# NingZhang1/pyscf_isdf

Measured on AMD Instinct MI355X. Metric: isdf_build_plus_get_jk_wall_time, lower is better.
Workload: dtype f64

## Files before the change

include/mi355_isdf.h:

```cpp
#ifndef MI355_ISDF_H
#define MI355_ISDF_H

#include <stdint.h>

#ifdef __cplusplus
extern "C" {
#endif

typedef struct isdf_ctx* isdf_handle;

#define ISDF_OK 0
#define ISDF_ERR_ARG 1
#define ISDF_ERR_HIP 2
#define ISDF_ERR_LIB 3
#define ISDF_ERR_NUM 4

int isdf_abi_version(void);

int isdf_create(int device_id, isdf_handle* out);
int isdf_destroy(isdf_handle h);
int isdf_set_stream(isdf_handle h, void* hip_stream);
const char* isdf_last_error(isdf_handle h);
int64_t isdf_workspace_bytes(isdf_handle h);
int isdf_release_workspace(isdf_handle h);
// ... 22 lines not shown
int isdf_eval_ao_deriv2(isdf_handle h, const int32_t* atm, int natm, const int32_t* bas, int nbas, const double* env,
                        int nenv, const double* Ls, int nimgs, const double* rcut, const double* d_coords,
                        int64_t ngrids, double* d_ao, int64_t ld, int64_t plane_stride);
int isdf_eval_ao_k_deriv1(isdf_handle h, const int32_t* atm, int natm, const int32_t* bas, int nbas, const double* env,
                          int nenv, const double* Ls, int nimgs, const double* rcut, const double kpt[3], int periodic_part,
                          const double* d_coords, int64_t ngrids, double* d_re, double* d_im, int64_t ld,
                          int64_t plane_stride);

int isdf_eval_ao_k(isdf_handle h,
                   const int32_t* atm, int natm, const int32_t* bas, int nbas,
                   const double* env, int nenv,
                   const double* Ls, int nimgs, const double* rcut,
                   const double kpt[3], int periodic_part,
                   const double* d_coords, int64_t ngrids,
                   double* d_re, double* d_im, int64_t ld);

int isdf_block_row_absmax(isdf_handle h, const double* d_src, int nrow, int64_t ld, int nblk, const int64_t* d_blk_off,
                          double* d_out);
int isdf_gather_cols(isdf_handle h, const double* d_src, int nrow, int64_t ld_src,
                     const int64_t* d_idx, int64_t n, double* d_dst, int64_t ld_dst);

int isdf_partition_by_atom(isdf_handle h, const double* d_coords, int64_t ngrids, const double* atom_coords, int natm,
                           const double a[9], double tie_atol, int32_t* d_owner);

int isdf_select_ip(isdf_handle h, const double* d_ao, int nao, int64_t ld,
                   int nblk, const int64_t* blk_off, const int32_t* nip,
                   double tol, double tie_rtol,
                   double* d_L, int64_t ldL, int64_t* d_piv, int32_t* rank);

int isdf_select_ip_ws(isdf_handle h, const double* d_ao, int nao, int64_t ld,
                      int nblk, const int64_t* blk_off, const int32_t* nip,
                      double tol, double tie_rtol,
                      double* d_L, int64_t ldL, int64_t* d_piv, int32_t* rank,
                      void* d_work, int64_t work_bytes);
int64_t isdf_select_ip_work_bytes(int nao, int64_t m);

int isdf_select_ip_gram(isdf_handle h, double* d_A, int m, int64_t ldA, int nip, double tol, double tie_rtol,
                        int panel, int64_t* d_piv, int32_t* rank);

int isdf_select_ip_cplx(isdf_handle h, const double* d_ao, int nao, int nh, int64_t ld,
                        int nblk, const int64_t* blk_off, const int32_t* nip,
                        double tol, double tie_rtol,
                        double* d_L, int64_t ldL, int64_t* d_piv, int32_t* rank);

int isdf_fit_from_chol(isdf_handle h, double* d_L, int k, int64_t m, int64_t ldL,
                       const int64_t* d_piv);

int isdf_fit_prepare(isdf_handle h, const double* d_ao, int nao, int64_t ld,
                     const int64_t* d_ip, int P, double reg_rel, double* d_aoP, double* d_chol,
                     double* reg_used);
int isdf_fit_apply(isdf_handle h, const double* d_chol, const double* d_aoP, int P, int nao,
                   const double* d_ao, int64_t ng, int64_t ld, int forward_only,
                   double* d_theta, int64_t ldt);
int isdf_fit_prepare_cplx(isdf_handle h, const double* d_ao, int nao, int nh, int64_t ld,
                          const int64_t* d_ip, int P, double reg_rel, double* d_aoP, double* d_chol,
                          double* reg_used);
int isdf_fit_apply_cplx(isdf_handle h, const double* d_chol, const double* d_aoP, int P, int nao, int nh,
                        const double* d_ao, int64_t ng, int64_t ld, int forward_only,
                        double* d_theta, int64_t ldt);
int isdf_fit_global(isdf_handle h, const double* d_ao, int nao, int64_t ngrids, int64_t ld,
                    const int64_t* d_ip, int P, double reg_rel, double* d_theta, int64_t ldt,
                    double* d_aoP, double* reg_used);

int isdf_gather_aoP(isdf_handle h, const double* d_ao, int nao, int64_t ld, const int64_t* d_ip, int P,
                    double* d_aoP);
int isdf_gram_sq(isdf_handle h, const double* d_aoP, int P, int nao, int nh, double* d_A);
int isdf_pair_gram_rows(isdf_handle h, const double* d_aoP, int P, int nao, int nh, const double* d_ao,
                        int64_t ng, int64_t ld, double* d_B, int64_t ldb);
int isdf_block_chol(isdf_handle h, const double* d_A, int P, int nblk, const int32_t* blk_off,
                    double shift_rel, double* d_D, double* shift_used);
int isdf_block_solve(isdf_handle h, const double* d_D, int P, int nblk, const int32_t* blk_off, int side,
                     int trans, double* d_X, int64_t n, int64_t ldx);
int isdf_block_invert(isdf_handle h, const double* d_D, int P, int nblk, const int32_t* blk_off, double* d_Dinv);
int isdf_block_apply(isdf_handle h, const double* d_Dinv, int64_t ldd, int nblk, const int32_t* blk_off,
                     double* d_X, int64_t n, int64_t ldx);
int isdf_pair_rows_block_apply(isdf_handle h, const double* d_aoP, int P, int nao, const double* d_ao, int64_t ng,
                               int64_t ld, const double* d_Dinv, int64_t ldd, int nblk, const int32_t* blk_off,
                               double* d_B, int64_t ldb);
int isdf_pair_rows_squared(isdf_handle h, const double* d_aoP, int rows, int nao, const double* d_ao, int64_t ng,
                           int64_t ld, int* squared);
int isdf_pair_rows_frontier(isdf_handle h, const double* d_aoP, int nnew, int nao, const double* d_ao, int64_t ng,
                            int64_t ld, int squared, const double* d_Dinv, int64_t ldd, int nblk, const int32_t* blk_off,
                            double* d_B, int64_t ldb, int have);

int isdf_gram_prod(isdf_handle h, const double* d_aoP, int P, int nao, const double* d_psiP, int nocc, double* d_A);
int isdf_pair_prod_rows(isdf_handle h, const double* d_aoP, int P, int nao, const double* d_psiP, int nocc,
                        const double* d_ao, int64_t ld, const double* d_psi, int64_t ldpsi, int64_t ng,
                        double* d_B, int64_t ldb);
int isdf_factor_solve_half(isdf_handle h, const double* d_fac, int P, int backward, double* d_X, int64_t n, int64_t ldx);
int isdf_gram_prod_cplx(isdf_handle h, const double* d_aoP, int P, int nao, int nh, const double* d_psiP, int npsi, int npsi_h,
                        double* d_A);
int isdf_pair_prod_rows_cplx(isdf_handle h, const double* d_aoP, int P, int nao, int nh, const double* d_psiP, int npsi,
                             int npsi_h, const double* d_ao, int64_t ld, const double* d_psi, int64_t ldpsi, int64_t ng,
                             double* d_B, int64_t ldb);

int isdf_shift_diag(isdf_handle h, double* d_A, int P, double shift_rel);
int isdf_chol_inplace(isdf_handle h, double* d_A, int P, double shift_rel, double* d_scratch, double* reg_used);

int isdf_factor_solve(isdf_handle h, const double* d_fac, int P, double* d_X, int64_t n, int64_t ldx);

int isdf_bj_probe_vectors(isdf_handle h, double* d_T, int n, const double* d_fac, const double* d_D, int P,
                          int nblk, const int32_t* blk_off);
int isdf_rows_combine(isdf_handle h, const double* d_E, int n, int64_t ldE, int rows, const double* d_Y,
                      int64_t ng, int64_t ldy, double* d_F, int64_t ldf, int accumulate);

int isdf_bj_probe_rows(isdf_handle h, double* d_T, int n, const double* d_fac, const double* d_D, int P, int nblk,
                       const int32_t* blk_off, const double* d_Yp, int64_t ng, int64_t ldy, double* d_F, int64_t ldf);

int isdf_gather_T(isdf_handle h, const double* d_L, int k, int64_t ldL, const int64_t* d_piv,
                  double* d_T);
int isdf_W_from_factor(isdf_handle h, const double* d_F, int P, int kind, double* d_M, int64_t ldm);

int isdf_coulomb_W(isdf_handle h, const double* d_theta, int P, int64_t ldt,
                   const int32_t mesh[3], const double a[9],
                   int row0, int nrows, int batch, int upper_only, double* d_W, int64_t ldw);
int isdf_coulG_half(isdf_handle h, const int32_t mesh[3], const double a[9], double* d_out);
int isdf_spectral_supported(isdf_handle h, const int32_t mesh[3], int batch, int* ok);
int isdf_spectral_rows(isdf_handle h, const double* d_in, int nrows, int64_t ld, const int32_t mesh[3], const int32_t* d_idx,
                       const double* d_scale, int npts, int batch, double* d_out, int64_t ldx);
int isdf_coulomb_rows(isdf_handle h, const double* d_in, int nrows, int64_t ld,
                      const int32_t mesh[3], const double a[9], int batch, double* d_out, int64_t ldo);
int isdf_symmetrize_upper(isdf_handle h, double* d_W, int P, int64_t ldw);
int isdf_symmetrize_mean(isdf_handle h, double* d_W, int P, int64_t ldw, int antisymmetric);

int isdf_get_j(isdf_handle h, const double* d_ao, int nao, int64_t ngrids, int64_t ld,
               const int32_t mesh[3], const double a[9],
               const double* d_dm, int nset, double* d_vj);
int isdf_rho(isdf_handle h, const double* d_ao, int nao, int64_t ng, int64_t ld,
             const double* d_dm, int nset, double* d_rho, int64_t ldrho);
int isdf_coulomb_potential(isdf_handle h, double* d_rho_inout, int nset, int64_t ldrho,
                           const int32_t mesh[3], const double a[9]);
int isdf_vj_from_vR(isdf_handle h, const double* d_ao, int nao, int64_t ng, int64_t ld,
                    const double* d_vR, int nset, int64_t ldv, double* d_vj);

int isdf_get_k_exact(isdf_handle h, const double* d_ao, int nao, int64_t ngrids, int64_t ld,
                     const double* d_C, int nocc, const int32_t mesh[3], const double a[9],
                     int i0, int ni, int max_rows, double* d_vk);

int isdf_get_k(isdf_handle h, const double* d_aoP, int P, int nao,
               const double* d_W, int64_t ldw, int row0, int nrows,
               const double* d_dm, int nset, double* d_vk);

int isdf_coulG_q(isdf_handle h, const int32_t mesh[3], const double a[9], const double q[3], int wrap_around,
                 double omega, double* d_out);

int isdf_coulomb_Wq(isdf_handle h, const double* d_theta, int P, int64_t ldt, const int32_t mesh[3],
                    const double* d_coulG, double weight, int row0, int nrows, int batch,
                    int upper_only, double* d_Wre, double* d_Wim, int64_t ldw);
int isdf_symmetrize_hermitian(isdf_handle h, double* d_Wre, double* d_Wim, int P, int64_t ldw);
int isdf_finish_Wq(isdf_handle h, const double* d_Wre, const double* d_Wim, int P, int64_t ldw,
                   const double* d_phase, double* d_Wc);
int isdf_get_k_pair(isdf_handle h, const double* d_A1, const double* d_A2, const double* d_D2,
                    const double* d_Wq, int P, int nao, double scale, double* d_vk);

int isdf_get_k_exact_kpt(isdf_handle h, const double* d_u1r, const double* d_u1i, int nao, int64_t ld1,
                         const double* d_m2r, const double* d_m2i, int nocc, int64_t ld2, const int32_t mesh[3],
                         const double* d_coulG, double weight, int i0, int ni, int max_rows, double* d_vk_re,
                         double* d_vk_im);

int isdf_coulomb_rows_q(isdf_handle h, const double* d_rows, int nrows, int64_t ld, const int32_t mesh[3],
                        const double* d_coulG, double* d_re, double* d_im);
int isdf_nyquist_spectra(isdf_handle h, const double* d_rows, int nrows, int64_t ld, const int32_t mesh[3], int axis,
                         double* d_re, double* d_im);
int isdf_zhadamard_planes(isdf_handle h, double* d_Ar, double* d_Ai, int64_t lda, const double* d_Br, const double* d_Bi,
                          int64_t ldb, int rows, int64_t cols);
int isdf_rho_k(isdf_handle h, const double* d_ur, const double* d_ui, int nao, int64_t ng, int64_t ld,
               const double* d_DTr, const double* d_DTi, double scale, double* d_rho);
int isdf_vj_k(isdf_handle h, const double* d_ur, const double* d_ui, int nao, int64_t ng, int64_t ld,
              const double* d_vR, double* d_vj_re, double* d_vj_im);

int isdf_pp_local_potential(isdf_handle h, int natm, const double* coords, const double* pp_par,
                            const int32_t mesh[3], const double a[9], double* d_vlocR);
int isdf_pp_projector_overlaps(isdf_handle h, const int32_t* atm, int natm, const int32_t* bas, int nbas,
                               const double* env, int nenv, const double* coords, const double kpt[3],
                               const int32_t* proj_tab, const double* proj_rl, int nproj,
                               const int32_t mesh[3], const double a[9], double* d_out);

int isdf_pp_local_force(isdf_handle h, const double* d_rho, int nset, int64_t ldrho, int natm, const double* coords,
                        const double* pp_par, const int32_t mesh[3], const double a[9], double* d_out);
int isdf_pp_projector_overlaps_ip(isdf_handle h, const int32_t* atm, int natm, const int32_t* bas, int nbas,
                                  const double* env, int nenv, const double* coords, const double kpt[3],
                                  const int32_t* proj_tab, const double* proj_rl, int nproj,
                                  const int32_t mesh[3], const double a[9], double* d_out);
int isdf_rowdot3(isdf_handle h, int M, int64_t K, double alpha, const double* d_A, int64_t lda, int64_t astride, const double* d_s,
                 const double* d_B, int64_t ldb, int accumulate, double* d_out, int64_t ldo);
int isdf_gga_aow(isdf_handle h, int M, int64_t K, const double* d_ao, int64_t ld, int64_t plane, const double* d_w, int64_t ldw,
                 double* d_Z, int64_t ldz, double* d_G, int64_t ldg, int64_t gstride);

int isdf_gemm_nn(isdf_handle h, int M, int64_t N, int K, double alpha, const double* d_A, int64_t lda, const double* d_B,
                 int64_t ldb, double beta, double* d_C, int64_t ldc);
int isdf_hadamard_rows(isdf_handle h, double* d_X, int64_t ldx, const double* d_Y, int64_t ldy, int rows, int64_t cols);

int isdf_uniform_grid(isdf_handle h, const int32_t mesh[3], const double a[9], double* d_coords_soa);
int isdf_rho_pair(isdf_handle h, const double* d_aoA, int nA, const double* d_aoB, int nB, int64_t ng, int64_t ld,
                  const double* d_dm, int nset, double* d_rho, int64_t ldrho);
int isdf_mg_embed_density(isdf_handle h, const double* d_field, int nset, const int32_t mesh_sub[3], double scale,
                          double* d_spec, const int32_t mesh[3], int accumulate);
int isdf_mg_restrict_potential(isdf_handle h, const double* d_spec, int nset, const int32_t mesh[3],
                               const int32_t mesh_sub[3], double scale, double* d_field);
int isdf_mg_coulomb_kernel(isdf_handle h, double* d_spec, int nset, const int32_t mesh[3], const double a[9]);
int isdf_lda_exchange(isdf_handle h, const double* d_rho, int64_t n, double* d_exc, double* d_vxc);
int isdf_lda_vwn_add(isdf_handle h, const double* d_rho, int64_t n, double* d_exc, double* d_vxc);
// ... 33 lines not shown
```

pyscf_isdf_amd/backend.py:

```python
import ctypes
import os
import numpy as np
import torch
from . import lib as _lib

_vp = ctypes.c_void_p


def _np_ptr(a):
    return a.ctypes.data_as(_vp)


class HipBackend:
    name = 'hip-gfx950'

    def __init__(self, device=0):
        if not torch.cuda.is_available():
            raise _lib.IsdfError('no GPU visible to torch; the ISDF path has no CPU fallback')
        self.device = torch.device('cuda', device)
        torch.cuda.set_device(self.device)
        self.handle = _lib.Handle(device)
        if os.environ.get('ISDF_TRSM') == 'subst':
            self.set_option('trsm_substitution', 1)
        if os.environ.get('ISDF_OWN_FFT') in ('0', '1', '2'):
# ... 217 lines not shown

    def gram_sq(self, aoP, A, nh=0):
        self._stream()
        self.handle.call('isdf_gram_sq', self._p(aoP), aoP.shape[0], aoP.shape[1], int(nh), self._p(A))

    def pair_gram_rows(self, aoP, ao, ng, B, nh=0):
        self._stream()
        self.handle.call('isdf_pair_gram_rows', self._p(aoP), aoP.shape[0], aoP.shape[1], int(nh), self._p(ao), int(ng),
                         ao.stride(0), self._p(B), B.stride(0))

    def gram_prod(self, aoP, psiP, A):
        self._stream()
        assert aoP.is_contiguous() and psiP.is_contiguous() and A.is_contiguous() and aoP.shape[0] == psiP.shape[0]
        self.handle.call('isdf_gram_prod', self._p(aoP), aoP.shape[0], aoP.shape[1], self._p(psiP), psiP.shape[1], self._p(A))

    def pair_prod_rows(self, aoP, psiP, ao, psi, ng, B):
        self._stream()
        assert aoP.is_contiguous() and psiP.is_contiguous() and aoP.shape[0] == psiP.shape[0]
        assert ao.stride(1) == 1 and psi.stride(1) == 1 and B.stride(1) == 1
        self.handle.call('isdf_pair_prod_rows', self._p(aoP), aoP.shape[0], aoP.shape[1], self._p(psiP), psiP.shape[1],
                         self._p(ao), ao.stride(0), self._p(psi), psi.stride(0), int(ng), self._p(B), B.stride(0))

    def gram_prod_cplx(self, aoP, nh, psiP, npsi_h, A):
        self._stream()
        assert aoP.is_contiguous() and psiP.is_contiguous() and A.is_contiguous() and aoP.shape[0] == psiP.shape[0]
        self.handle.call('isdf_gram_prod_cplx', self._p(aoP), aoP.shape[0], aoP.shape[1], int(nh), self._p(psiP), psiP.shape[1],
                         int(npsi_h), self._p(A))

    def pair_prod_rows_cplx(self, aoP, nh, psiP, npsi_h, ao, psi, ng, B):
        self._stream()
        assert aoP.is_contiguous() and psiP.is_contiguous() and aoP.shape[0] == psiP.shape[0]
        assert ao.stride(1) == 1 and psi.stride(1) == 1 and B.stride(1) == 1
        self.handle.call('isdf_pair_prod_rows_cplx', self._p(aoP), aoP.shape[0], aoP.shape[1], int(nh), self._p(psiP),
                         psiP.shape[1], int(npsi_h), self._p(ao), ao.stride(0), self._p(psi), psi.stride(0), int(ng), self._p(B),
                         B.stride(0))

    def factor_solve_half(self, fac, backward, X):
        self._stream()
        self.handle.call('isdf_factor_solve_half', self._p(fac), fac.shape[0], int(bool(backward)), self._p(X), X.shape[1],
                         X.stride(0))

    def block_chol(self, A, blk_off, shift_rel, D):
        self._stream()
        blk_off = np.ascontiguousarray(blk_off, dtype=np.int32)
        used = ctypes.c_double(0.0)
        self.handle.call('isdf_block_chol', self._p(A), A.shape[0], len(blk_off) - 1, _np_ptr(blk_off), float(shift_rel),
                         self._p(D), ctypes.byref(used))
        return used.value

    def block_solve(self, D, blk_off, side, trans, X):
        self._stream()
        blk_off = np.ascontiguousarray(blk_off, dtype=np.int32)
        n = X.shape[1] if side == 0 else X.shape[0]
        self.handle.call('isdf_block_solve', self._p(D), D.stride(0), len(blk_off) - 1, _np_ptr(blk_off), int(side), int(trans),
                         self._p(X), int(n), X.stride(0))

    def block_invert(self, D, blk_off, Dinv):
        self._stream()
        blk_off = np.ascontiguousarray(blk_off, dtype=np.int32)
        assert D.is_contiguous() and Dinv.is_contiguous() and Dinv.shape == D.shape
        self.handle.call('isdf_block_invert', self._p(D), D.shape[0], len(blk_off) - 1, _np_ptr(blk_off), self._p(Dinv))

    def block_apply(self, Dinv, blk_off, X):
        self._stream()
        blk_off = np.ascontiguousarray(blk_off, dtype=np.int32)
        self.handle.call('isdf_block_apply', self._p(Dinv), Dinv.stride(0), len(blk_off) - 1, _np_ptr(blk_off), self._p(X),
                         X.shape[1], X.stride(0))

    def pair_rows_block_apply(self, aoP, ao, ng, Dinv, blk_off, B):
        self._stream()
        blk_off = np.ascontiguousarray(blk_off, dtype=np.int32)
        assert aoP.stride(1) == 1 and aoP.stride(0) == aoP.shape[1]
        self.handle.call('isdf_pair_rows_block_apply', self._p(aoP), aoP.shape[0], aoP.shape[1], self._p(ao), int(ng), ao.stride(0),
                         self._p(Dinv), Dinv.stride(0), len(blk_off) - 1, _np_ptr(blk_off), self._p(B), B.stride(0))

    def pair_rows_squared(self, aoP, rows, ao, ng):
        self._stream()
        sq = ctypes.c_int(0)
        self.handle.call('isdf_pair_rows_squared', self._p(aoP), int(rows), aoP.shape[1], self._p(ao), int(ng), ao.stride(0),
                         ctypes.byref(sq))
        return bool(sq.value)

    def pair_rows_frontier(self, aoP_new, ao, ng, squared, Dinv, blk_off, B, have):
        self._stream()
        blk_off = np.ascontiguousarray(blk_off, dtype=np.int32)
        nnew = aoP_new.shape[0]
        assert aoP_new.stride(1) == 1 and aoP_new.stride(0) == aoP_new.shape[1] and B.stride(1) == 1
        assert have + nnew <= B.shape[0] and blk_off[0] == 0 and blk_off[-1] <= have + nnew and B.shape[1] >= ng
        assert len(blk_off) == 1 or (Dinv.shape[0] >= blk_off[-1] and Dinv.shape[1] >= blk_off[-1])
        self.handle.call('isdf_pair_rows_frontier', self._p(aoP_new) if nnew else None, nnew, aoP_new.shape[1], self._p(ao), int(ng),
                         ao.stride(0), int(bool(squared)), self._p(Dinv) if len(blk_off) > 1 else None, Dinv.stride(0) if len(blk_off) > 1 else 0,
                         len(blk_off) - 1, _np_ptr(blk_off), self._p(B), B.stride(0), int(have))

    def shift_diag(self, A, shift_rel):
        self._stream()
        self.handle.call('isdf_shift_diag', self._p(A), A.shape[0], float(shift_rel))

    def chol_inplace(self, A, shift_rel, scratch=None):
        self._stream()
        reg = ctypes.c_double(0.0)
        assert scratch is None or scratch.numel() >= A.numel()
        self.handle.call('isdf_chol_inplace', self._p(A), A.shape[0], float(shift_rel),
                         self._p(scratch) if scratch is not None else None, ctypes.byref(reg))
        return reg.value

    def factor_solve(self, fac, X):
        self._stream()
        self.handle.call('isdf_factor_solve', self._p(fac), fac.shape[0], self._p(X), X.shape[1], X.stride(0))

    def bj_probe_rows(self, T, fac, D, blk_off, Yp, ng, F):
        self._stream()
        blk_off = np.ascontiguousarray(blk_off, dtype=np.int32)
        self.handle.call('isdf_bj_probe_rows', self._p(T), T.shape[0], self._p(fac), self._p(D), D.shape[0],
                         len(blk_off) - 1, _np_ptr(blk_off), self._p(Yp), int(ng), Yp.stride(0), self._p(F), F.stride(0))

    def bj_probe_vectors(self, T, fac, D, blk_off):
        self._stream()
        blk_off = np.ascontiguousarray(blk_off, dtype=np.int32)
        assert T.is_contiguous()
        self.handle.call('isdf_bj_probe_vectors', self._p(T), T.shape[0], self._p(fac), self._p(D), D.shape[0],
                         len(blk_off) - 1, _np_ptr(blk_off))

    def rows_combine(self, E, Y, F, accumulate=False):
        self._stream()
        assert E.stride(1) == 1 and Y.stride(1) == 1 and F.stride(1) == 1 and E.shape[1] == Y.shape[0]
        self.handle.call('isdf_rows_combine', self._p(E), E.shape[0], E.stride(0), E.shape[1], self._p(Y), Y.shape[1],
                         Y.stride(0), self._p(F), F.stride(0), int(bool(accumulate)))

    def gather_T(self, L, k, piv, T):
        self._stream()
        assert T.is_contiguous() and T.shape == (k, k)
        self.handle.call('isdf_gather_T', self._p(L), int(k), L.stride(0), self._p(piv), self._p(T))

    def W_from_factor(self, F, kind, M):
        self._stream()
        assert F.is_contiguous()
        self.handle.call('isdf_W_from_factor', self._p(F), M.shape[0], int(kind), self._p(M), M.stride(0))

    def fit_global(self, ao, ngrids, ip, reg_rel, theta, aoP):
        self._stream()
        assert ip.dtype == torch.int64 and aoP.is_contiguous()
        reg = ctypes.c_double(0.0)
        self.handle.call('isdf_fit_global', self._p(ao), ao.shape[0], int(ngrids), ao.stride(0), self._p(ip),
                         ip.numel(), float(reg_rel), self._p(theta), theta.stride(0), self._p(aoP), ctypes.byref(reg))
        return reg.value

    def coulomb_W(self, theta, mesh, a, row0, nrows, batch, W, upper_only=False):
        self._stream()
        mesh = np.ascontiguousarray(mesh, dtype=np.int32)
        a = np.ascontiguousarray(a, dtype=np.float64)
        self.handle.call('isdf_coulomb_W', self._p(theta), theta.shape[0], theta.stride(0), _np_ptr(mesh), _np_ptr(a),
                         int(row0), int(nrows), int(batch), int(bool(upper_only)), self._p(W), W.stride(0))

    def coulomb_rows(self, rows, mesh, a, batch, out=None):
        self._stream()
        out = rows if out is None else out
        mesh = np.ascontiguousarray(mesh, dtype=np.int32)
        a = np.ascontiguousarray(a, dtype=np.float64)
        self.handle.call('isdf_coulomb_rows', self._p(rows), rows.shape[0], rows.stride(0), _np_ptr(mesh), _np_ptr(a),
                         int(batch), self._p(out), out.stride(0))

    def spectral_supported(self, mesh, batch=512):
        ok = ctypes.c_int(0)
        mesh = np.ascontiguousarray(mesh, dtype=np.int32)
        self.handle.call('isdf_spectral_supported', _np_ptr(mesh), int(batch), ctypes.byref(ok))
        return bool(ok.value)

    def coulG_half(self, mesh, a):
        self._stream()
        mesh = np.ascontiguousarray(mesh, dtype=np.int32)
        a = np.ascontiguousarray(a, dtype=np.float64)
        out = self.empty((int(mesh[0]) * int(mesh[1]) * (int(mesh[2]) // 2 + 1),))
        self.handle.call('isdf_coulG_half', _np_ptr(mesh), _np_ptr(a), self._p(out))
        return self.to_host(out).reshape(int(mesh[0]), int(mesh[1]), int(mesh[2]) // 2 + 1)

    def spectral_rows(self, rows, mesh, idx, scale, out, batch=512):
        self._stream()
        mesh = np.ascontiguousarray(mesh, dtype=np.int32)
        assert rows.is_contiguous() and out.stride(1) == 1 and idx.dtype == torch.int32 and out.stride(0) % 2 == 0
        self.handle.call('isdf_spectral_rows', self._p(rows), rows.shape[0], rows.stride(0), _np_ptr(mesh), self._p(idx),
                         self._p(scale), int(idx.numel()), int(batch), self._p(out), out.stride(0))

    def symmetrize_upper(self, W):
        self._stream()
        self.handle.call('isdf_symmetrize_upper', self._p(W), W.shape[0], W.stride(0))

    def symmetrize_mean(self, W, antisymmetric=False):
        self._stream()
        self.handle.call('isdf_symmetrize_mean', self._p(W), W.shape[0], W.stride(0), int(bool(antisymmetric)))

    def get_j(self, ao, ngrids, mesh, a, dm, vj):
        self._stream()
        mesh = np.ascontiguousarray(mesh, dtype=np.int32)
        a = np.ascontiguousarray(a, dtype=np.float64)
        assert dm.is_contiguous() and vj.is_contiguous()
        self.handle.call('isdf_get_j', self._p(ao), ao.shape[0], int(ngrids), ao.stride(0), _np_ptr(mesh), _np_ptr(a),
                         self._p(dm), dm.shape[0], self._p(vj))

    def rho(self, ao, ng, dm, rho):
        self._stream()
        self.handle.call('isdf_rho', self._p(ao), ao.shape[0], int(ng), ao.stride(0), self._p(dm), dm.shape[0],
                         self._p(rho), rho.stride(0))

    def coulomb_potential(self, rho, mesh, a):
        self._stream()
        mesh = np.ascontiguousarray(mesh, dtype=np.int32)
        a = np.ascontiguousarray(a, dtype=np.float64)
        self.handle.call('isdf_coulomb_potential', self._p(rho), rho.shape[0], rho.stride(0), _np_ptr(mesh), _np_ptr(a))

    def vj_from_vR(self, ao, ng, vR, vj):
        self._stream()
        self.handle.call('isdf_vj_from_vR', self._p(ao), ao.shape[0], int(ng), ao.stride(0), self._p(vR), vR.shape[0],
                         vR.stride(0), self._p(vj))

    def get_k(self, aoP, W, row0, nrows, dm, vk):
        self._stream()
        assert aoP.is_contiguous() and dm.is_contiguous() and vk.is_contiguous()
        self.handle.call('isdf_get_k', self._p(aoP), aoP.shape[0], aoP.shape[1], self._p(W), W.stride(0), int(row0),
                         int(nrows), self._p(dm), dm.shape[0], self._p(vk))

    def get_k_exact(self, ao, ngrids, C, mesh, a, i0, ni, max_rows, vk):
        self._stream()
        mesh = np.ascontiguousarray(mesh, dtype=np.int32)
        a = np.ascontiguousarray(a, dtype=np.float64)
        assert C.is_contiguous() and vk.is_contiguous()
        self.handle.call('isdf_get_k_exact', self._p(ao), ao.shape[0], int(ngrids), ao.stride(0), self._p(C), C.shape[1],
                         _np_ptr(mesh), _np_ptr(a), int(i0), int(ni), int(max_rows), self._p(vk))

    def gemm_nn(self, A, B, C, alpha=1.0, beta=0.0):
        self._stream()
        self.handle.call('isdf_gemm_nn', A.shape[0], B.shape[1], A.shape[1], float(alpha), self._p(A), A.stride(0), self._p(B),
                         B.stride(0), float(beta), self._p(C), C.stride(0))

    def hadamard_rows(self, X, Y):
        self._stream()
        self.handle.call('isdf_hadamard_rows', self._p(X), X.stride(0), self._p(Y), Y.stride(0), X.shape[0], X.shape[1])

    def gemm_nt(self, A, B, C, alpha=1.0, beta=0.0, kscale=None):
        self._stream()
        M, K = A.shape
        N = B.shape[0]
        assert B.shape[1] == K and tuple(C.shape) == (M, N) and A.stride(1) == 1 and B.stride(1) == 1 and C.stride(1) == 1
        ks = self._p(kscale) if kscale is not None else _vp(0)
        self.handle.call('isdf_gemm_nt', M, N, K, float(alpha), self._p(A), A.stride(0), self._p(B), B.stride(0), ks,
                         float(beta), self._p(C), C.stride(0))

    def gemm_nt_had3(self, A, H, B3, C3, alpha=1.0, beta=0.0):
        self._stream()
        M, K = A.shape
        N = B3.shape[1]
        assert tuple(B3.shape) == (3, N, K) and tuple(C3.shape) == (3, M, N) and A.stride(1) == 1 and B3.stride(2) == 1 and C3.stride(2) == 1
        assert H is None or (tuple(H.shape) == (M, K) and H.stride(1) == 1)
        self.handle.call('isdf_gemm_nt_had3', M, N, K, float(alpha), self._p(A), A.stride(0), self._p(H) if H is not None else _vp(0),
                         H.stride(0) if H is not None else 0, self._p(B3), B3.stride(1), B3.stride(0), float(beta), self._p(C3),
                         C3.stride(1), C3.stride(0))

    def pack_table_pm(self, table, mesh, idx, scale, s, a):
        self._stream()
        mesh = np.ascontiguousarray(mesh, dtype=np.int32)
        assert idx.dtype == torch.int32 and table.is_contiguous() and table.numel() == int(np.prod(mesh))
        assert s.is_contiguous() and a.is_contiguous() and s.numel() == a.numel()
        self.handle.call('isdf_pack_table_pm', self._p(table), _np_ptr(mesh), self._p(idx), int(idx.numel()), float(scale),
                         self._p(s), self._p(a), int(s.numel()))

# ... 274 lines not shown
```

pyscf_isdf_amd/csrc/common.h:

```cpp
#pragma once
#include <hip/hip_runtime.h>
#include <rocblas/rocblas.h>
#include <rocsolver/rocsolver.h>
#include <hipfft/hipfft.h>
#include <cstdint>
#include <cstdio>
#include <cstring>
#include <string>
#include <vector>
#include <map>
#include "../../include/mi355_isdf.h"

struct FftPlan {
  hipfftHandle fwd = 0, bwd = 0;
  size_t work_bytes = 0;
};

struct ProfRec {
  hipEvent_t e0 = nullptr, e1 = nullptr;
};
struct ProfEntry {
  std::vector<ProfRec> recs;
  double work = 0.0;
  double ms = 0.0;
  int64_t launches = 0;
};

struct WsKernel {
  double alpha = 0.0;
  double ak[9] = {0};
  int mesh[3] = {0, 0, 0};
  double maxq[3] = {0, 0, 0};
  const double* vq = nullptr;
};

struct isdf_ctx {
  int profiling = 0;
  std::map<std::string, ProfEntry> prof;
  int device = 0;
  hipStream_t stream = nullptr;
  rocblas_handle blas = nullptr;
  std::string err;
  std::map<std::vector<int>, FftPlan> plans;
  std::map<std::string, std::pair<void*, size_t>> ws;
  int num_cu = 256;
  int trsm_substitution = 0;
  int own_fft = 2;
  int gemm_nn_own = 0;
  int attr_gemm_b = 0, attr_gemm_nn = 0, attr_gram_tri = 0, attr_herm = 0;
  int cand_gram = 1;
  int conv_pipe = 1;
  int conv_sub_rows = 0;
  int gram_pivot_tpb = 256;
  int gram_compact = 1;
  int gram_compact_permille = 875;
  int block_apply_waves = 16;
  int block_apply_reg = 1;
  double coul_omega = 0.0;
  double coul_rc = 0.0;
  int coul_sphere = 0;
  WsKernel wsk;
};

int isdf_fail(isdf_handle h, int code, const char* fmt, ...);
void* isdf_ws(isdf_handle h, const char* name, size_t bytes);
int isdf_get_plan(isdf_handle h, const int32_t mesh[3], int batch, FftPlan** out);
int get_coulG_half(isdf_handle h, const int32_t mesh[3], const double a[9], double extra_scale, double** out);
bool conv_rows_own_supported(const int32_t mesh[3], int nb);
bool conv_rows_q_own_supported(isdf_handle h, const int32_t mesh[3], int nb);
bool spectral_rows_own_supported(isdf_handle h, const int32_t mesh[3], int nb);
int spectral_rows_own(isdf_handle h, const double* d_in, int nb, const int32_t mesh[3], const int32_t* d_idx, const double* d_scale,
                      int npts, double* d_out, int64_t ldx, HIP_vector_type<double, 2u>* zbuf);
int conv_rows_q_own(isdf_handle h, const double* d_in, double* d_re, double* d_im, int nb, const int32_t mesh[3], const double* tab,
                    double2* zhalf, double2* zfull);
int conv_rows_own(isdf_handle h, const double* d_in, double* d_out, int nb, const int32_t mesh[3], const double* cg,
                  double2* zbuf);

#define HIP_TRY(h, expr)                                                                    \
  do {                                                                                      \
    hipError_t e_ = (expr);                                                                 \
    if (e_ != hipSuccess)                                                                   \
      return isdf_fail(h, ISDF_ERR_HIP, "%s:%d %s -> %s", __FILE__, __LINE__, #expr,        \
                       hipGetErrorString(e_));                                              \
  } while (0)
#define BLAS_TRY(h, expr)                                                                   \
  do {                                                                                      \
    rocblas_status s_ = (expr);                                                             \
    if (s_ != rocblas_status_success)                                                       \
      return isdf_fail(h, ISDF_ERR_LIB, "%s:%d %s -> rocblas status %d", __FILE__, __LINE__, \
                       #expr, (int)s_);                                                     \
  } while (0)
#define FFT_TRY(h, expr)                                                                    \
  do {                                                                                      \
    hipfftResult r_ = (expr);                                                               \
    if (r_ != HIPFFT_SUCCESS)                                                               \
      return isdf_fail(h, ISDF_ERR_LIB, "%s:%d %s -> hipfft result %d", __FILE__, __LINE__,  \
                       #expr, (int)r_);                                                     \
  } while (0)
#define KERNEL_CHECK(h) HIP_TRY(h, hipGetLastError())
#define ARG_CHECK(h, cond)                                                                  \
  do {                                                                                      \
    if (!(cond)) return isdf_fail(h, ISDF_ERR_ARG, "%s:%d argument check failed: %s",       \
                                  __FILE__, __LINE__, #cond);                               \
  } while (0)

static inline int64_t cdiv(int64_t a, int64_t b) { return (a + b - 1) / b; }

struct ProfScope {
  isdf_handle h;
  ProfRec rec;
  ProfEntry* ent = nullptr;
  ProfScope(isdf_handle h_, const char* name, double work, int64_t launches = 1) : h(h_) {
    if (!h || !h->profiling) return;
    ent = &h->prof[name];
    ent->work += work;
    ent->launches += launches;
    if (hipEventCreate(&rec.e0) != hipSuccess || hipEventCreate(&rec.e1) != hipSuccess) { ent = nullptr; return; }
    (void)hipEventRecord(rec.e0, h->stream);
  }
  ~ProfScope() {
    if (!ent) return;
    (void)hipEventRecord(rec.e1, h->stream);
    ent->recs.push_back(rec);
  }
};

int gemm_nt_f64(isdf_handle h, int M, int N, int64_t K, double alpha, const double* A, int64_t lda,
                const double* B, int64_t ldb, double beta, double* C, int64_t ldc);
int gemm_nt_f64_scaled(isdf_handle h, int M, int N, int64_t K, double alpha, const double* A, int64_t lda,
                       const double* B, int64_t ldb, const double* kscale, double beta, double* C,
                       int64_t ldc);
int trsm_lower_left(isdf_handle h, bool trans, int m, int64_t n, const double* L, int64_t ldl, double* X, int64_t ldx);
int trsm_lower_right(isdf_handle h, bool trans, int m, int64_t n, const double* L, int64_t ldl, double* X, int64_t ldx);
int block_forward_solve(isdf_handle h, const double* D, int64_t ldd, int nblk, const int32_t* blk_off_host, double* X,
                        int64_t ldx, int64_t n);
int block_apply_inverse(isdf_handle h, const double* Dinv, int64_t ldd, int nblk, const int32_t* blk_off_host, double* X,
                        int64_t ldx, int64_t n, bool square_input = false);
int transpose_rm(isdf_handle h, const double* src, int64_t lds, int64_t rows, int64_t cols, double* dst, int64_t ldd);
int tri_left(isdf_handle h, bool trans, int m, int64_t n, const double* L, int64_t ldl, double* X, int64_t ldx);
int tri_right(isdf_handle h, bool trans, int m, int64_t n, const double* L, int64_t ldl, double* X, int64_t ldx);
bool gemm_nn_f64_supported(isdf_handle h, int64_t M, int64_t N, int64_t K, const double* A, int64_t lda, const double* B,
                           int64_t ldb);
int gemm_nn_f64(isdf_handle h, int64_t M, int64_t N, int64_t K, const double* A, int64_t lda, const double* B, int64_t ldb,
                double* C, int64_t ldc, bool square);
int gemm_rm(isdf_handle h, char opA, char opB, int64_t M, int64_t N, int64_t K, double alpha,
            const double* A, int64_t lda, const double* B, int64_t ldb, double beta, double* C,
            int64_t ldc);

__host__ __device__ inline int64_t gram_tri_row(int64_t r) {
  const int64_t tm = r >> 8;
  return 32768 * tm * (tm + 1) + (r & 255) * ((tm + 1) << 8);
}
static inline int64_t gram_tri_size(int64_t m) { return m > 0 ? gram_tri_row(m - 1) + (((m - 1) >> 8) + 1) * 256 : 0; }
struct GramTriUnit { int blk, tm, tn, pad; };
int gram_tri_blocks(isdf_handle h, const double* X, int64_t ldx, int K, const GramTriUnit* d_units, int64_t nunits,
                    const int64_t* d_blk_off, int64_t row0, const int64_t* d_tri_off, double* S, double flop);
```

pyscf_isdf_amd/csrc/coulomb.hip:

```cpp
#include "common.h"

namespace {

struct Recip { double b[9]; };
__device__ inline double g2_of(int ix, int iy, int iz, int n0, int n1, int n2, const Recip& r) {
  const double fx = (ix < (n0 + 1) / 2) ? ix : ix - n0;
  const double fy = (iy < (n1 + 1) / 2) ? iy : iy - n1;
  const double fz = (iz < (n2 + 1) / 2) ? iz : iz - n2;
  const double gx = fx * r.b[0] + fy * r.b[3] + fz * r.b[6];
  const double gy = fx * r.b[1] + fy * r.b[4] + fz * r.b[7];
  const double gz = fx * r.b[2] + fy * r.b[5] + fz * r.b[8];
  return gx * gx + gy * gy + gz * gz;
}

__device__ inline double range_factor(double g2, double omega) {
  if (omega == 0.0) return 1.0;
  const double e = exp(-0.25 * g2 / (omega * omega));
  return omega > 0.0 ? e : 1.0 - e;
}
__device__ inline double kernel_value(double g2, double omega, double rc) {
  const double fourpi = 4.0 * 3.14159265358979323846;
  if (rc > 0.0) return g2 == 0.0 ? 0.5 * fourpi * rc * rc : fourpi / g2 * (1.0 - cos(sqrt(g2) * rc));
  return g2 == 0.0 ? 0.0 : fourpi / g2 * range_factor(g2, omega);
}
// ... 250 lines not shown
  const int64_t gc = (int64_t)mesh[0] * mesh[1] * (mesh[2] / 2 + 1);
  ARG_CHECK(h, ldt == G);
  if (nrows == 0) return ISDF_OK;
  if (batch > nrows) batch = nrows;
  double* cg = nullptr;
  int rc = get_coulG_half(h, mesh, a, 1.0, &cg);
  if (rc) return rc;
  double* V = (double*)isdf_ws(h, "coul_V", sizeof(double) * (size_t)batch * G);
  double2* Z = (double2*)isdf_ws(h, "coul_Z", sizeof(double2) * (size_t)batch * gc);
  if (!V || !Z) return ISDF_ERR_HIP;
  const double det = a[0] * (a[4] * a[8] - a[5] * a[7]) - a[1] * (a[3] * a[8] - a[5] * a[6]) +
                     a[2] * (a[3] * a[7] - a[4] * a[6]);
  const double w = fabs(det) / (double)G;
  for (int r = row0; r < row0 + nrows; r += batch) {
    const int nb = std::min(batch, row0 + nrows - r);
    rc = convolve_rows(h, d_theta + (int64_t)r * ldt, V, nb, mesh, cg, Z);
    if (rc) return rc;
    const int c0 = upper_only ? r : 0;
    rc = gemm_nt_f64(h, nb, P - c0, G, w, V, G, d_theta + (int64_t)c0 * ldt, ldt, 0.0,
                     d_W + (int64_t)r * ldw + c0, ldw);
    if (rc) return rc;
  }
  return ISDF_OK;
}

extern "C" int isdf_coulomb_potential(isdf_handle h, double* d_rho, int nset, int64_t ldrho,
                                      const int32_t mesh[3], const double a[9]) {
  if (!h) return ISDF_ERR_ARG;
  ARG_CHECK(h, d_rho && mesh && a && nset > 0);
  const int64_t G = (int64_t)mesh[0] * mesh[1] * mesh[2];
  const int64_t gc = (int64_t)mesh[0] * mesh[1] * (mesh[2] / 2 + 1);
  ARG_CHECK(h, ldrho == G);
  const double det = a[0] * (a[4] * a[8] - a[5] * a[7]) - a[1] * (a[3] * a[8] - a[5] * a[6]) +
                     a[2] * (a[3] * a[7] - a[4] * a[6]);
  double* cg = nullptr;
  int rc = get_coulG_half(h, mesh, a, fabs(det) / (double)G, &cg);
  if (rc) return rc;
  double2* Z = (double2*)isdf_ws(h, "coul_Z", sizeof(double2) * (size_t)nset * gc);
  if (!Z) return ISDF_ERR_HIP;
  return convolve_rows(h, d_rho, d_rho, nset, mesh, cg, Z);
}

extern "C" int isdf_coulomb_rows(isdf_handle h, const double* d_in, int nrows, int64_t ld,
                                 const int32_t mesh[3], const double a[9], int batch, double* d_out,
                                 int64_t ldo) {
  if (!h) return ISDF_ERR_ARG;
  ARG_CHECK(h, d_in && d_out && mesh && a && nrows >= 0 && batch > 0);
  const int64_t G = (int64_t)mesh[0] * mesh[1] * mesh[2];
  const int64_t gc = (int64_t)mesh[0] * mesh[1] * (mesh[2] / 2 + 1);
  ARG_CHECK(h, ld == G && ldo == G);
  if (nrows == 0) return ISDF_OK;
  if (batch > nrows) batch = nrows;
  double* cg = nullptr;
  int rc = get_coulG_half(h, mesh, a, 1.0, &cg);
  if (rc) return rc;
  double2* Z = (double2*)isdf_ws(h, "coul_Z", sizeof(double2) * (size_t)batch * gc);
  if (!Z) return ISDF_ERR_HIP;
  for (int r = 0; r < nrows; r += batch) {
    const int nb = std::min(batch, nrows - r);
    rc = convolve_rows(h, d_in + (int64_t)r * ld, d_out + (int64_t)r * ldo, nb, mesh, cg, Z);
    if (rc) return rc;
  }
  return ISDF_OK;
}

extern "C" int isdf_coulG_half(isdf_handle h, const int32_t mesh[3], const double a[9], double* d_out) {
  if (!h) return ISDF_ERR_ARG;
  ARG_CHECK(h, mesh && a && d_out);
  double* cg = nullptr;
  int rc = get_coulG_half(h, mesh, a, 1.0, &cg);
  if (rc) return rc;
  const int64_t gc = (int64_t)mesh[0] * mesh[1] * (mesh[2] / 2 + 1);
  HIP_TRY(h, hipMemcpyAsync(d_out, cg, sizeof(double) * gc, hipMemcpyDeviceToDevice, h->stream));
  return ISDF_OK;
}

extern "C" int isdf_spectral_supported(isdf_handle h, const int32_t mesh[3], int batch, int* ok) {
  if (!h) return ISDF_ERR_ARG;
  ARG_CHECK(h, mesh && ok && batch > 0);
  *ok = spectral_rows_own_supported(h, mesh, batch) ? 1 : 0;
  return ISDF_OK;
}

extern "C" int isdf_spectral_rows(isdf_handle h, const double* d_in, int nrows, int64_t ld, const int32_t mesh[3],
                                  const int32_t* d_idx, const double* d_scale, int npts, int batch, double* d_out, int64_t ldx) {
  if (!h) return ISDF_ERR_ARG;
  ARG_CHECK(h, d_in && d_out && mesh && d_idx && d_scale && nrows >= 0 && batch > 0 && npts > 0);
  const int64_t G = (int64_t)mesh[0] * mesh[1] * mesh[2];
  const int64_t gc = (int64_t)mesh[0] * mesh[1] * (mesh[2] / 2 + 1);
  ARG_CHECK(h, ld == G && npts <= gc);
  if (nrows == 0) return ISDF_OK;
  if (batch > nrows) batch = nrows;
  if (!spectral_rows_own_supported(h, mesh, batch))
    return isdf_fail(h, ISDF_ERR_ARG, "isdf_spectral_rows: mesh %d x %d x %d is not covered by the plane FFT", mesh[0], mesh[1], mesh[2]);
  double2* Z = (double2*)isdf_ws(h, "coul_Z", sizeof(double2) * (size_t)batch * gc);
  if (!Z) return ISDF_ERR_HIP;
  for (int r = 0; r < nrows; r += batch) {
    const int nb = std::min(batch, nrows - r);
    int rc = spectral_rows_own(h, d_in + (int64_t)r * ld, nb, mesh, d_idx, d_scale, npts, d_out + (int64_t)r * ldx, ldx, Z);
    if (rc) return rc;
  }
  return ISDF_OK;
}
```

pyscf_isdf_amd/csrc/fft_conv.hip:

```cpp
#include "common.h"
#include <type_traits>

namespace {

constexpr int TPB = 256;
constexpr int MAXSTAGE = 12;

struct Axis {
  int n;
  int nstage;
  int radix[MAXSTAGE];
  const double2* tw;
};

__device__ inline double2 cadd(double2 a, double2 b) { return make_double2(a.x + b.x, a.y + b.y); }
__device__ inline double2 csub(double2 a, double2 b) { return make_double2(a.x - b.x, a.y - b.y); }
__device__ inline double2 cmul(double2 a, double2 b) { return make_double2(a.x * b.x - a.y * b.y, a.x * b.y + a.y * b.x); }
template <int SIGN>
__device__ inline double2 mul_si(double2 a) { return SIGN > 0 ? make_double2(-a.y, a.x) : make_double2(a.y, -a.x); }
template <int SIGN>
__device__ inline double2 twid(const double2* __restrict__ tw, int idx) {
  double2 w = tw[idx];
  if (SIGN > 0) w.y = -w.y;
  return w;
// ... 388 lines not shown
      }
      __syncthreads();
      z = stockham_all<1>(z, (z == x) ? y : x, ax, ZC, M);
    }
  }
  for (int c = threadIdx.x; c < n * ZC; c += TPB) {
    const int e = c / ZC, m = c - e * ZC;
    if (m < M) base[(int64_t)e * es + m] = z[c];
  }
}

template <int SIGN, int ZCT>
__device__ inline void fft_fast(double2* buf, const Axis& ax, int Ls, const double2* tw) {
  fft<SIGN, TPB, 2048 / TPB, true, FixedLines<ZCT>>(buf, ax, Ls, ZCT, tw);
}

template <int ZCT>
__global__ __launch_bounds__(TPB) void z_r2c_fast_kernel(const double* __restrict__ in, double2* __restrict__ out,
                                                         int64_t nlines, Axis ax) {
  extern __shared__ double2 lds[];
  const int n = ax.n, nh = n / 2 + 1;
  constexpr int Ls = ZCT + 1;
  double2* x = lds;
  double2* tw = lds + n * Ls;
  for (int k = threadIdx.x; k < n; k += TPB) tw[k] = ax.tw[k];
  const int64_t line0 = (int64_t)blockIdx.x * 2 * ZCT;
  const int nl = (int)min((int64_t)2 * ZCT, nlines - line0);
  const double* src = in + line0 * n;
  const float inv_n = 1.0f / (float)n;
  for (int c = threadIdx.x; c < 2 * ZCT * n; c += TPB) {
    const int l = (int)(((float)c + 0.5f) * inv_n), e = c - l * n;
    const double v = (l < nl) ? src[c] : 0.0;
    ((double*)(x + e * Ls + (l >> 1)))[l & 1] = v;
  }
  __syncthreads();
  fft_fast<-1, ZCT>(x, ax, Ls, tw);
  double2* dstc = out + line0 * nh;
  const float inv_nh = 1.0f / (float)nh;
  for (int c = threadIdx.x; c < nl * nh; c += TPB) {
    const int l = (int)(((float)c + 0.5f) * inv_nh), k = c - l * nh;
    const int m = l >> 1;
    const double2 zk = x[k * Ls + m];
    const double2 zn = x[(k == 0 ? 0 : n - k) * Ls + m];
    double2 r;
    if ((l & 1) == 0) r = make_double2(0.5 * (zk.x + zn.x), 0.5 * (zk.y - zn.y));
    else r = make_double2(0.5 * (zk.y + zn.y), -0.5 * (zk.x - zn.x));
    dstc[c] = r;
  }
}

template <int ZCT>
__global__ __launch_bounds__(TPB) void z_c2r_fast_kernel(const double2* __restrict__ in, double* __restrict__ out,
                                                         int64_t nlines, Axis ax) {
  extern __shared__ double2 lds[];
  const int n = ax.n, nh = n / 2 + 1;
  constexpr int Ls = ZCT + 1;
  double2* x = lds;
  double2* tw = lds + n * Ls;
  for (int k = threadIdx.x; k < n; k += TPB) tw[k] = ax.tw[k];
  const int64_t line0 = (int64_t)blockIdx.x * 2 * ZCT;
  const int nl = (int)min((int64_t)2 * ZCT, nlines - line0);
  const int M = (nl + 1) / 2;
  const double2* src = in + line0 * nh;
  const float inv_nh = 1.0f / (float)nh;
  for (int c = threadIdx.x; c < M * nh; c += TPB) {
    const int m = (int)(((float)c + 0.5f) * inv_nh), k = c - m * nh;
    double2 a = src[(int64_t)(2 * m) * nh + k];
    double2 b = (2 * m + 1 < nl) ? src[(int64_t)(2 * m + 1) * nh + k] : make_double2(0.0, 0.0);
    const bool selfconj = (k == 0) || (2 * k == n);
    if (selfconj) { a.y = 0.0; b.y = 0.0; }
    x[k * Ls + m] = make_double2(a.x - b.y, a.y + b.x);
    if (!selfconj) x[(n - k) * Ls + m] = make_double2(a.x + b.y, -a.y + b.x);
  }
  __syncthreads();
  fft_fast<1, ZCT>(x, ax, Ls, tw);
  double* dst = out + line0 * n;
  const float inv_n = 1.0f / (float)n;
  for (int c = threadIdx.x; c < nl * n; c += TPB) {
    const int l = (int)(((float)c + 0.5f) * inv_n), e = c - l * n;
    dst[c] = ((const double*)(x + e * Ls + (l >> 1)))[l & 1];
  }
}

template <int MODE, int ZCT>
__global__ __launch_bounds__(TPB) void strided_fft_fast_kernel(double2* __restrict__ data, int64_t os, int64_t es, int Mtot,
                                                               Axis ax, int ntile, const double* __restrict__ table) {
  extern __shared__ double2 lds[];
  const int n = ax.n;
  double2* x = lds;
  double2* tw = lds + n * ZCT;
  for (int k = threadIdx.x; k < n; k += TPB) tw[k] = ax.tw[k];
  const int nouter = gridDim.x / ntile;
  const int64_t outer = (MODE == 2) ? blockIdx.x % nouter : blockIdx.x / ntile;
  const int m0 = (int)((MODE == 2) ? blockIdx.x / nouter : blockIdx.x % ntile) * ZCT;
  const int M = min(ZCT, Mtot - m0);
  double2* base = data + outer * os + m0;
  for (int c = threadIdx.x; c < n * ZCT; c += TPB) {
    const int e = c / ZCT, m = c & (ZCT - 1);
    if (m < M) x[c] = base[(int64_t)e * es + m];
  }
  __syncthreads();
  if (MODE == 1) {
    fft_fast<1, ZCT>(x, ax, ZCT, tw);
  } else {
    fft_fast<-1, ZCT>(x, ax, ZCT, tw);
    if (MODE == 2) {
      const double* tb = table + m0;
      for (int c = threadIdx.x; c < n * ZCT; c += TPB) {
        const int e = c / ZCT, m = c & (ZCT - 1);
        if (m < M) {
          const double g = tb[(int64_t)e * es + m];
          double2 v = x[c];
          v.x *= g;
          v.y *= g;
          x[c] = v;
        }
      }
      __syncthreads();
      fft_fast<1, ZCT>(x, ax, ZCT, tw);
    }
  }
  for (int c = threadIdx.x; c < n * ZCT; c += TPB) {
    const int e = c / ZCT, m = c & (ZCT - 1);
    if (m < M) base[(int64_t)e * es + m] = x[c];
  }
}

constexpr int TPBP = 1024;
constexpr int PLANE_ENTRIES = 10240;
constexpr int PIPE_NT = 768;

template <int SIGN, int NT, int N, int RA, int RB, int MMAX>
__device__ __forceinline__ void fft_plane_fixed(double2* buf, int Ls, int M, const double2* tw) {
  static_assert(RA * RB == N, "two stages");
  stage<SIGN, RA, NT, ((N / RA) * MMAX + NT - 1) / NT, true, AnyLines>(buf, N, N, 1, Ls, M, tw, opaque_tid());
  stage<SIGN, RB, NT, ((N / RB) * MMAX + NT - 1) / NT, true, AnyLines>(buf, N, N / RA, RA, Ls, M, tw, opaque_tid());
}

struct PlaneAny {
  static constexpr int NT = TPBP, PER = PLANE_ENTRIES / TPBP;
  static constexpr int KS_HALF = PER, KS_PAIR = PER / 2 + 1, KS_FULL = PER;
  int n1, n2, n2h, npair;
  __device__ PlaneAny(const Axis& az, const Axis& ay) : n1(ay.n), n2(az.n), n2h(az.n / 2 + 1), npair((ay.n + 1) / 2) {}
  __device__ static int tid() { return threadIdx.x; }
  template <int SIGN, bool FULL>
  __device__ __forceinline__ static void transform(double2* buf, const Axis& ax, int Ls, int M, const double2* tw) {
    fft<SIGN, NT, PER, false, AnyLines>(buf, ax, Ls, M, tw);
  }
};
template <int N, int RA, int RB>
struct PlaneSquare {
  static constexpr int NT = PIPE_NT, n1 = N, n2 = N, n2h = N / 2 + 1, npair = (N + 1) / 2;
  static constexpr int KS_HALF = (n1 * n2h + NT - 1) / NT, KS_PAIR = (npair * n2h + NT - 1) / NT, KS_FULL = (N * N + NT - 1) / NT;
  constexpr PlaneSquare() = default;
  __device__ static int tid() { return opaque_tid(); }
  template <int SIGN, bool FULL>
  __device__ __forceinline__ static void transform(double2* buf, const Axis&, int Ls, int M, const double2* tw) {
    fft_plane_fixed<SIGN, NT, N, RA, RB, FULL ? N : N / 2 + 1>(buf, Ls, M, tw);
  }
};

__device__ inline double zero_of(const double*) { return 0.0; }
__device__ inline double2 zero_of(const double2*) { return make_double2(0.0, 0.0); }
template <int NT, int NPRE, class T>
__device__ __forceinline__ void prefetch(T (&pre)[NPRE], const T* __restrict__ src, int count, int tid) {
#pragma unroll
  for (int u = 0; u < NPRE; ++u) {
    const int c = tid + u * NT;
    pre[u] = c < count ? src[c] : zero_of(src);
  }
}

template <class D>
__device__ __forceinline__ void plane_fwd_body(const D d, double2* lds, int Lz, int bufsz, const Axis& az, const Axis& ay,
                                               double2* __restrict__ dst, double2 (&r)[D::KS_HALF]) {
  double2* x = lds;
  const double2* twz = lds + bufsz;
  const double2* twy = twz + d.n2;
  d.template transform<-1, false>(x, az, Lz, d.npair, twz);
  int tid = D::tid();
  const float inv_nh = 1.0f / (float)d.n2h;
#pragma unroll
  for (int u = 0; u < D::KS_HALF; ++u) {
    const int c = tid + u * D::NT;
    if (c < d.n1 * d.n2h) {
      const int l = fdiv(c, inv_nh), k = c - l * d.n2h;
      const int m = l >> 1;
      r[u] = separate_pair(x[k * Lz + m], x[(k == 0 ? 0 : d.n2 - k) * Lz + m], l & 1);
    }
  }
  __syncthreads();
#pragma unroll
  for (int u = 0; u < D::KS_HALF; ++u) {
    const int c = tid + u * D::NT;
    if (c < d.n1 * d.n2h) x[c] = r[u];
  }
  __syncthreads();
  d.template transform<-1, false>(x, ay, d.n2h, d.n2h, twy);
  tid = D::tid();
  for (int c = tid; c < d.n1 * d.n2h; c += D::NT) dst[c] = x[c];
}

template <class D>
__device__ __forceinline__ void plane_inv_body(const D d, double2* lds, int Lz, int bufsz, const Axis& az, const Axis& ay,
                                               double* __restrict__ dst, double2 (&za)[D::KS_PAIR], double2 (&zb)[D::KS_PAIR]) {
  double2* x = lds;
  const double2* twz = lds + bufsz;
  const double2* twy = twz + d.n2;
// ... 281 lines not shown
    static const int big[] = {16, 15, 12, 10, 9, 8, 6, 5, 4, 3, 2};
    int best[MAXSTAGE], nbest = MAXSTAGE + 1, bestmax = 1 << 30;
    int cur[MAXSTAGE];
    struct Rec {
      static void go(int rest, int maxr, int depth, int* cur, int* best, int& nbest, int& bestmax) {
        if (rest == 1) {
          const int mx = depth ? cur[0] : 1;
          if (depth < nbest || (depth == nbest && mx < bestmax)) {
            nbest = depth; bestmax = mx;
            for (int i = 0; i < depth; ++i) best[i] = cur[i];
          }
          return;
        }
        if (depth + 1 > nbest || depth >= MAXSTAGE) return;
        for (int r : big)
          if (r <= maxr && rest % r == 0) { cur[depth] = r; go(rest / r, r, depth + 1, cur, best, nbest, bestmax); }
      }
    };
    Rec::go(n, 16, 0, cur, best, nbest, bestmax);
    if (nbest <= MAXSTAGE) {
      ax->nstage = nbest;
      for (int i = 0; i < nbest; ++i) ax->radix[i] = best[i];
      return true;
    }
  }
  const int order[4] = {4, 2, 3, 5};
  for (int r : order)
    while (n % r == 0 && n > 1) {
      if (ax->nstage >= MAXSTAGE) return false;
      ax->radix[ax->nstage++] = r;
      n /= r;
    }
  for (int p = 7; n > 1 && p <= 13; p += 2)
    while (n % p == 0) {
      if (ax->nstage >= MAXSTAGE) return false;
      ax->radix[ax->nstage++] = p;
      n /= p;
    }
  return n == 1;
}

int make_axes(isdf_handle h, const int32_t mesh[3], Axis ax[3], const char* who) {
  for (int d = 0; d < 3; ++d) {
    if (!factorise(mesh[d], &ax[d])) return isdf_fail(h, ISDF_ERR_ARG, "%s: unsupported mesh dimension %d", who, mesh[d]);
    char name[32];
    snprintf(name, sizeof(name), "fft_tw_%d", mesh[d]);
    const bool fresh = h->ws.find(name) == h->ws.end();
    double2* tw = (double2*)isdf_ws(h, name, sizeof(double2) * (size_t)mesh[d]);
    if (!tw) return ISDF_ERR_HIP;
    if (fresh) {
      std::vector<double2> host(mesh[d]);
      for (int k = 0; k < mesh[d]; ++k) {
        const double t = -2.0 * 3.14159265358979323846 * (double)k / (double)mesh[d];
        host[k] = make_double2(cos(t), sin(t));
      }
      HIP_TRY(h, hipMemcpyAsync(tw, host.data(), sizeof(double2) * (size_t)mesh[d], hipMemcpyHostToDevice, h->stream));
      HIP_TRY(h, hipStreamSynchronize(h->stream));
    }
    ax[d].tw = tw;
  }
  return ISDF_OK;
}

template <bool FWD, class IN, class OUT>
void launch_z(isdf_handle h, bool fast, int L, const IN* in, OUT* out, int64_t nlines, const Axis& ax) {
  const dim3 grid((unsigned)cdiv(nlines, 2 * L));
  const size_t n = ax.n;
  if (fast) {
    const size_t lds = sizeof(double2) * (n * (L + 1) + n);
    with_lines(L, [&](auto z) {
      constexpr int ZCT = decltype(z)::value;
      if constexpr (FWD) z_r2c_fast_kernel<ZCT><<<grid, dim3(TPB), lds, h->stream>>>(in, out, nlines, ax);
      else z_c2r_fast_kernel<ZCT><<<grid, dim3(TPB), lds, h->stream>>>(in, out, nlines, ax);
    });
  } else {
    const size_t lds = sizeof(double2) * 2 * n * (L + 1);
    if constexpr (FWD) z_r2c_kernel<<<grid, dim3(TPB), lds, h->stream>>>(in, out, nlines, ax, L);
    else z_c2r_kernel<<<grid, dim3(TPB), lds, h->stream>>>(in, out, nlines, ax, L);
  }
}

template <int MODE>
void launch_strided(isdf_handle h, bool fast, int L, double2* data, int64_t nouter, int64_t os, int64_t es, int Mtot, const Axis& ax,
                    const double* table) {
  const int nt = (int)cdiv(Mtot, L);
  const dim3 grid((unsigned)(nouter * nt));
  const size_t n = ax.n;
  if (fast)
    with_lines(L, [&](auto z) {
      strided_fft_fast_kernel<MODE, decltype(z)::value><<<grid, dim3(TPB), sizeof(double2) * (n * L + n), h->stream>>>(
          data, os, es, Mtot, ax, nt, table);
    });
  else
    strided_fft_kernel<MODE><<<grid, dim3(TPB), sizeof(double2) * 2 * n * L, h->stream>>>(data, os, es, Mtot, ax, L, nt, table);
}

#define ISDF_PLANE_SIZES(X) X(64, 8, 8) X(72, 9, 8) X(80, 10, 8) X(96, 12, 8) X(100, 10, 10) X(108, 12, 9) X(120, 12, 10)
constexpr int PIPE_ANY = 1024, PIPE_Q_MAX = 96;

template <class F>
bool with_pipe_size(isdf_handle h, const Axis& az, const Axis& ay, int nmax, F f) {
  if (h->conv_pipe == 0 || ay.n != az.n || ay.n > nmax || ay.nstage != 2) return false;
#define ISDF_PLANE_SIZE(NN, RA, RB)                                \
  if (ay.n == NN && ay.radix[0] == RA && ay.radix[1] == RB) {      \
    f(PlaneSquare<NN, RA, RB>{});                                  \
    return true;                                                   \
  }
  ISDF_PLANE_SIZES(ISDF_PLANE_SIZE)
#undef ISDF_PLANE_SIZE
  return false;
}

template <class K>
int raise_lds(isdf_handle h, K kernel) {
  HIP_TRY(h, hipFuncSetAttribute((const void*)kernel, hipFuncAttributeMaxDynamicSharedMemorySize, LDS_MAX));
  return ISDF_OK;
}
dim3 pipe_grid(isdf_handle h, int nplanes) { return dim3((unsigned)std::min<int64_t>(nplanes, h->num_cu)); }

int launch_plane_fwd(isdf_handle h, const double* in, double2* out, const Axis* ax, const PlaneGeo& g, int nplanes, int pipe_max) {
  int rc = ISDF_OK;
  const bool piped = with_pipe_size(h, ax[2], ax[1], pipe_max, [&](auto d) {
    auto kernel = plane_fwd_pipe_kernel<decltype(d)>;
    if ((rc = raise_lds(h, kernel)) == ISDF_OK)
      kernel<<<pipe_grid(h, nplanes), dim3(PIPE_NT), g.bytes, h->stream>>>(in, out, ax[2], ax[1], g.Lz, g.bufsz, nplanes);
  });
  if (!piped && (rc = raise_lds(h, plane_fwd_kernel)) == ISDF_OK)
    plane_fwd_kernel<<<dim3((unsigned)nplanes), dim3(TPBP), g.bytes, h->stream>>>(in, out, ax[2], ax[1], g.Lz, g.bufsz);
  return rc;
}

int launch_plane_inv(isdf_handle h, const double2* in, double* out, const Axis* ax, const PlaneGeo& g, int nplanes, int pipe_max) {
  int rc = ISDF_OK;
  const bool piped = with_pipe_size(h, ax[2], ax[1], pipe_max, [&](auto d) {
    auto kernel = plane_inv_pipe_kernel<decltype(d)>;
    if ((rc = raise_lds(h, kernel)) == ISDF_OK)
      kernel<<<pipe_grid(h, nplanes), dim3(PIPE_NT), g.bytes, h->stream>>>(in, out, ax[2], ax[1], g.Lz, g.bufsz, nplanes);
  });
  if (!piped && (rc = raise_lds(h, plane_inv_kernel)) == ISDF_OK)
    plane_inv_kernel<<<dim3((unsigned)nplanes), dim3(TPBP), g.bytes, h->stream>>>(in, out, ax[2], ax[1], g.Lz, g.bufsz);
  return rc;
}

int launch_plane_c2c_inv(isdf_handle h, const double2* in, double* out_re, double* out_im, const Axis* ax, const PlaneGeo& g,
                         int nplanes) {
  int rc = ISDF_OK;
  const bool piped = with_pipe_size(h, ax[2], ax[1], PIPE_Q_MAX, [&](auto d) {
    if constexpr (decltype(d)::n1 <= PIPE_Q_MAX) {
      auto kernel = plane_c2c_inv_pipe_kernel<decltype(d)>;
      if ((rc = raise_lds(h, kernel)) == ISDF_OK)
        kernel<<<pipe_grid(h, nplanes), dim3(PIPE_NT), g.bytes, h->stream>>>(in, out_re, out_im, ax[2], ax[1], g.Lz, g.bufsz, nplanes);
    } else {
      rc = isdf_fail(h, ISDF_ERR_ARG, "launch_plane_c2c_inv: no pipelined kernel for %d^2", (int)decltype(d)::n1);
    }
  });
  if (!piped && (rc = raise_lds(h, plane_c2c_inv_kernel)) == ISDF_OK)
    plane_c2c_inv_kernel<<<dim3((unsigned)nplanes), dim3(TPBP), g.bytes, h->stream>>>(in, out_re, out_im, ax[2], ax[1], g.Lz, g.bufsz);
  return rc;
}

}

bool conv_rows_own_supported(const int32_t mesh[3], int nb) {
  if (nb < 1 || (int64_t)nb * mesh[0] * mesh[1] * 4 >= 2147483647LL || (int64_t)nb * mesh[1] * (mesh[2] / 2 + 1) >= 2147483647LL)
    return false;
  for (int d = 0; d < 3; ++d) {
    Axis ax;
    if (mesh[d] < 1 || mesh[d] > 1024 || !factorise(mesh[d], &ax)) return false;
    if (lines_per_tile(mesh[d], d == 2 ? 1 : 0) < 1) return false;
  }
  return true;
}

int conv_rows_own(isdf_handle h, const double* d_in, double* d_out, int nb, const int32_t mesh[3], const double* cg,
                  double2* zbuf) {
  const int n0 = mesh[0], n1 = mesh[1], n2 = mesh[2], n2h = n2 / 2 + 1;
  Axis ax[3];
  if (int rc = make_axes(h, mesh, ax, "conv_rows_own")) return rc;
  const int64_t gc = (int64_t)n0 * n1 * n2h;
  const int64_t nlines = (int64_t)nb * n0 * n1;
  ARG_CHECK(h, nlines * 4 < 2147483647LL && (int64_t)nb * cdiv((int64_t)n1 * n2h, 1) < 2147483647LL);
  const int LP = lines_per_tile(n2, 1);
  const int ZY = lines_per_tile(n1, 0), ZX = lines_per_tile(n0, 0);
  if (LP < 1 || ZY < 1 || ZX < 1) return isdf_fail(h, ISDF_ERR_ARG, "conv_rows_own: mesh too large for the LDS tiles");
  const int64_t G = (int64_t)n0 * n1 * n2;
  const int FZ = fast_lines(n2), FY = fast_lines(n1), FX = fast_lines(n0);
  const bool smooth = smooth235(ax[0]) && smooth235(ax[1]) && smooth235(ax[2]);
  const PlaneGeo geo = (h->own_fft == 2 && smooth && FX >= 1) ? plane_geometry(n1, n2, false) : PlaneGeo{0, 0, 0};
  ProfScope ps(h, geo.bytes ? "coulomb_conv_own_3pass[byte]" : "coulomb_conv_own_5pass[byte]", 32.0 * (double)G * nb,
               geo.bytes ? 3 : 5);
  if (geo.bytes) {
    const int sub = h->conv_sub_rows > 0 ? std::min(nb, h->conv_sub_rows) : nb;
    for (int r0 = 0; r0 < nb; r0 += sub) {
      const int nr = std::min(sub, nb - r0);
      double2* zb = zbuf + (int64_t)r0 * gc;
      const int nplanes = (int)((int64_t)nr * n0);
      if (int rc = launch_plane_fwd(h, d_in + (int64_t)r0 * G, zb, ax, geo, nplanes, PIPE_ANY)) return rc;
      launch_strided<2>(h, true, FX, zb, nr, gc, (int64_t)n1 * n2h, n1 * n2h, ax[0], cg);
      if (int rc = launch_plane_inv(h, zb, d_out + (int64_t)r0 * G, ax, geo, nplanes, PIPE_ANY)) return rc;
    }
    KERNEL_CHECK(h);
    return ISDF_OK;
  }
  const bool fast = smooth && FZ >= 1 && FY >= 1 && FX >= 1;
  const int Lz = fast ? FZ : LP, Ly = fast ? FY : ZY, Lx = fast ? FX : ZX;
  launch_z<true>(h, fast, Lz, d_in, zbuf, nlines, ax[2]);
  launch_strided<0>(h, fast, Ly, zbuf, (int64_t)nb * n0, (int64_t)n1 * n2h, (int64_t)n2h, n2h, ax[1], nullptr);
  launch_strided<2>(h, fast, Lx, zbuf, nb, gc, (int64_t)n1 * n2h, n1 * n2h, ax[0], cg);
  launch_strided<1>(h, fast, Ly, zbuf, (int64_t)nb * n0, (int64_t)n1 * n2h, (int64_t)n2h, n2h, ax[1], nullptr);
  launch_z<false>(h, fast, Lz, zbuf, d_out, nlines, ax[2]);
  KERNEL_CHECK(h);
  return ISDF_OK;
}

__global__ void spectral_pack_kernel(const double2* __restrict__ z, int64_t gc, const int32_t* __restrict__ idx,
                                     const double* __restrict__ scale, int npts, double2* __restrict__ out, int64_t ldx2) {
  const int64_t j = (int64_t)blockIdx.x * blockDim.x + threadIdx.x;
  if (j >= ldx2) return;
  const int row = blockIdx.y;
  double2 v = make_double2(0.0, 0.0);
  if (j < npts) {
    const double2 t = z[(int64_t)row * gc + idx[j]];
    const double s = scale[j];
    v = make_double2(t.x * s, t.y * s);
  }
  out[(int64_t)row * ldx2 + j] = v;
}

bool spectral_rows_own_supported(isdf_handle h, const int32_t mesh[3], int nb) {
  if (h->own_fft != 2 || !conv_rows_own_supported(mesh, nb)) return false;
  Axis ax[3];
  for (int d = 0; d < 3; ++d)
    if (!factorise(mesh[d], &ax[d]) || !smooth235(ax[d])) return false;
  return fast_lines(mesh[0]) >= 1 && plane_geometry(mesh[1], mesh[2], false).bytes != 0;
}

int spectral_rows_own(isdf_handle h, const double* d_in, int nb, const int32_t mesh[3], const int32_t* d_idx,
                      const double* d_scale, int npts, double* d_out, int64_t ldx, double2* zbuf) {
  const int n0 = mesh[0], n1 = mesh[1], n2 = mesh[2], n2h = n2 / 2 + 1;
  Axis ax[3];
  if (int rc = make_axes(h, mesh, ax, "spectral_rows_own")) return rc;
  const int64_t gc = (int64_t)n0 * n1 * n2h;
  const PlaneGeo geo = plane_geometry(n1, n2, false);
  const int FX = fast_lines(n0);
  ARG_CHECK(h, geo.bytes && FX >= 1 && (int64_t)nb * n0 < 2147483647LL && nb <= 65535 && (ldx & 1) == 0 && ldx >= 2 * (int64_t)npts);
  ProfScope ps(h, "spectral_rows_own[byte]", (8.0 * (double)n0 * n1 * n2 + 8.0 * (double)ldx) * nb, 3);
  if (int rc = launch_plane_fwd(h, d_in, zbuf, ax, geo, (int)((int64_t)nb * n0), PIPE_ANY)) return rc;
  launch_strided<0>(h, true, FX, zbuf, nb, gc, (int64_t)n1 * n2h, n1 * n2h, ax[0], nullptr);
  const int64_t ldx2 = ldx / 2;
  spectral_pack_kernel<<<dim3((unsigned)cdiv(ldx2, 256), (unsigned)nb), dim3(256), 0, h->stream>>>(zbuf, gc, d_idx, d_scale, npts,
                                                                                                  (double2*)d_out, ldx2);
  KERNEL_CHECK(h);
  return ISDF_OK;
}

bool conv_rows_q_own_supported(isdf_handle h, const int32_t mesh[3], int nb) {
  if (!h->own_fft) return false;
  if (nb < 1 || nb > 65535 || (int64_t)nb * mesh[0] >= 2147483647LL) return false;
  Axis ax[3];
  for (int d = 0; d < 3; ++d)
    if (mesh[d] < 2 || mesh[d] > 1024 || !factorise(mesh[d], &ax[d]) || !smooth235(ax[d])) return false;
  return fast_lines(mesh[0]) >= 1 && plane_geometry(mesh[1], mesh[2], false).bytes && plane_geometry(mesh[1], mesh[2], true).bytes;
}

int conv_rows_q_own(isdf_handle h, const double* d_in, double* d_re, double* d_im, int nb, const int32_t mesh[3],
                    const double* tab, double2* zhalf, double2* zfull) {
  const int n0 = mesh[0], n1 = mesh[1], n2 = mesh[2], n2h = n2 / 2 + 1;
  Axis ax[3];
  if (int rc = make_axes(h, mesh, ax, "conv_rows_q_own")) return rc;
  const int64_t G = (int64_t)n0 * n1 * n2, gc = (int64_t)n0 * n1 * n2h;
  const PlaneGeo geo_r = plane_geometry(n1, n2, false), geo_c = plane_geometry(n1, n2, true);
  const int FX = fast_lines(n0);
  ARG_CHECK(h, geo_r.bytes && geo_c.bytes && FX >= 1 && (int64_t)nb * n0 < 2147483647LL && nb <= 65535);
  ProfScope ps(h, "coulomb_conv_q_own[byte]", 64.0 * (double)G * nb, 5);
  const int nplanes = (int)((int64_t)nb * n0);
  if (int rc = launch_plane_fwd(h, d_in, zhalf, ax, geo_r, nplanes, PIPE_Q_MAX)) return rc;
  launch_strided<0>(h, true, FX, zhalf, nb, gc, (int64_t)n1 * n2h, n1 * n2h, ax[0], nullptr);
  expand_mul_kernel<<<dim3((unsigned)cdiv(G, 256), (unsigned)nb), dim3(256), 0, h->stream>>>(zhalf, zfull, tab, n0, n1, n2,
                                                                                            1.0 / (double)G);
  launch_strided<1>(h, true, FX, zfull, nb, G, (int64_t)n1 * n2, n1 * n2, ax[0], nullptr);
  if (int rc = launch_plane_c2c_inv(h, zfull, d_re, d_im, ax, geo_c, nplanes)) return rc;
  KERNEL_CHECK(h);
  return ISDF_OK;
}
```

pyscf_isdf_amd/csrc/fit.hip:

```cpp
#include "common.h"
#include <cstdlib>

namespace {

__global__ void gather_T_kernel(const double* __restrict__ L, int64_t ldL,
                                const int64_t* __restrict__ piv, int k, double* __restrict__ T) {
  const int s = blockIdx.x * blockDim.x + threadIdx.x;
  const int t = blockIdx.y;
  if (s >= k) return;
  T[(int64_t)t * k + s] = (s >= t) ? L[(int64_t)t * ldL + piv[s]] : 0.0;
}

__global__ void square_kernel(double* __restrict__ x, int64_t rows, int64_t cols, int64_t ld) {
  const int64_t c = (int64_t)blockIdx.x * blockDim.x + threadIdx.x;
  const int64_t r = blockIdx.y;
  if (c >= cols) return;
  const double v = x[r * ld + c];
  x[r * ld + c] = v * v;
}

__global__ void square_add_kernel(double* __restrict__ x, int64_t ld, const double* __restrict__ y, int64_t ldy,
                                  int64_t cols) {
  const int64_t c = (int64_t)blockIdx.x * blockDim.x + threadIdx.x;
  const int64_t r = blockIdx.y;
// ... 284 lines not shown
      for (int pp = 0; pp < np; ++pp) {
        const double v = y[(int64_t)pp * ldy];
#pragma unroll
        for (int j = 0; j < 8; ++j) acc[j] = fma(sE[j][pp], v, acc[j]);
      }
    }
  }
  if (live)
    for (int j = 0; j < n; ++j) F[(int64_t)j * ldf + g] = accumulate ? F[(int64_t)j * ldf + g] + acc[j] : acc[j];
}

__global__ void add_diag_const_kernel(double* __restrict__ A, int n, int64_t ld, double v) {
  const int i = blockIdx.x * blockDim.x + threadIdx.x;
  if (i < n) A[(int64_t)i * ld + i] += v;
}
}

extern "C" int isdf_block_chol(isdf_handle h, const double* d_A, int P, int nblk, const int32_t* blk_off,
                               double shift_rel, double* d_D, double* shift_used) {
  if (!h) return ISDF_ERR_ARG;
  ARG_CHECK(h, d_A && d_D && blk_off && P > 0 && nblk > 0 && blk_off[0] == 0 && blk_off[nblk] == P && shift_rel >= 0);
  int* info = (int*)isdf_ws(h, "fit_info", 256);
  if (!info) return ISDF_ERR_HIP;
  double* maxdiag = (double*)(info + 16);
  HIP_TRY(h, hipMemsetAsync(d_D, 0, sizeof(double) * (size_t)P * P, h->stream));
  hipLaunchKernelGGL(max_diag_kernel, dim3(1), dim3(256), 0, h->stream, d_A, P, maxdiag);
  double md = 0.0;
  HIP_TRY(h, hipMemcpyAsync(&md, maxdiag, sizeof(double), hipMemcpyDeviceToHost, h->stream));
  HIP_TRY(h, hipStreamSynchronize(h->stream));
  double worst = 0.0;
  for (int b = 0; b < nblk; ++b) {
    const int off = blk_off[b], nb = blk_off[b + 1] - off;
    if (nb <= 0) continue;
    ARG_CHECK(h, nb <= 65535);
    double reg = shift_rel;
    int h_info = 1;
    for (int attempt = 0; attempt < 6 && h_info != 0; ++attempt) {
      hipLaunchKernelGGL(copy_block_kernel, dim3((unsigned)cdiv(nb, 128), (unsigned)nb), dim3(128), 0, h->stream, d_A, P,
                         off, nb, d_D);
      if (reg > 0)
        hipLaunchKernelGGL(add_diag_const_kernel, dim3((unsigned)cdiv(nb, 256)), dim3(256), 0, h->stream,
                           d_D + (int64_t)off * P + off, nb, (int64_t)P, reg * md);
      KERNEL_CHECK(h);
      BLAS_TRY(h, rocsolver_dpotrf(h->blas, rocblas_fill_upper, nb, d_D + (int64_t)off * P + off, P, info));
      HIP_TRY(h, hipMemcpyAsync(&h_info, info, sizeof(int), hipMemcpyDeviceToHost, h->stream));
      HIP_TRY(h, hipStreamSynchronize(h->stream));
      if (h_info == 0) { worst = std::max(worst, reg); break; }
      reg = (reg > 0.0) ? reg * 100.0 : 1e-14;
    }
    if (h_info != 0)
      return isdf_fail(h, ISDF_ERR_NUM, "diagonal block %d of A_PP is not positive definite even with shift %g * max diag "
                       "(minor %d of %d)", b, reg / 100.0, h_info, nb);
  }
  if (shift_used) *shift_used = worst;
  return ISDF_OK;
}

extern "C" int isdf_block_solve(isdf_handle h, const double* d_D, int P, int nblk, const int32_t* blk_off, int side,
                                int trans, double* d_X, int64_t n, int64_t ldx) {
  if (!h) return ISDF_ERR_ARG;
  ARG_CHECK(h, d_D && d_X && blk_off && P > 0 && nblk > 0 && n > 0 && (side == 0 || side == 1) && (trans == 0 || trans == 1));
  ARG_CHECK(h, n < 2147483647LL && ldx < 2147483647LL);
  if (side == 0 && trans == 0 && !h->trsm_substitution) {
    ARG_CHECK(h, blk_off[0] == 0 && blk_off[nblk] <= P);
    return block_forward_solve(h, d_D, P, nblk, blk_off, d_X, ldx, n);
  }
  for (int b = 0; b < nblk; ++b) {
    const int off = blk_off[b], nb = blk_off[b + 1] - off;
    if (nb <= 0) continue;
    const double* Db = d_D + (int64_t)off * P + off;
    const int rc = (side == 0) ? tri_left(h, trans != 0, nb, n, Db, P, d_X + (int64_t)off * ldx, ldx)
                               : tri_right(h, trans != 0, nb, n, Db, P, d_X + off, ldx);
    if (rc) return rc;
  }
  return ISDF_OK;
}

namespace {
__global__ void block_identity_kernel(double* __restrict__ E, int P, const int32_t* __restrict__ blk_of_row) {
  const int64_t i = (int64_t)blockIdx.x * blockDim.x + threadIdx.x;
  if (i < (int64_t)P * P) E[i] = (i / P == i % P) ? 1.0 : 0.0;
  (void)blk_of_row;
}
}

extern "C" int isdf_block_invert(isdf_handle h, const double* d_D, int P, int nblk, const int32_t* blk_off, double* d_Dinv) {
  if (!h) return ISDF_ERR_ARG;
  ARG_CHECK(h, d_D && d_Dinv && blk_off && P > 0 && nblk > 0 && blk_off[0] == 0 && blk_off[nblk] <= P);
  hipLaunchKernelGGL(block_identity_kernel, dim3((unsigned)cdiv((int64_t)P * P, 256)), dim3(256), 0, h->stream, d_Dinv, P,
                     (const int32_t*)nullptr);
  KERNEL_CHECK(h);
  return block_forward_solve(h, d_D, P, nblk, blk_off, d_Dinv, P, P);
}

extern "C" int isdf_block_apply(isdf_handle h, const double* d_Dinv, int64_t ldd, int nblk, const int32_t* blk_off,
                                double* d_X, int64_t n, int64_t ldx) {
  if (!h) return ISDF_ERR_ARG;
  ARG_CHECK(h, d_Dinv && d_X && blk_off && nblk > 0 && n > 0 && ldx >= n && blk_off[0] == 0 && blk_off[nblk] <= ldd);
  return block_apply_inverse(h, d_Dinv, ldd, nblk, blk_off, d_X, ldx, n);
}

extern "C" int isdf_pair_rows_block_apply(isdf_handle h, const double* d_aoP, int P, int nao, const double* d_ao, int64_t ng,
                                          int64_t ld, const double* d_Dinv, int64_t ldd, int nblk, const int32_t* blk_off,
                                          double* d_B, int64_t ldb) {
  if (!h) return ISDF_ERR_ARG;
  ARG_CHECK(h, d_aoP && d_ao && d_Dinv && d_B && blk_off && P > 0 && nao > 0 && ng > 0 && ld >= ng && ldb >= ng && nblk > 0);
  ARG_CHECK(h, blk_off[0] == 0 && blk_off[nblk] == P);
  const bool own = gemm_nn_f64_supported(h, P, ng, nao, d_aoP, nao, d_ao, ld);
  int rc = product_rows(h, P, ng, nao, d_aoP, d_ao, ld, d_B, ldb, own);
  if (rc) return rc;
  return block_apply_inverse(h, d_Dinv, ldd, nblk, blk_off, d_B, ldb, ng, !own);
}

extern "C" int isdf_pair_rows_squared(isdf_handle h, const double* d_aoP, int rows, int nao, const double* d_ao, int64_t ng,
                                      int64_t ld, int* squared) {
  if (!h) return ISDF_ERR_ARG;
  ARG_CHECK(h, d_aoP && d_ao && squared && rows > 0 && nao > 0 && ng > 0 && ld >= ng);
  *squared = gemm_nn_f64_supported(h, rows, ng, nao, d_aoP, nao, d_ao, ld) ? 1 : 0;
  return ISDF_OK;
}

extern "C" int isdf_pair_rows_frontier(isdf_handle h, const double* d_aoP, int nnew, int nao, const double* d_ao, int64_t ng,
                                       int64_t ld, int squared, const double* d_Dinv, int64_t ldd, int nblk,
                                       const int32_t* blk_off, double* d_B, int64_t ldb, int have) {
  if (!h) return ISDF_ERR_ARG;
  ARG_CHECK(h, d_ao && d_B && nnew >= 0 && nnew <= 65535 && have >= 0 && nblk >= 0 && nao > 0 && ng > 0 && ld >= ng && ldb >= ng);
  ARG_CHECK(h, (nnew == 0 || d_aoP) && (nblk == 0 || (d_Dinv && blk_off && blk_off[0] == 0 && blk_off[nblk] <= have + nnew)));
  if (nnew > 0) {
    double* rows = d_B + (int64_t)have * ldb;
    int rc = squared ? product_rows(h, nnew, ng, nao, d_aoP, d_ao, ld, rows, ldb, true)
                     : gemm_rm(h, 'N', 'N', nnew, ng, nao, 1.0, d_aoP, nao, d_ao, ld, 0.0, rows, ldb);
    if (rc) return rc;
  }
  if (nblk == 0) return ISDF_OK;
  return block_apply_inverse(h, d_Dinv, ldd, nblk, blk_off, d_B, ldb, ng, !squared);
}

extern "C" int isdf_shift_diag(isdf_handle h, double* d_A, int P, double shift_rel) {
  if (!h) return ISDF_ERR_ARG;
  ARG_CHECK(h, d_A && P > 0 && shift_rel >= 0);
  if (shift_rel == 0.0) return ISDF_OK;
  int* info = (int*)isdf_ws(h, "fit_info", 256);
  if (!info) return ISDF_ERR_HIP;
  double* maxdiag = (double*)(info + 16);
  hipLaunchKernelGGL(max_diag_kernel, dim3(1), dim3(256), 0, h->stream, d_A, P, maxdiag);
  hipLaunchKernelGGL(add_diag_kernel, dim3((unsigned)cdiv(P, 256)), dim3(256), 0, h->stream, d_A, P, maxdiag, shift_rel);
  KERNEL_CHECK(h);
  return ISDF_OK;
}

extern "C" int isdf_chol_inplace(isdf_handle h, double* d_A, int P, double shift_rel, double* d_scratch,
                                 double* reg_used) {
  if (!h) return ISDF_ERR_ARG;
  ARG_CHECK(h, d_A && P > 0 && shift_rel >= 0);
  int* info = (int*)isdf_ws(h, "fit_info", 256);
  double* keep = d_scratch ? d_scratch : (double*)isdf_ws(h, "chol_keep", sizeof(double) * (size_t)P * P);
  if (!info || !keep) return ISDF_ERR_HIP;
  double* maxdiag = (double*)(info + 16);
  HIP_TRY(h, hipMemcpyAsync(keep, d_A, sizeof(double) * (size_t)P * P, hipMemcpyDeviceToDevice, h->stream));
  double reg = shift_rel;
  for (int attempt = 0; attempt < 5; ++attempt) {
    if (attempt > 0)
      HIP_TRY(h, hipMemcpyAsync(d_A, keep, sizeof(double) * (size_t)P * P, hipMemcpyDeviceToDevice, h->stream));
    if (reg > 0) {
      hipLaunchKernelGGL(max_diag_kernel, dim3(1), dim3(256), 0, h->stream, d_A, P, maxdiag);
      hipLaunchKernelGGL(add_diag_kernel, dim3((unsigned)cdiv(P, 256)), dim3(256), 0, h->stream, d_A, P, maxdiag, reg);
      KERNEL_CHECK(h);
    }
    { ProfScope ps(h, "rocsolver_dpotrf[flop]", (double)P * P * P / 3.0);
      BLAS_TRY(h, rocsolver_dpotrf(h->blas, rocblas_fill_upper, P, d_A, P, info)); }
    int h_info = 0;
    HIP_TRY(h, hipMemcpyAsync(&h_info, info, sizeof(int), hipMemcpyDeviceToHost, h->stream));
    HIP_TRY(h, hipStreamSynchronize(h->stream));
    if (h_info == 0) {
      if (reg_used) *reg_used = reg;
      return ISDF_OK;
    }
    reg = (reg > 0.0) ? reg * 100.0 : 1e-14;
  }
  return isdf_fail(h, ISDF_ERR_NUM, "matrix is not numerically positive definite even with diagonal shift %g * max diag",
                   reg / 100.0);
}

extern "C" int isdf_factor_solve(isdf_handle h, const double* d_fac, int P, double* d_X, int64_t n, int64_t ldx) {
  if (!h) return ISDF_ERR_ARG;
  ARG_CHECK(h, d_fac && d_X && P > 0 && n > 0 && ldx >= n && n < 2147483647LL && ldx < 2147483647LL);
  int rc = tri_left(h, false, P, n, d_fac, P, d_X, ldx);
  if (rc) return rc;
  return tri_left(h, true, P, n, d_fac, P, d_X, ldx);
}

extern "C" int isdf_bj_probe_vectors(isdf_handle h, double* d_T, int n, const double* d_fac, const double* d_D, int P,
                                     int nblk, const int32_t* blk_off) {
  if (!h) return ISDF_ERR_ARG;
  ARG_CHECK(h, d_T && d_fac && d_D && n > 0 && P > 0);
  int rc = isdf_block_solve(h, d_D, P, nblk, blk_off, 1, 1, d_T, n, P);
  if (rc) return rc;
  rc = tri_right(h, true, P, n, d_fac, P, d_T, P);
  if (rc) return rc;
  return tri_right(h, false, P, n, d_fac, P, d_T, P);
}

extern "C" int isdf_rows_combine(isdf_handle h, const double* d_E, int n, int64_t ldE, int rows, const double* d_Y,
                                 int64_t ng, int64_t ldy, double* d_F, int64_t ldf, int accumulate) {
  if (!h) return ISDF_ERR_ARG;
  ARG_CHECK(h, d_E && d_Y && d_F && n > 0 && rows > 0 && ng > 0 && ldE >= rows && ldy >= ng && ldf >= ng);
  if (n > 8) return gemm_rm(h, 'N', 'N', n, ng, rows, 1.0, d_E, ldE, d_Y, ldy, accumulate ? 1.0 : 0.0, d_F, ldf);
  ProfScope ps(h, "skinny_rows_kernel[byte]", 8.0 * (double)rows * (double)ng);
  hipLaunchKernelGGL(skinny_rows_kernel, dim3((unsigned)cdiv(ng, 256)), dim3(256), 0, h->stream, d_E, n, rows, ldE, d_Y, ldy,
                     ng, d_F, ldf, accumulate ? 1 : 0);
  KERNEL_CHECK(h);
  return ISDF_OK;
}

extern "C" int isdf_bj_probe_rows(isdf_handle h, double* d_T, int n, const double* d_fac, const double* d_D, int P,
                                  int nblk, const int32_t* blk_off, const double* d_Yp, int64_t ng, int64_t ldy,
                                  double* d_F, int64_t ldf) {
  if (!h) return ISDF_ERR_ARG;
// ... 183 lines not shown
```

pyscf_isdf_amd/csrc/handle.hip:

```cpp
#include "common.h"
#include <cstdarg>

int isdf_fail(isdf_handle h, int code, const char* fmt, ...) {
  char buf[1024];
  va_list ap;
  va_start(ap, fmt);
  vsnprintf(buf, sizeof(buf), fmt, ap);
  va_end(ap);
  if (h) h->err = buf;
  else fprintf(stderr, "mi355_isdf: %s\n", buf);
  return code;
}

void* isdf_ws(isdf_handle h, const char* name, size_t bytes) {
  auto& slot = h->ws[name];
  if (slot.second >= bytes && slot.first) return slot.first;
  if (slot.first) {
    (void)hipStreamSynchronize(h->stream);
    (void)hipFree(slot.first);
    slot.first = nullptr;
    slot.second = 0;
  }
  void* p = nullptr;
  hipError_t e = hipMalloc(&p, bytes ? bytes : 8);
// ... 6 lines not shown
  slot.second = bytes;
  return p;
}

int isdf_get_plan(isdf_handle h, const int32_t mesh[3], int batch, FftPlan** out) {
  std::vector<int> key = {mesh[0], mesh[1], mesh[2], batch};
  auto it = h->plans.find(key);
  if (it != h->plans.end()) {
    *out = &it->second;
    return ISDF_OK;
  }
  FftPlan p;
  int dims[3] = {mesh[0], mesh[1], mesh[2]};
  int64_t G = (int64_t)mesh[0] * mesh[1] * mesh[2];
  int64_t Gc = (int64_t)mesh[0] * mesh[1] * (mesh[2] / 2 + 1);
  ARG_CHECK(h, G < (int64_t)2147483647);
  FFT_TRY(h, hipfftPlanMany(&p.fwd, 3, dims, nullptr, 1, (int)G, nullptr, 1, (int)Gc, HIPFFT_D2Z, batch));
  hipfftResult r2 = hipfftPlanMany(&p.bwd, 3, dims, nullptr, 1, (int)Gc, nullptr, 1, (int)G, HIPFFT_Z2D, batch);
  if (r2 == HIPFFT_SUCCESS) r2 = hipfftSetStream(p.fwd, h->stream);
  if (r2 == HIPFFT_SUCCESS) r2 = hipfftSetStream(p.bwd, h->stream);
  if (r2 != HIPFFT_SUCCESS) {
    (void)hipfftDestroy(p.fwd);
    if (p.bwd) (void)hipfftDestroy(p.bwd);
    return isdf_fail(h, ISDF_ERR_LIB, "hipFFT plan (%d x %d x %d, batch %d) failed: result %d", mesh[0], mesh[1], mesh[2], batch,
                     (int)r2);
  }
  auto res = h->plans.emplace(key, p);
  *out = &res.first->second;
  return ISDF_OK;
}

extern "C" {

int isdf_abi_version(void) { return 21; }

int isdf_set_coulomb_omega(isdf_handle h, double omega) {
  if (!h) return ISDF_ERR_ARG;
  h->coul_omega = omega;
  return ISDF_OK;
}

int isdf_set_coulomb_cutoff(isdf_handle h, double rc) {
  if (!h) return ISDF_ERR_ARG;
  ARG_CHECK(h, rc >= 0.0);
  h->coul_rc = rc;
  return ISDF_OK;
}

int isdf_set_coulomb_ws(isdf_handle h, double alpha, const double ak[9], const int32_t mesh[3], const double maxq[3],
                        const double* d_vq) {
  if (!h) return ISDF_ERR_ARG;
  if (alpha <= 0.0) { h->wsk = WsKernel(); return ISDF_OK; }
  ARG_CHECK(h, ak && mesh && maxq && d_vq && mesh[0] > 0 && mesh[1] > 0 && mesh[2] > 0);
  h->wsk.alpha = alpha;
  for (int i = 0; i < 9; ++i) h->wsk.ak[i] = ak[i];
  for (int i = 0; i < 3; ++i) { h->wsk.mesh[i] = mesh[i]; h->wsk.maxq[i] = maxq[i]; }
  h->wsk.vq = d_vq;
  return ISDF_OK;
}

int isdf_set_option(isdf_handle h, const char* key, int value) {
  if (!h) return ISDF_ERR_ARG;
  ARG_CHECK(h, key != nullptr);
  if (std::string(key) == "trsm_substitution") { h->trsm_substitution = value ? 1 : 0; return ISDF_OK; }
  if (std::string(key) == "own_fft") { h->own_fft = value < 0 ? 0 : (value > 2 ? 2 : value); return ISDF_OK; }
  if (std::string(key) == "gemm_nn_own") { h->gemm_nn_own = value ? 1 : 0; return ISDF_OK; }
  if (std::string(key) == "coul_sphere") { h->coul_sphere = value < 0 ? 0 : value; return ISDF_OK; }
  if (std::string(key) == "conv_pipe") { h->conv_pipe = value != 0; return ISDF_OK; }
  if (std::string(key) == "conv_sub_rows") { h->conv_sub_rows = value < 0 ? 0 : value; return ISDF_OK; }
  if (std::string(key) == "gram_pivot_tpb") {
    if (value != 64 && value != 128 && value != 256) return ISDF_ERR_ARG;
    h->gram_pivot_tpb = value;
    return ISDF_OK;
  }
  if (std::string(key) == "cand_gram") { h->cand_gram = value ? 1 : 0; return ISDF_OK; }
  if (std::string(key) == "gram_compact") { h->gram_compact = value ? 1 : 0; return ISDF_OK; }
  if (std::string(key) == "gram_compact_permille") {
    if (value < 1 || value > 1000) return isdf_fail(h, ISDF_ERR_ARG, "isdf_set_option: gram_compact_permille %d not in [1, 1000]", value);
    h->gram_compact_permille = value;
    return ISDF_OK;
  }
  if (std::string(key) == "block_apply_waves") { h->block_apply_waves = value < 1 ? 1 : value; return ISDF_OK; }
  if (std::string(key) == "block_apply_reg") { h->block_apply_reg = value ? 1 : 0; return ISDF_OK; }
  return isdf_fail(h, ISDF_ERR_ARG, "isdf_set_option: unknown key '%s'", key);
}

int isdf_create(int device_id, isdf_handle* out) {
  if (!out) return ISDF_ERR_ARG;
  *out = nullptr;
  int ndev = 0;
  hipError_t e = hipGetDeviceCount(&ndev);
  if (e != hipSuccess || ndev == 0)
    return isdf_fail(nullptr, ISDF_ERR_HIP, "no HIP device visible (%s)", hipGetErrorString(e));
  if (device_id < 0 || device_id >= ndev)
    return isdf_fail(nullptr, ISDF_ERR_ARG, "device %d out of range (%d devices)", device_id, ndev);
  isdf_ctx* h = new isdf_ctx();
  h->device = device_id;
  if (hipSetDevice(device_id) != hipSuccess) { delete h; return ISDF_ERR_HIP; }
  hipDeviceProp_t prop;
  if (hipGetDeviceProperties(&prop, device_id) == hipSuccess) h->num_cu = prop.multiProcessorCount;
  if (rocblas_create_handle(&h->blas) != rocblas_status_success) {
    delete h;
    return isdf_fail(nullptr, ISDF_ERR_LIB, "rocblas_create_handle failed");
  }
  rocblas_set_pointer_mode(h->blas, rocblas_pointer_mode_host);
  *out = h;
  return ISDF_OK;
}

int isdf_release_workspace(isdf_handle h) {
  if (!h) return ISDF_ERR_ARG;
  (void)hipStreamSynchronize(h->stream);
  for (auto& kv : h->ws)
    if (kv.second.first) (void)hipFree(kv.second.first);
  h->ws.clear();
  for (auto& kv : h->plans) {
    if (kv.second.fwd) hipfftDestroy(kv.second.fwd);
    if (kv.second.bwd) hipfftDestroy(kv.second.bwd);
  }
  h->plans.clear();
  return ISDF_OK;
}

int isdf_destroy(isdf_handle h) {
  if (!h) return ISDF_OK;
  isdf_prof_reset(h);
  isdf_release_workspace(h);
  if (h->blas) rocblas_destroy_handle(h->blas);
  delete h;
  return ISDF_OK;
}

int isdf_set_stream(isdf_handle h, void* hip_stream) {
  if (!h) return ISDF_ERR_ARG;
  h->stream = (hipStream_t)hip_stream;
  BLAS_TRY(h, rocblas_set_stream(h->blas, h->stream));
  for (auto& kv : h->plans) {
    if (kv.second.fwd) FFT_TRY(h, hipfftSetStream(kv.second.fwd, h->stream));
    if (kv.second.bwd) FFT_TRY(h, hipfftSetStream(kv.second.bwd, h->stream));
  }
  return ISDF_OK;
}

const char* isdf_last_error(isdf_handle h) { return h ? h->err.c_str() : "null handle"; }

int isdf_prof_enable(isdf_handle h, int on) {
  if (!h) return ISDF_ERR_ARG;
  h->profiling = on ? 1 : 0;
  return ISDF_OK;
}

int isdf_prof_reset(isdf_handle h) {
  if (!h) return ISDF_ERR_ARG;
  (void)hipStreamSynchronize(h->stream);
  for (auto& kv : h->prof)
    for (auto& r : kv.second.recs) { (void)hipEventDestroy(r.e0); (void)hipEventDestroy(r.e1); }
  h->prof.clear();
  return ISDF_OK;
}

int isdf_prof_count(isdf_handle h) { return h ? (int)h->prof.size() : 0; }

int isdf_prof_get(isdf_handle h, int index, char* name, int name_cap, int64_t* launches, double* total_ms,
                  double* total_work) {
  if (!h || index < 0 || index >= (int)h->prof.size()) return ISDF_ERR_ARG;
  auto it = h->prof.begin();
// ... 23 lines not shown
```

pyscf_isdf_amd/csrc/trsm.hip:

```cpp
#include "common.h"
#include <cstdlib>

namespace {

constexpr int SB = 64;

template <bool TRANS>
__global__ __launch_bounds__(256) void subst_kernel(const double* __restrict__ L, int64_t ldl, int nb,
                                                    double* __restrict__ X, int64_t ldx, int64_t n) {
  const int64_t c = (int64_t)blockIdx.x * 256 + threadIdx.x;
  if (c >= n) return;
  double x[SB];
#pragma unroll
  for (int i = 0; i < SB; ++i) x[i] = (i < nb) ? X[(int64_t)i * ldx + c] : 0.0;
  if (!TRANS) {
#pragma unroll
    for (int i = 0; i < SB; ++i) {
      if (i < nb) {
        double s = x[i];
#pragma unroll
        for (int k = 0; k < i; ++k) s = fma(-L[(int64_t)i * ldl + k], x[k], s);
        x[i] = s / L[(int64_t)i * ldl + i];
      }
    }
  } else {
#pragma unroll
    for (int i = SB - 1; i >= 0; --i) {
      if (i < nb) {
        double s = x[i];
#pragma unroll
        for (int k = i + 1; k < SB; ++k)
          if (k < nb) s = fma(-L[(int64_t)k * ldl + i], x[k], s);
        x[i] = s / L[(int64_t)i * ldl + i];
      }
    }
  }
#pragma unroll
  for (int i = 0; i < SB; ++i)
    if (i < nb) X[(int64_t)i * ldx + c] = x[i];
}

__global__ void transpose_kernel(const double* __restrict__ src, int64_t lds, int64_t rows, int64_t cols,
                                 double* __restrict__ dst, int64_t ldd) {
  __shared__ double tile[32][33];
  const int64_t r0 = (int64_t)blockIdx.y * 32, c0 = (int64_t)blockIdx.x * 32;
  const int tx = threadIdx.x, ty = threadIdx.y;
  for (int i = ty; i < 32; i += 8) {
    const int64_t r = r0 + i, c = c0 + tx;
    tile[i][tx] = (r < rows && c < cols) ? src[r * lds + c] : 0.0;
  }
  __syncthreads();
  for (int i = ty; i < 32; i += 8) {
    const int64_t r = c0 + i, c = r0 + tx;
    if (r < cols && c < rows) dst[r * ldd + c] = tile[tx][i];
  }
}

__global__ __launch_bounds__(256) void block_forward_kernel(const double* __restrict__ D, int64_t ldd,
                                                            const int32_t* __restrict__ blk_off,
                                                            double* __restrict__ X, int64_t ldx, int64_t n) {
  const int b = blockIdx.y;
  const int off = blk_off[b], m = blk_off[b + 1] - off;
  if (m <= 0) return;
  const int64_t c = (int64_t)blockIdx.x * 256 + threadIdx.x;
  if (c >= n) return;
  const double* Db = D + (int64_t)off * ldd + off;
  double* Xb = X + (int64_t)off * ldx + c;
  const int nsub = (m + 63) >> 6;
  double x[SB];
  for (int j = 0; j < nsub; ++j) {
    const int nbj = min(SB, m - j * SB);
    const double* Lj = Db + (int64_t)(j * SB) * ldd;
#pragma unroll
    for (int q = 0; q < SB; ++q) x[q] = (q < nbj) ? Xb[(int64_t)(j * SB + q) * ldx] : 0.0;
    for (int r0 = 0; r0 < j * SB; r0 += 8) {
      double v[8];
#pragma unroll
      for (int t = 0; t < 8; ++t) v[t] = Xb[(int64_t)(r0 + t) * ldx];
#pragma unroll
      for (int q = 0; q < SB; ++q) {
        if (q < nbj) {
          const double* Lq = Lj + (int64_t)q * ldd + r0;
#pragma unroll
          for (int t = 0; t < 8; ++t) x[q] = fma(-Lq[t], v[t], x[q]);
        }
      }
    }
    const double* Ld = Lj + j * SB;
#pragma unroll
    for (int q = 0; q < SB; ++q) {
      if (q < nbj) {
        double s_ = x[q];
#pragma unroll
        for (int k = 0; k < q; ++k) s_ = fma(-Ld[(int64_t)q * ldd + k], x[k], s_);
        x[q] = s_ / Ld[(int64_t)q * ldd + q];
      }
    }
#pragma unroll
    for (int q = 0; q < SB; ++q)
      if (q < nbj) Xb[(int64_t)(j * SB + q) * ldx] = x[q];
  }
}

int subst(isdf_handle h, bool trans, const double* L, int64_t ldl, int nb, double* X, int64_t ldx, int64_t n) {
  ProfScope ps(h, trans ? "trsm_subst_kernel<true>[flop]" : "trsm_subst_kernel<false>[flop]", (double)nb * nb * (double)n);
  const dim3 grid((unsigned)cdiv(n, 256));
  if (trans) hipLaunchKernelGGL(subst_kernel<true>, grid, dim3(256), 0, h->stream, L, ldl, nb, X, ldx, n);
  else hipLaunchKernelGGL(subst_kernel<false>, grid, dim3(256), 0, h->stream, L, ldl, nb, X, ldx, n);
  KERNEL_CHECK(h);
  return ISDF_OK;
}

}

typedef double d4v __attribute__((ext_vector_type(4)));
template <int TN, bool SQ>
__global__ __launch_bounds__(256) void block_apply_mfma_kernel(const double* __restrict__ Dinv, int64_t ldd,
                                                               const int32_t* __restrict__ blk_off, double* __restrict__ X,
                                                               int64_t ldx, int64_t n) {
  extern __shared__ double sB[];
  constexpr int LDB = TN + 2;
  const int b = blockIdx.y;
  const int off = blk_off[b], m = blk_off[b + 1] - off;
  if (m <= 0) return;
  const int mpad = (m + 31) & ~31;
  const int64_t c0 = (int64_t)blockIdx.x * TN;
  const int ncol = (int)min((int64_t)TN, n - c0);
  double* Xb = X + (int64_t)off * ldx + c0;
  for (int idx = threadIdx.x; idx < mpad * TN; idx += 256) {
    const int r = idx / TN, c = idx - r * TN;
    double v = (r < m && c < ncol) ? Xb[(int64_t)r * ldx + c] : 0.0;
    if (SQ) v = v * v;
    sB[r * LDB + c] = v;
  }
  __syncthreads();
  const int wave = threadIdx.x >> 6, lane = threadIdx.x & 63;
  const int fr = lane & 15, fk = lane >> 4;
  for (int rt = wave; rt < (m + 15) / 16; rt += 4) {
    d4v acc[TN / 16];
#pragma unroll
    for (int ct = 0; ct < TN / 16; ++ct) acc[ct] = (d4v){0.0, 0.0, 0.0, 0.0};
    const int arow = rt * 16 + fr;
    const bool rowok = arow < m;
    const double* pa = Dinv + (int64_t)(off + (rowok ? arow : 0)) * ldd + off + 8 * fk;
    const double* pb = sB + (8 * fk) * LDB + fr;
    const int kend = min(mpad, ((rt + 1) * 16 + 31) & ~31);
    double a_cur[8], a_nxt[8];
#pragma unroll
    for (int j = 0; j < 8; ++j) a_cur[j] = (rowok && 8 * fk + j < m) ? pa[j] : 0.0;
    for (int k0 = 0; k0 < kend; k0 += 32) {
      if (k0 + 32 < kend) {
#pragma unroll
        for (int j = 0; j < 8; ++j) a_nxt[j] = (rowok && k0 + 32 + 8 * fk + j < m) ? pa[k0 + 32 + j] : 0.0;
      }
#pragma unroll
      for (int j = 0; j < 8; ++j)
#pragma unroll
        for (int ct = 0; ct < TN / 16; ++ct)
          acc[ct] = __builtin_amdgcn_mfma_f64_16x16x4f64(a_cur[j], pb[(k0 + j) * LDB + ct * 16], acc[ct], 0, 0, 0);
#pragma unroll
      for (int j = 0; j < 8; ++j) a_cur[j] = a_nxt[j];
    }
#pragma unroll
    for (int ct = 0; ct < TN / 16; ++ct)
#pragma unroll
      for (int r = 0; r < 4; ++r) {
        const int row = rt * 16 + fk + 4 * r, col = ct * 16 + fr;
        if (row < m && col < ncol) Xb[(int64_t)row * ldx + col] = acc[ct][r];
      }
  }
}

template <int NT, int NCT, bool SQ>
__global__ __launch_bounds__(64 * ((NT + 1) / 2)) __attribute__((amdgpu_waves_per_eu(1, 2))) void block_apply_reg_kernel(const double* __restrict__ Dinv, int64_t ldd,
                                                                            const int32_t* __restrict__ blk_off,
                                                                            double* __restrict__ X, int64_t ldx, int64_t n) {
  constexpr int TN = 16 * NCT;
  constexpr int LDB = TN + 2;
  constexpr int NPAIR = (NT + 1) / 2;
  constexpr int NTHREADS = 64 * NPAIR;
  constexpr int NCH = NT / 2 + 1;
  constexpr int MP = 16 * NT;
  constexpr int NPRE = (MP * TN + NTHREADS - 1) / NTHREADS;
  extern __shared__ double sB[];
  const int b = blockIdx.y;
  const int off = blk_off[b], m = blk_off[b + 1] - off;
  if (m <= 0) return;
  const int pair = threadIdx.x >> 6, lane = threadIdx.x & 63;
  const int fr = lane & 15, fk = lane >> 4;
  const int tA = pair, tB = NT - 1 - pair;
  const int nchA = (tA + 2) / 2, nchB = (tB == tA) ? 0 : (tB + 2) / 2;
  double a[8 * NCH];
#pragma unroll
  for (int c = 0; c < NCH; ++c) {
    const bool isA = c < nchA;
    const int t = isA ? tA : tB;
    const int k0 = 32 * (isA ? c : c - nchA) + 8 * fk;
    const int row = t * 16 + fr;
    const bool live = (c < nchA + nchB) && row < m;
    const double* pa = Dinv + (int64_t)(off + (live ? row : 0)) * ldd + off + k0;
#pragma unroll
    for (int j = 0; j < 8; ++j) a[8 * c + j] = (live && k0 + j < m) ? pa[j] : 0.0;
  }
  const int64_t ntile = (n + TN - 1) / TN;
  double pre[NPRE];
  const int r0 = threadIdx.x / TN, cc = threadIdx.x % TN;
  constexpr int RSTEP = NTHREADS / TN;
  double* const Xrow = X + (int64_t)(off + r0) * ldx + cc;
  auto fetch = [&](int64_t tile) {
    const int64_t c0 = tile * TN;
    const bool colok = c0 + cc < n;
#pragma unroll
    for (int i = 0; i < NPRE; ++i) {
      const int r = r0 + i * RSTEP;
      pre[i] = (r < m && colok) ? Xrow[(int64_t)i * RSTEP * ldx + c0] : 0.0;
    }
  };
  int64_t tile = blockIdx.x;
  if (tile < ntile) fetch(tile);
  for (; tile < ntile; tile += gridDim.x) {
#pragma unroll
    for (int i = 0; i < NPRE; ++i) {
      const int r = r0 + i * RSTEP;
      if (r < MP) {
        const double v = pre[i];
        sB[r * LDB + cc] = SQ ? v * v : v;
      }
    }
    __syncthreads();
    if (tile + gridDim.x < ntile) fetch(tile + gridDim.x);
    const int64_t c0 = tile * TN;
#pragma unroll
    for (int ct = 0; ct < NCT; ++ct) {
      d4v accA = (d4v){0.0, 0.0, 0.0, 0.0}, accB = (d4v){0.0, 0.0, 0.0, 0.0};
      const double* pb = sB + (8 * fk) * LDB + 16 * ct + fr;
#pragma unroll
      for (int c = 0; c < NCH; ++c) {
        if (c < nchA) {
          const double* q = pb + (32 * c) * LDB;
#pragma unroll
          for (int j = 0; j < 8; ++j) accA = __builtin_amdgcn_mfma_f64_16x16x4f64(a[8 * c + j], q[j * LDB], accA, 0, 0, 0);
        } else if (c < nchA + nchB) {
          const double* q = pb + (32 * (c - nchA)) * LDB;
#pragma unroll
          for (int j = 0; j < 8; ++j) accB = __builtin_amdgcn_mfma_f64_16x16x4f64(a[8 * c + j], q[j * LDB], accB, 0, 0, 0);
        }
        __builtin_amdgcn_sched_barrier(0);
      }
      const int64_t col = c0 + ct * 16 + fr;
      if (col < n) {
        double* Xb = X + (int64_t)off * ldx + col;
#pragma unroll
        for (int r = 0; r < 4; ++r) {
          const int rowA = tA * 16 + fk + 4 * r;
          if (rowA < m) Xb[(int64_t)rowA * ldx] = accA[r];
          if (nchB > 0) {
            const int rowB = tB * 16 + fk + 4 * r;
            if (rowB < m) Xb[(int64_t)rowB * ldx] = accB[r];
          }
        }
      }
    }
    __syncthreads();
  }
}

template <int NT, int NCT>
static int block_apply_reg_launch(isdf_handle h, const double* Dinv, int64_t ldd, int nblk, const int32_t* d_off, double* X,
                                  int64_t ldx, int64_t n, bool sq) {
  constexpr int TN = 16 * NCT;
  constexpr int NTHREADS = 64 * ((NT + 1) / 2);
  static_assert(NTHREADS % TN == 0 && (16 * NT * TN) % NTHREADS == 0, "tile elements must divide evenly over the threads");
  const size_t lds = (size_t)16 * NT * (TN + 2) * sizeof(double);
  const int64_t ntile = (n + TN - 1) / TN;
  const unsigned gx = (unsigned)std::max<int64_t>(1, std::min<int64_t>(ntile, ((int64_t)h->num_cu * h->block_apply_waves + nblk - 1) / nblk));
  if (sq) {
    if (lds > 64 * 1024)
      HIP_TRY(h, hipFuncSetAttribute((const void*)&block_apply_reg_kernel<NT, NCT, true>, hipFuncAttributeMaxDynamicSharedMemorySize, 160 * 1024));
    hipLaunchKernelGGL(HIP_KERNEL_NAME(block_apply_reg_kernel<NT, NCT, true>), dim3(gx, (unsigned)nblk), dim3(NTHREADS), lds, h->stream,
                       Dinv, ldd, d_off, X, ldx, n);
  } else {
    if (lds > 64 * 1024)
      HIP_TRY(h, hipFuncSetAttribute((const void*)&block_apply_reg_kernel<NT, NCT, false>, hipFuncAttributeMaxDynamicSharedMemorySize, 160 * 1024));
    hipLaunchKernelGGL(HIP_KERNEL_NAME(block_apply_reg_kernel<NT, NCT, false>), dim3(gx, (unsigned)nblk), dim3(NTHREADS), lds, h->stream,
                       Dinv, ldd, d_off, X, ldx, n);
  }
  KERNEL_CHECK(h);
  return ISDF_OK;
}

template <int TN, bool SQ>
static hipError_t block_apply_lds_attr() {
  return hipFuncSetAttribute((const void*)&block_apply_mfma_kernel<TN, SQ>, hipFuncAttributeMaxDynamicSharedMemorySize, 160 * 1024);
}

int block_apply_inverse(isdf_handle h, const double* Dinv, int64_t ldd, int nblk, const int32_t* blk_off_host, double* X,
                        int64_t ldx, int64_t n, bool square_input) {
  ARG_CHECK(h, Dinv && X && blk_off_host && nblk > 0 && n > 0 && nblk <= 65535);
  int mmax = 0;
  for (int b = 0; b < nblk; ++b) mmax = std::max(mmax, blk_off_host[b + 1] - blk_off_host[b]);
  const int mpad = (mmax + 31) & ~31;
  ARG_CHECK(h, mmax > 0);
  const bool reg = h->block_apply_reg && mmax <= 256;
  const int nt = (mmax + 15) / 16;
  int tn = 0;
  const char* label;
  if (reg) {
    label = nt <= 8 ? "block_apply_reg_kernel<8,2>[byte]" : nt <= 10 ? "block_apply_reg_kernel<10,2>[byte]"
          : nt <= 12 ? "block_apply_reg_kernel<12,2>[byte]" : "block_apply_reg_kernel<16,1>[byte]";
  } else if ((size_t)mpad * (64 + 2) * sizeof(double) <= 52 * 1024) {
    tn = 64; label = "block_apply_mfma_kernel<64>[byte]";
  } else if ((size_t)mpad * (32 + 2) * sizeof(double) <= 80 * 1024) {
    tn = 32; label = "block_apply_mfma_kernel<32>[byte]";
  } else {
    ARG_CHECK(h, (size_t)mpad * (16 + 2) * sizeof(double) <= 160 * 1024);
    tn = 16; label = "block_apply_mfma_kernel<16>[byte]";
  }
  int32_t* d_off = (int32_t*)isdf_ws(h, "trsm_blk_off", sizeof(int32_t) * (size_t)(nblk + 1));
  if (!d_off) return ISDF_ERR_HIP;
  HIP_TRY(h, hipMemcpyAsync(d_off, blk_off_host, sizeof(int32_t) * (size_t)(nblk + 1), hipMemcpyHostToDevice, h->stream));
  ProfScope ps(h, label, 16.0 * (double)blk_off_host[nblk] * (double)n);
  if (reg) {
    if (nt <= 8) return block_apply_reg_launch<8, 2>(h, Dinv, ldd, nblk, d_off, X, ldx, n, square_input);
    if (nt <= 10) return block_apply_reg_launch<10, 2>(h, Dinv, ldd, nblk, d_off, X, ldx, n, square_input);
    if (nt <= 12) return block_apply_reg_launch<12, 2>(h, Dinv, ldd, nblk, d_off, X, ldx, n, square_input);
    return block_apply_reg_launch<16, 1>(h, Dinv, ldd, nblk, d_off, X, ldx, n, square_input);
  }
#define ISDF_BA_LAUNCH(TN_, SQ_)                                                                                       \
  do {                                                                                                                 \
    if ((size_t)mpad * (TN_ + 2) * sizeof(double) > 64 * 1024) {                                                       \
      HIP_TRY(h, (block_apply_lds_attr<TN_, SQ_>()));                                                                  \
    }                                                                                                                  \
    hipLaunchKernelGGL(HIP_KERNEL_NAME(block_apply_mfma_kernel<TN_, SQ_>), dim3((unsigned)cdiv(n, TN_), (unsigned)nblk),   \
                       dim3(256), (size_t)mpad * (TN_ + 2) * sizeof(double), h->stream, Dinv, ldd, d_off, X, ldx, n);  \
  } while (0)
  if (tn == 64) {
    if (square_input) ISDF_BA_LAUNCH(64, true); else ISDF_BA_LAUNCH(64, false);
  } else if (tn == 32) {
    if (square_input) ISDF_BA_LAUNCH(32, true); else ISDF_BA_LAUNCH(32, false);
  } else {
    if (square_input) ISDF_BA_LAUNCH(16, true); else ISDF_BA_LAUNCH(16, false);
  }
#undef ISDF_BA_LAUNCH
  KERNEL_CHECK(h);
  return ISDF_OK;
}

int block_forward_solve(isdf_handle h, const double* D, int64_t ldd, int nblk, const int32_t* blk_off_host, double* X,
                        int64_t ldx, int64_t n) {
  ARG_CHECK(h, D && X && blk_off_host && nblk > 0 && n > 0 && nblk <= 65535);
  int32_t* d_off = (int32_t*)isdf_ws(h, "trsm_blk_off", sizeof(int32_t) * (size_t)(nblk + 1));
  if (!d_off) return ISDF_ERR_HIP;
  HIP_TRY(h, hipMemcpyAsync(d_off, blk_off_host, sizeof(int32_t) * (size_t)(nblk + 1), hipMemcpyHostToDevice, h->stream));
  double rows2 = 0.0;
  for (int b = 0; b < nblk; ++b) rows2 += (double)(blk_off_host[b + 1] - blk_off_host[b]) * (blk_off_host[b + 1] - blk_off_host[b]);
  ProfScope ps(h, "block_forward_kernel[byte]", 16.0 * (double)blk_off_host[nblk] * (double)n);
  (void)rows2;
  hipLaunchKernelGGL(block_forward_kernel, dim3((unsigned)cdiv(n, 256), (unsigned)nblk), dim3(256), 0, h->stream, D, ldd, d_off,
                     X, ldx, n);
  KERNEL_CHECK(h);
  return ISDF_OK;
}

int transpose_rm(isdf_handle h, const double* src, int64_t lds, int64_t rows, int64_t cols, double* dst, int64_t ldd) {
  ARG_CHECK(h, src && dst && rows > 0 && cols > 0 && lds >= cols && ldd >= rows);
  hipLaunchKernelGGL(transpose_kernel, dim3((unsigned)cdiv(cols, 32), (unsigned)cdiv(rows, 32)), dim3(32, 8), 0, h->stream,
                     src, lds, rows, cols, dst, ldd);
  KERNEL_CHECK(h);
  return ISDF_OK;
}

int trsm_lower_left(isdf_handle h, bool trans, int m, int64_t n, const double* L, int64_t ldl, double* X, int64_t ldx) {
  ARG_CHECK(h, L && X && m > 0 && n > 0 && ldl >= m && ldx >= n);
  const int PB = 512;
  int rc;
  if (!trans) {
    for (int r0 = 0; r0 < m; r0 += PB) {
      const int r1 = std::min(m, r0 + PB);
      if (r0 > 0) {
        rc = gemm_rm(h, 'N', 'N', r1 - r0, n, r0, -1.0, L + (int64_t)r0 * ldl, ldl, X, ldx, 1.0, X + (int64_t)r0 * ldx, ldx);
        if (rc) return rc;
      }
      for (int s0 = r0; s0 < r1; s0 += SB) {
        const int s1 = std::min(r1, s0 + SB);
        if (s0 > r0) {
          rc = gemm_rm(h, 'N', 'N', s1 - s0, n, s0 - r0, -1.0, L + (int64_t)s0 * ldl + r0, ldl, X + (int64_t)r0 * ldx, ldx,
                       1.0, X + (int64_t)s0 * ldx, ldx);
          if (rc) return rc;
        }
        rc = subst(h, false, L + (int64_t)s0 * ldl + s0, ldl, s1 - s0, X + (int64_t)s0 * ldx, ldx, n);
        if (rc) return rc;
      }
    }
  } else {
    const int npan = (int)cdiv(m, PB);
    for (int p = npan - 1; p >= 0; --p) {
      const int r0 = p * PB, r1 = std::min(m, r0 + PB);
      if (r1 < m) {
        rc = gemm_rm(h, 'T', 'N', r1 - r0, n, m - r1, -1.0, L + (int64_t)r1 * ldl + r0, ldl, X + (int64_t)r1 * ldx, ldx, 1.0,
                     X + (int64_t)r0 * ldx, ldx);
        if (rc) return rc;
      }
      const int nsb = (int)cdiv(r1 - r0, SB);
      for (int q = nsb - 1; q >= 0; --q) {
        const int s0 = r0 + q * SB, s1 = std::min(r1, s0 + SB);
        if (s1 < r1) {
          rc = gemm_rm(h, 'T', 'N', s1 - s0, n, r1 - s1, -1.0, L + (int64_t)s1 * ldl + s0, ldl, X + (int64_t)s1 * ldx, ldx,
                       1.0, X + (int64_t)s0 * ldx, ldx);
          if (rc) return rc;
        }
        rc = subst(h, true, L + (int64_t)s0 * ldl + s0, ldl, s1 - s0, X + (int64_t)s0 * ldx, ldx, n);
        if (rc) return rc;
      }
    }
  }
  return ISDF_OK;
}

int trsm_lower_right(isdf_handle h, bool trans, int m, int64_t n, const double* L, int64_t ldl, double* X, int64_t ldx) {
  ARG_CHECK(h, L && X && m > 0 && n > 0 && ldl >= m && ldx >= m);
  double* T = (double*)isdf_ws(h, "trsm_T", sizeof(double) * (size_t)m * (size_t)n);
  if (!T) return ISDF_ERR_HIP;
  int rc = transpose_rm(h, X, ldx, n, m, T, n);
  if (rc) return rc;
  rc = trsm_lower_left(h, !trans, m, n, L, ldl, T, n);
  if (rc) return rc;
  return transpose_rm(h, T, n, m, n, X, ldx);
}

namespace {
int trsm_block_size() {
  static const int nb = getenv("ISDF_TRSM_NB") ? std::max(64, atoi(getenv("ISDF_TRSM_NB"))) : 1024;
  return nb;
}
int rb_left(isdf_handle h, bool trans, int m, int64_t n, const double* L, int64_t ldl, double* X, int64_t ldx) {
  const double one = 1.0;
  ProfScope ps(h, "rocblas_dtrsm[flop]", (double)n * m * m);
  BLAS_TRY(h, rocblas_dtrsm(h->blas, rocblas_side_right, rocblas_fill_upper,
                            trans ? rocblas_operation_transpose : rocblas_operation_none, rocblas_diagonal_non_unit,
                            (rocblas_int)n, m, &one, L, (rocblas_int)ldl, X, (rocblas_int)ldx));
  return ISDF_OK;
}
// ... 73 lines not shown
```

pyscf_isdf_amd/fit_route.py:

```python
import numpy as np


class FitRouteMixin:
    def _bj_prepare(self, ao, nh, d_ip, ip_off, aoP, scratch=None):
        be = self.backend
        P = aoP.shape[0]
        be.gather_aoP(ao, d_ip, aoP)
        A = self._buffer('factor', (P, P))
        if getattr(self, '_psi', None) is not None and not nh:
            be.gram_prod(aoP, self._psiP, A)
        else:
            be.gram_sq(aoP, A, nh)
        self._Dinv_key = None
        be.shift_diag(A, self.reg_rel)
        Dblk = self._buffer('Dblk', (P, P))
        self.block_shift_used = be.block_chol(A, ip_off, self.block_shift, Dblk)
        be.block_solve(Dblk, ip_off, 0, 0, A)
        be.block_solve(Dblk, ip_off, 1, 1, A)
        extra = be.chol_inplace(A, 0.0, scratch=scratch)
        self.reg_used = self.reg_rel + extra
        return A, Dblk

    def _block_inverse(self, Dblk, ip_off):
        if not self.block_apply_mfma or int(np.diff(np.asarray(ip_off)).max()) > 1100:
            return None
        key = (Dblk.data_ptr(), getattr(self, '_build_serial', 0), len(ip_off))
        if getattr(self, '_Dinv_key', None) != key:
            Dinv = self._buffer('Dinv', tuple(Dblk.shape))
            self.backend.block_invert(Dblk, ip_off, Dinv)
            self._Dinv, self._Dinv_key = Dinv, key
        return self._Dinv

    def _bj_rows(self, aoP, nh, ao, ng, Dblk, ip_off, out):
        be = self.backend
        Dinv = self._block_inverse(Dblk, ip_off)
        if getattr(self, '_psi', None) is not None and not nh:
            be.pair_prod_rows(aoP, self._psiP, ao, self._psi, ng, out)
            if Dinv is not None:
                be.block_apply(Dinv, ip_off, out)
            else:
                be.block_solve(Dblk, ip_off, 0, 0, out)
            return
        if Dinv is not None and not nh:
            be.pair_rows_block_apply(aoP, ao, ng, Dinv, ip_off, out)
            return
        be.pair_gram_rows(aoP, ao, ng, out, nh)
        if Dinv is not None:
            be.block_apply(Dinv, ip_off, out)
        else:
            be.block_solve(Dblk, ip_off, 0, 0, out)

    def _resident_rows(self, G, P):
        if self.max_resident_rows:
            return int(self.max_resident_rows), int(self.max_resident_rows)
        be = self.backend
        have = be.free_bytes() + sum(int(b.numel()) * 8 for k, b in self._bufs.items() if k in ('theta', 'W', 'factor', 'Dblk', 'Dinv', 'rows_scratch'))
        if self.max_device_memory:
            have = min(have, int(self.max_device_memory) - sum(int(b.numel()) * 8 for k, b in self._bufs.items() if k in ('ao', 'psi')))
        fixed = 4 * 8 * P * P + (3 << 30)
        if getattr(self, 'pair_space', 'ao') == 'occ':
            nocc = min(self.cell.nao_nr() // 2, int(getattr(self.cell, 'nelectron', 0)) // 2 + 8)
            fixed += 8 * G * nocc + (2 << 30)
        fb = int(self.fft_batch or 0)
        single = (have - fixed - 24 * (min(128, fb) if fb else 128) * G) // (8 * G)
        panel = (have - fixed - 40 * (fb or 512) * G) // (8 * G)
        return max(0, int(single)), max(0, int(panel))

    def _panel_plan(self, ip_off, nrows_max):
        ip_off = np.asarray(ip_off, dtype=np.int64)
        P = int(ip_off[-1])
        big = int(np.diff(ip_off).max())
        if nrows_max < big:
            raise MemoryError('ISDF: not enough device memory for one block of %d fit rows' % big)
        npan = max(1, -(-P // int(nrows_max)))
        while True:
            cuts = [P]
            for k in range(npan - 1):
                want = max(cuts[-1] - int(nrows_max), 0)
                i0 = int(np.searchsorted(ip_off, want, side='left'))
                cand = [int(x) for x in ip_off[i0:] if x < cuts[-1] and x < want + 768]
                if not cand:
                    break
                b = min(cand, key=lambda x: ((-x) % 256, x)) if want > 0 else 0
# ... 27 lines not shown

    def _finish_W_paneled(self, W, probe=None):
        be, st = self.backend, self._fit_state
        cell = self.cell
        P = W.shape[0]
        mesh = np.asarray(self.mesh, dtype=np.int32)
        G = int(np.prod(mesh))
        a = np.asarray(cell.lattice_vectors(), dtype=float)
        w = cell.vol / G
        ip_off = np.asarray(st['ip_off'], dtype=np.int64)
        panels = st['panels']
        buf = st['rows']
        nbat = int(self.fft_batch or 512)
        big = int(np.diff(ip_off).max())
        self._last_fft_batch = nbat
        scratch = self._buffer('rows_scratch', (nbat + big, G))
        for q, (q0, q1) in enumerate(panels):
            Yq = buf[:q1 - q0]
            self._bj_rows_range(q0, q1, Yq)
            be.coulomb_W(Yq, mesh, a, 0, q1 - q0, min(nbat, q1 - q0), W[q0:q1, q0:q1], upper_only=True)
            if probe is not None:
                be.rows_combine(probe[0][:, q0:q1], Yq, probe[1], accumulate=q > 0)
            for p0, p1 in panels[:q]:
                nxt, fill, g0 = p0, 0, p0
                while nxt < p1 or fill > 0:
                    while fill < nbat and nxt < p1:
                        i = int(np.searchsorted(ip_off, nxt))
                        j = i + 1
                        while j + 1 < len(ip_off) and ip_off[j + 1] <= p1 and fill + (ip_off[j + 1] - nxt) <= nbat + big:
                            j += 1
                        b1 = int(ip_off[j])
                        self._bj_rows_range(nxt, b1, scratch[fill:fill + (b1 - nxt)])
                        fill += b1 - nxt
                        nxt = b1
                    take = min(nbat, fill)
                    V = scratch[:take]
                    be.coulomb_rows(V, mesh, a, take)
                    be.gemm_nt(V, Yq, W[g0:g0 + take, q0:q1], alpha=w)
                    if fill > take:
                        scratch[:fill - take].copy_(scratch[take:fill].clone() if fill - take > take else scratch[take:fill])
                    g0 += take
                    fill -= take
        be.symmetrize_upper(W)
        self._bj_finish(st['Afac'], st['Dblk'], st['ip_off'], W)

    def _spectral_plan(self):
        be = self.backend
        if not getattr(self, 'w_spectral', False) or not hasattr(be, 'spectral_rows'):
            return None
        mesh = np.asarray(self.mesh, dtype=np.int32)
        epoch = getattr(be, 'kernel_epoch', None)
        ckey = (tuple(int(x) for x in mesh), epoch, str(getattr(self, 'w_sphere', 'auto')), float(getattr(self, 'w_sphere_tol', 0.0)),
                int(self.fft_batch or 512), int(getattr(self, 'w_sort_bins', 0) or 0))
        cached = getattr(self, '_spectral_plan_cache', None)
        if epoch is not None and cached is not None and cached[0] == ckey:
            return cached[1]
        plan = self._spectral_plan_make(mesh)
        self._spectral_plan_cache = (ckey, plan)
        return plan

    def _spectral_plan_make(self, mesh):
        be = self.backend
        if not be.spectral_supported(mesh, int(self.fft_batch or 512)):
            return None
        a = np.asarray(self.cell.lattice_vectors(), dtype=float)
        G = int(np.prod(mesh))
        cg = be.coulG_half(mesh, a)
        if (cg < 0).any():
            return None
        w = self.cell.vol / G

        def share(pct, mult, box, keep):
            key = (tuple(int(x) for x in mesh), round(float(pct), 6))
            if getattr(self, '_sphere_share', (None,))[0] != key:
                self._sphere_share = (key, self._sphere_energy_share(mesh, cg, mult, box, keep, w))
            return self._sphere_share[1]
        pts = self._spectral_point_set(mesh, cg > 0, share)
        if pts is None:
            return None
        idx, mult = pts
        scale = np.sqrt(mult.ravel()[idx] * w * cg.ravel()[idx])
        npts = len(idx)
        ldx = -(-2 * npts // 128) * 128
        return dict(idx=be.to_device(idx), scale=be.to_device(scale), npts=npts, ldx=ldx, fraction=2.0 * npts / G)

    def _spectral_point_set(self, mesh, box, share):
        a = np.asarray(self.cell.lattice_vectors(), dtype=float)
        n0, n1, n2 = (int(x) for x in mesh)
        n2h = n2 // 2 + 1
        keep = box.copy()
        pct = getattr(self, 'w_sphere', 'auto')
        auto = isinstance(pct, str)
        pct = 100.0 if auto else float(pct or 0.0)
        if pct > 0:
            b = 2 * np.pi * np.linalg.inv(a).T
            f0, f1, f2 = np.fft.fftfreq(n0, 1.0 / n0), np.fft.fftfreq(n1, 1.0 / n1), np.arange(n2h, dtype=float)
            Gv = f0[:, None, None, None] * b[0] + f1[None, :, None, None] * b[1] + f2[None, None, :, None] * b[2]
            g2 = np.einsum('xyzc,xyzc->xyz', Gv, Gv)
            rmin = min(2 * np.pi * ((int(n) - 1) // 2) / np.linalg.norm(a[i]) for i, n in enumerate(mesh)) * pct / 100.0
            keep &= g2 <= rmin * rmin * (1 + 1e-12)
        mult = np.full((n0, n1, n2h), 2.0)
        mult[:, :, 0] = 1.0
        if n2 % 2 == 0:
            mult[:, :, n2 // 2] = 1.0
        if auto:
            if not (share(pct, mult, box, keep) <= float(getattr(self, 'w_sphere_tol', 1e-11))):
                return None
        idx = np.flatnonzero(keep.ravel()).astype(np.int32)
        if len(idx) == 0:
            return None
        nbins = int(getattr(self, 'w_sort_bins', 0) or 0)
        if nbins > 0:
            b = 2 * np.pi * np.linalg.inv(a).T
            f0, f1, f2 = np.fft.fftfreq(n0, 1.0 / n0), np.fft.fftfreq(n1, 1.0 / n1), np.arange(n2h, dtype=float)
            Gv = f0[:, None, None, None] * b[0] + f1[None, :, None, None] * b[1] + f2[None, None, :, None] * b[2]
            g2p = np.einsum('xyzc,xyzc->xyz', Gv, Gv).ravel()[idx]
            bins = np.minimum((g2p * (nbins / g2p.max())).astype(np.int64), nbins - 1)
            idx = idx[np.argsort(-bins, kind='stable')]
        return idx, mult

    def _sphere_energy_share(self, mesh, cg, mult, box, keep, w, ntest=8):
        import torch
        be = self.backend
        ao = getattr(self, 'ao', None)
        if ao is None:
            return np.inf
        nao, G = ao.shape
        rng = np.random.default_rng(7)
        cd = be.to_device(rng.standard_normal((2 * ntest, nao)) / np.sqrt(nao))
        rows = be.empty((2 * ntest, G))
        be.gemm_nn(cd, ao, rows)
        t = rows[:ntest].contiguous()
        be.hadamard_rows(t, rows[ntest:].contiguous())
        Gfull = int(np.prod(mesh))
        if G != Gfull:
            g0, g1 = self._slice
            full = be.zeros((ntest, Gfull))
            full[:, g0:g1] = t
            self.comm.all_reduce_sum(full)
            t = full
        idx = np.flatnonzero(box.ravel()).astype(np.int32)
        scale = np.sqrt(mult.ravel()[idx] * w * cg.ravel()[idx])
        ldx = -(-2 * len(idx) // 128) * 128
        X = be.empty((ntest, ldx))
        be.spectral_rows(t, mesh, be.to_device(idx), be.to_device(scale), X, batch=ntest)
        x = be.to_host(X)[:, :2 * len(idx)]
        e = x[:, 0::2] ** 2 + x[:, 1::2] ** 2
        outside = ~keep.ravel()[idx]
        tot = e.sum(axis=1)
        return float((e[:, outside].sum(axis=1) / np.where(tot > 0, tot, 1.0)).max())

    def _finish_W_spectral(self, W, probe=None):
        be, st = self.backend, self._fit_state
        plan = self._spectral_plan()
        ip_off = np.asarray(st['ip_off'], dtype=np.int64)
        P = W.shape[0]
        mesh = np.asarray(self.mesh, dtype=np.int32)
        G = int(np.prod(mesh))
        if plan is None:
            rows_avail = int(self._bufs['theta'].numel() // G)
            st2 = dict(st, kind='blockjacobi-paneled', rows=self._buffer('theta', (rows_avail, G)),
                       panels=self._panel_plan(ip_off, rows_avail))
            self._fit_state = st2
            try:
                return self._finish_W_paneled(W, probe=probe)
            finally:
                self._fit_state = st
        nbat = int(self.fft_batch or 512)
        big = int(np.diff(ip_off).max())
        self._last_fft_batch = nbat
        ldx = plan['ldx']
        X = self._buffer('theta', (P, ldx))
        piece = self._pair_rows_piece(big)
        scratch = self._buffer('rows_scratch', (nbat + big, G))
        self.w_spectral_fraction = plan['fraction']
        self._last_spectral_ldx = ldx
        if piece:
            self._spectral_rows_two_frontiers(X, scratch, piece, plan, probe)
            return self._spectral_W_finish(X, W, nbat)
        nxt, fill, g0 = 0, 0, 0
        while nxt < P or fill > 0:
            while fill < nbat and nxt < P:
                i = int(np.searchsorted(ip_off, nxt))
                j = i + 1
                while j + 1 < len(ip_off) and fill + (ip_off[j + 1] - nxt) <= nbat + big:
                    j += 1
                b1 = int(ip_off[j])
                self._bj_rows_range(nxt, b1, scratch[fill:fill + (b1 - nxt)])
                fill += b1 - nxt
                nxt = b1
            take = min(nbat, fill)
            rows = scratch[:take]
            if probe is not None:
                be.rows_combine(probe[0][:, g0:g0 + take], rows, probe[1], accumulate=g0 > 0)
            be.spectral_rows(rows, mesh, plan['idx'], plan['scale'], X[g0:g0 + take], batch=take)
            if fill > take:
                scratch[:fill - take].copy_(scratch[take:fill].clone() if fill - take > take else scratch[take:fill])
            g0 += take
            fill -= take
        self._spectral_W_finish(X, W, nbat)

    def _spectral_W_finish(self, X, W, nbat):
        be, st = self.backend, self._fit_state
        P = W.shape[0]
        for b0 in range(0, P, nbat):
            b1 = min(P, b0 + nbat)
            be.gemm_nt(X[b0:b1], X[b0:], W[b0:b1, b0:], alpha=1.0)
        be.symmetrize_upper(W)
        self._bj_finish(st['Afac'], st['Dblk'], st['ip_off'], W)

    def _pair_rows_piece(self, big):
        align = int(getattr(self, 'pair_rows_align', 0) or 0)
        if align <= 0 or not hasattr(self.backend, 'pair_rows_frontier') or getattr(self, '_psi', None) is not None \
                or not self.block_apply_mfma or big > 1100:
            return 0
        return int(self.fft_batch or 512) // align * align

    def _spectral_rows_two_frontiers(self, X, scratch, piece, plan, probe):
        be, st = self.backend, self._fit_state
        ip_off = np.asarray(st['ip_off'], dtype=np.int64)
        P = int(ip_off[-1])
        mesh = np.asarray(self.mesh, dtype=np.int32)
        G = self.ao.shape[1]
        Dinv = self._block_inverse(st['Dblk'], ip_off)
        nbat = int(self.fft_batch or 512)
        squared = be.pair_rows_squared(self.aoP, min(piece, P), self.ao, G)
        app, prod = 0, 0
        while app < P:
            new = min(piece, P - prod)
            j = int(np.searchsorted(ip_off, prod + new, side='right')) - 1
            i = int(np.searchsorted(ip_off, app))
            end = int(ip_off[j])
            be.pair_rows_frontier(self.aoP[prod:prod + new], self.ao, G, squared, Dinv[app:, app:],
                                  (ip_off[i:j + 1] - app).astype(np.int32), scratch, prod - app)
            prod += new
            if end > app:
                rows = scratch[:end - app]
                if probe is not None:
                    be.rows_combine(probe[0][:, app:end], rows, probe[1], accumulate=app > 0)
                be.spectral_rows(rows, mesh, plan['idx'], plan['scale'], X[app:end], batch=min(nbat, end - app))
                tail = prod - end
                if tail > 0:
                    src = scratch[end - app:prod - app]
                    scratch[:tail].copy_(src.clone() if tail > end - app else src)
                app = end

    def _bj_finish(self, Afac, Dblk, ip_off, W, antisymmetric=False):
        be = self.backend
        be.W_from_factor(Afac, 2, W)
        be.W_from_factor(Afac, 0, W)
        be.block_solve(Dblk, ip_off, 0, 1, W)
        be.block_solve(Dblk, ip_off, 1, 0, W)
        be.symmetrize_mean(W, antisymmetric)

    def _bj_clusters(self):
        cell = self.cell
        natm = cell.natm
        parent = list(range(natm))

        def find(i):
            while parent[i] != i:
                parent[i] = parent[parent[i]]
                i = parent[i]
            return i
        r = float(self.bj_cluster_radius or 0.0)
        if r > 0 and natm > 1:
            a = np.asarray(cell.lattice_vectors(), dtype=float)
            frac = np.asarray(cell.atom_coords(), dtype=float).dot(np.linalg.inv(a))
            d = frac[:, None, :] - frac[None, :, :]
            d -= np.round(d)
            dist = np.linalg.norm(d.dot(a), axis=2)
            for i, j in zip(*np.nonzero(np.triu(dist < r, 1))):
                ri, rj = find(int(i)), find(int(j))
                if ri != rj:
                    parent[max(ri, rj)] = min(ri, rj)
        groups = {}
        for i in range(natm):
            groups.setdefault(find(i), []).append(i)
        return [groups[k] for k in sorted(groups)]

    def _bj_blocks(self, counts, clusters):
        per = [int(sum(counts[b] for b in cl)) for cl in clusters]
        off = np.append(0, np.cumsum(per)).astype(np.int32)
        g = max(1, int(self.bj_group))
        if g > 1:
            off = np.unique(np.append(off[::g], off[-1])).astype(np.int32)
        return off

    def _fit_routes(self):
        if self.fit_route not in ('auto', 'blockjacobi', 'cholesky'):
            raise ValueError("fit_route must be 'auto', 'blockjacobi' or 'cholesky'")
        if self._want_theta or self.fit_route == 'cholesky':
            return ['cholesky']
        if self.fit_route == 'blockjacobi':
            return ['blockjacobi']
        if self.c_isdf > self.bj_max_c:
            return ['cholesky']
        return ['blockjacobi', 'cholesky']

    def _bj_probe_densities(self, aoT_P):
        be = self.backend
        planes = aoT_P if isinstance(aoT_P, (list, tuple)) else [aoT_P]
        nao, P = planes[0].shape
        n = int(self.bj_nprobe)
        if getattr(self, '_psi', None) is not None and len(planes) == 1:
            psiP = self._psiP
            nocc = psiP.shape[1]
            cached = getattr(self, '_probe_Rocc', None)
            if cached is None or cached[0] != (n, nao, nocc):
                rng = np.random.default_rng(20240203)
                self._probe_Rocc = ((n, nao, nocc), be.to_device(rng.standard_normal((n, nao, nocc))))
            d_R = self._probe_Rocc[1]
            aoP = planes[0].T.contiguous()
            ones = be.to_device(np.ones((nocc, 1)))
            T = be.empty((n, P))
            tmp = be.empty((P, nocc))
            col = be.empty((P, 1))
            for j in range(n):
                be.gemm_nn(aoP, d_R[j], tmp)
                be.hadamard_rows(tmp, psiP)
                be.gemm_nn(tmp, ones, col)
                T[j].copy_(col[:, 0])
            return T
# ... 55 lines not shown
```

pyscf_isdf_amd/lib.py:

```python
import ctypes
import os

_HERE = os.path.dirname(os.path.abspath(__file__))
LIB_PATH = os.path.join(_HERE, 'lib', 'libmi355_isdf.so')
ABI_VERSION = 21

_lib = None

c_int, c_i64, c_dbl, c_vp = ctypes.c_int, ctypes.c_int64, ctypes.c_double, ctypes.c_void_p

SIGNATURES = {
    'isdf_abi_version': (c_int, []),
    'isdf_create': (c_int, [c_int, ctypes.POINTER(c_vp)]),
    'isdf_destroy': (c_int, [c_vp]),
    'isdf_set_stream': (c_int, [c_vp, c_vp]),
    'isdf_last_error': (ctypes.c_char_p, [c_vp]),
    'isdf_workspace_bytes': (c_i64, [c_vp]),
    'isdf_set_coulomb_omega': (c_int, [c_vp, c_dbl]),
    'isdf_set_coulomb_cutoff': (c_int, [c_vp, c_dbl]),
    'isdf_set_coulomb_ws': (c_int, [c_vp, c_dbl, c_vp, c_vp, c_vp, c_vp]),
    'isdf_set_option': (c_int, [c_vp, ctypes.c_char_p, c_int]),
    'isdf_release_workspace': (c_int, [c_vp]),
    'isdf_prof_enable': (c_int, [c_vp, c_int]),
    'isdf_prof_reset': (c_int, [c_vp]),
    'isdf_prof_count': (c_int, [c_vp]),
    'isdf_prof_get': (c_int, [c_vp, c_int, ctypes.c_char_p, c_int, ctypes.POINTER(c_i64), ctypes.POINTER(c_dbl), ctypes.POINTER(c_dbl)]),
    'isdf_eval_ao': (c_int, [c_vp, c_vp, c_int, c_vp, c_int, c_vp, c_int, c_vp, c_int, c_vp, c_vp, c_i64, c_vp, c_i64]),
    'isdf_block_row_absmax': (c_int, [c_vp, c_vp, c_int, c_i64, c_int, c_vp, c_vp]),
    'isdf_gather_cols': (c_int, [c_vp, c_vp, c_int, c_i64, c_vp, c_i64, c_vp, c_i64]),
    'isdf_partition_by_atom': (c_int, [c_vp, c_vp, c_i64, c_vp, c_int, c_vp, c_dbl, c_vp]),
    'isdf_select_ip': (c_int, [c_vp, c_vp, c_int, c_i64, c_int, c_vp, c_vp, c_dbl, c_dbl, c_vp, c_i64, c_vp, c_vp]),
    'isdf_select_ip_ws': (c_int, [c_vp, c_vp, c_int, c_i64, c_int, c_vp, c_vp, c_dbl, c_dbl, c_vp, c_i64, c_vp, c_vp, c_vp,
                                  c_i64]),
    'isdf_select_ip_work_bytes': (c_i64, [c_int, c_i64]),
    'isdf_select_ip_gram': (c_int, [c_vp, c_vp, c_int, c_i64, c_int, c_dbl, c_dbl, c_int, c_vp, ctypes.POINTER(ctypes.c_int32)]),
    'isdf_fit_from_chol': (c_int, [c_vp, c_vp, c_int, c_i64, c_i64, c_vp]),
    'isdf_fit_prepare': (c_int, [c_vp, c_vp, c_int, c_i64, c_vp, c_int, c_dbl, c_vp, c_vp, ctypes.POINTER(c_dbl)]),
    'isdf_fit_apply': (c_int, [c_vp, c_vp, c_vp, c_int, c_int, c_vp, c_i64, c_i64, c_int, c_vp, c_i64]),
    'isdf_gather_aoP': (c_int, [c_vp, c_vp, c_int, c_i64, c_vp, c_int, c_vp]),
    'isdf_gram_sq': (c_int, [c_vp, c_vp, c_int, c_int, c_int, c_vp]),
    'isdf_pair_gram_rows': (c_int, [c_vp, c_vp, c_int, c_int, c_int, c_vp, c_i64, c_i64, c_vp, c_i64]),
    'isdf_gram_prod': (c_int, [c_vp, c_vp, c_int, c_int, c_vp, c_int, c_vp]),
    'isdf_pair_prod_rows': (c_int, [c_vp, c_vp, c_int, c_int, c_vp, c_int, c_vp, c_i64, c_vp, c_i64, c_i64, c_vp, c_i64]),
    'isdf_factor_solve_half': (c_int, [c_vp, c_vp, c_int, c_int, c_vp, c_i64, c_i64]),
    'isdf_gram_prod_cplx': (c_int, [c_vp, c_vp, c_int, c_int, c_int, c_vp, c_int, c_int, c_vp]),
    'isdf_pair_prod_rows_cplx': (c_int, [c_vp, c_vp, c_int, c_int, c_int, c_vp, c_int, c_int, c_vp, c_i64, c_vp, c_i64, c_i64,
                                         c_vp, c_i64]),
    'isdf_block_chol': (c_int, [c_vp, c_vp, c_int, c_int, c_vp, c_dbl, c_vp, ctypes.POINTER(c_dbl)]),
    'isdf_block_solve': (c_int, [c_vp, c_vp, c_int, c_int, c_vp, c_int, c_int, c_vp, c_i64, c_i64]),
    'isdf_block_invert': (c_int, [c_vp, c_vp, c_int, c_int, c_vp, c_vp]),
    'isdf_block_apply': (c_int, [c_vp, c_vp, c_i64, c_int, c_vp, c_vp, c_i64, c_i64]),
    'isdf_pair_rows_block_apply': (c_int, [c_vp, c_vp, c_int, c_int, c_vp, c_i64, c_i64, c_vp, c_i64, c_int, c_vp, c_vp, c_i64]),
    'isdf_pair_rows_squared': (c_int, [c_vp, c_vp, c_int, c_int, c_vp, c_i64, c_i64, ctypes.POINTER(c_int)]),
    'isdf_pair_rows_frontier': (c_int, [c_vp, c_vp, c_int, c_int, c_vp, c_i64, c_i64, c_int, c_vp, c_i64, c_int, c_vp, c_vp, c_i64,
                                        c_int]),
    'isdf_shift_diag': (c_int, [c_vp, c_vp, c_int, c_dbl]),
    'isdf_chol_inplace': (c_int, [c_vp, c_vp, c_int, c_dbl, c_vp, ctypes.POINTER(c_dbl)]),
    'isdf_factor_solve': (c_int, [c_vp, c_vp, c_int, c_vp, c_i64, c_i64]),
    'isdf_bj_probe_vectors': (c_int, [c_vp, c_vp, c_int, c_vp, c_vp, c_int, c_int, c_vp]),
    'isdf_rows_combine': (c_int, [c_vp, c_vp, c_int, c_i64, c_int, c_vp, c_i64, c_i64, c_vp, c_i64, c_int]),
    'isdf_bj_probe_rows': (c_int, [c_vp, c_vp, c_int, c_vp, c_vp, c_int, c_int, c_vp, c_vp, c_i64, c_i64, c_vp, c_i64]),
    'isdf_gather_T': (c_int, [c_vp, c_vp, c_int, c_i64, c_vp, c_vp]),
    'isdf_W_from_factor': (c_int, [c_vp, c_vp, c_int, c_int, c_vp, c_i64]),
    'isdf_fit_global': (c_int, [c_vp, c_vp, c_int, c_i64, c_i64, c_vp, c_int, c_dbl, c_vp, c_i64, c_vp, ctypes.POINTER(c_dbl)]),
    'isdf_coulomb_W': (c_int, [c_vp, c_vp, c_int, c_i64, c_vp, c_vp, c_int, c_int, c_int, c_int, c_vp, c_i64]),
    'isdf_coulomb_rows': (c_int, [c_vp, c_vp, c_int, c_i64, c_vp, c_vp, c_int, c_vp, c_i64]),
    'isdf_symmetrize_upper': (c_int, [c_vp, c_vp, c_int, c_i64]),
    'isdf_symmetrize_mean': (c_int, [c_vp, c_vp, c_int, c_i64, c_int]),
    'isdf_get_j': (c_int, [c_vp, c_vp, c_int, c_i64, c_i64, c_vp, c_vp, c_vp, c_int, c_vp]),
    'isdf_rho': (c_int, [c_vp, c_vp, c_int, c_i64, c_i64, c_vp, c_int, c_vp, c_i64]),
    'isdf_coulomb_potential': (c_int, [c_vp, c_vp, c_int, c_i64, c_vp, c_vp]),
    'isdf_vj_from_vR': (c_int, [c_vp, c_vp, c_int, c_i64, c_i64, c_vp, c_int, c_i64, c_vp]),
    'isdf_eval_ao_k': (c_int, [c_vp, c_vp, c_int, c_vp, c_int, c_vp, c_int, c_vp, c_int, c_vp, c_vp, c_int, c_vp, c_i64, c_vp, c_vp, c_i64]),
    'isdf_select_ip_cplx': (c_int, [c_vp, c_vp, c_int, c_int, c_i64, c_int, c_vp, c_vp, c_dbl, c_dbl, c_vp, c_i64, c_vp, c_vp]),
    'isdf_fit_prepare_cplx': (c_int, [c_vp, c_vp, c_int, c_int, c_i64, c_vp, c_int, c_dbl, c_vp, c_vp, ctypes.POINTER(c_dbl)]),
    'isdf_fit_apply_cplx': (c_int, [c_vp, c_vp, c_vp, c_int, c_int, c_int, c_vp, c_i64, c_i64, c_int, c_vp, c_i64]),
    'isdf_coulG_q': (c_int, [c_vp, c_vp, c_vp, c_vp, c_int, c_dbl, c_vp]),
    'isdf_coulomb_Wq': (c_int, [c_vp, c_vp, c_int, c_i64, c_vp, c_vp, c_dbl, c_int, c_int, c_int, c_int, c_vp, c_vp, c_i64]),
    'isdf_symmetrize_hermitian': (c_int, [c_vp, c_vp, c_vp, c_int, c_i64]),
    'isdf_finish_Wq': (c_int, [c_vp, c_vp, c_vp, c_int, c_i64, c_vp, c_vp]),
    'isdf_get_k_pair': (c_int, [c_vp, c_vp, c_vp, c_vp, c_vp, c_int, c_int, c_dbl, c_vp]),
    'isdf_get_k_exact_kpt': (c_int, [c_vp, c_vp, c_vp, c_int, c_i64, c_vp, c_vp, c_int, c_i64, c_vp, c_vp, c_dbl, c_int, c_int, c_int, c_vp, c_vp]),
    'isdf_coulG_half': (c_int, [c_vp, c_vp, c_vp, c_vp]),
    'isdf_spectral_supported': (c_int, [c_vp, c_vp, c_int, ctypes.POINTER(c_int)]),
    'isdf_spectral_rows': (c_int, [c_vp, c_vp, c_int, c_i64, c_vp, c_vp, c_vp, c_int, c_int, c_vp, c_i64]),
    'isdf_coulomb_rows_q': (c_int, [c_vp, c_vp, c_int, c_i64, c_vp, c_vp, c_vp, c_vp]),
    'isdf_nyquist_spectra': (c_int, [c_vp, c_vp, c_int, c_i64, c_vp, c_int, c_vp, c_vp]),
    'isdf_zhadamard_planes': (c_int, [c_vp, c_vp, c_vp, c_i64, c_vp, c_vp, c_i64, c_int, c_i64]),
    'isdf_rho_k': (c_int, [c_vp, c_vp, c_vp, c_int, c_i64, c_i64, c_vp, c_vp, c_dbl, c_vp]),
    'isdf_vj_k': (c_int, [c_vp, c_vp, c_vp, c_int, c_i64, c_i64, c_vp, c_vp, c_vp]),
    'isdf_pp_local_potential': (c_int, [c_vp, c_int, c_vp, c_vp, c_vp, c_vp, c_vp]),
    'isdf_pp_projector_overlaps': (c_int, [c_vp, c_vp, c_int, c_vp, c_int, c_vp, c_int, c_vp, c_vp, c_vp, c_vp, c_int, c_vp, c_vp, c_vp]),
    'isdf_pp_local_force': (c_int, [c_vp, c_vp, c_int, c_i64, c_int, c_vp, c_vp, c_vp, c_vp, c_vp]),
    'isdf_pp_projector_overlaps_ip': (c_int, [c_vp, c_vp, c_int, c_vp, c_int, c_vp, c_int, c_vp, c_vp, c_vp, c_vp, c_int, c_vp, c_vp,
                                              c_vp]),
    'isdf_rowdot3': (c_int, [c_vp, c_int, c_i64, c_dbl, c_vp, c_i64, c_i64, c_vp, c_vp, c_i64, c_int, c_vp, c_i64]),
    'isdf_gemm_nn': (c_int, [c_vp, c_int, c_i64, c_int, c_dbl, c_vp, c_i64, c_vp, c_i64, c_dbl, c_vp, c_i64]),
    'isdf_hadamard_rows': (c_int, [c_vp, c_vp, c_i64, c_vp, c_i64, c_int, c_i64]),
    'isdf_eval_ao_deriv1': (c_int, [c_vp, c_vp, c_int, c_vp, c_int, c_vp, c_int, c_vp, c_int, c_vp, c_vp, c_i64, c_vp, c_i64, c_i64]),
    'isdf_eval_ao_deriv2': (c_int, [c_vp, c_vp, c_int, c_vp, c_int, c_vp, c_int, c_vp, c_int, c_vp, c_vp, c_i64, c_vp, c_i64, c_i64]),
    'isdf_gga_aow': (c_int, [c_vp, c_int, c_i64, c_vp, c_i64, c_i64, c_vp, c_i64, c_vp, c_i64, c_vp, c_i64, c_i64]),
    'isdf_eval_ao_k_deriv1': (c_int, [c_vp, c_vp, c_int, c_vp, c_int, c_vp, c_int, c_vp, c_int, c_vp, c_vp, c_int, c_vp, c_i64, c_vp, c_vp, c_i64, c_i64]),
    'isdf_uniform_grid': (c_int, [c_vp, c_vp, c_vp, c_vp]),
    'isdf_rho_pair': (c_int, [c_vp, c_vp, c_int, c_vp, c_int, c_i64, c_i64, c_vp, c_int, c_vp, c_i64]),
    'isdf_mg_embed_density': (c_int, [c_vp, c_vp, c_int, c_vp, c_dbl, c_vp, c_vp, c_int]),
    'isdf_mg_restrict_potential': (c_int, [c_vp, c_vp, c_int, c_vp, c_vp, c_dbl, c_vp]),
    'isdf_mg_coulomb_kernel': (c_int, [c_vp, c_vp, c_int, c_vp, c_vp]),
    'isdf_lda_exchange': (c_int, [c_vp, c_vp, c_i64, c_vp, c_vp]),
    'isdf_lda_vwn_add': (c_int, [c_vp, c_vp, c_i64, c_vp, c_vp]),
    'isdf_gga_b88': (c_int, [c_vp, c_vp, c_vp, c_i64, c_i64, c_vp, c_vp, c_vp, c_i64]),
    'isdf_xc_fused': (c_int, [c_vp, c_vp, c_vp, c_i64, c_i64, c_dbl, c_dbl, c_dbl, c_int, c_dbl, c_vp, c_vp, c_vp, c_i64]),
    'isdf_gga_lyp_polarised': (c_int, [c_vp, c_vp, c_vp, c_i64, c_i64, c_i64, c_dbl, c_int, c_vp, c_vp, c_vp, c_i64, c_i64]),
    'isdf_lda_exchange_fxc': (c_int, [c_vp, c_vp, c_i64, c_vp]),
    'isdf_lda_vwn_fxc_add': (c_int, [c_vp, c_vp, c_i64, c_vp]),
    'isdf_gga_b88_fxc': (c_int, [c_vp, c_vp, c_i64, c_i64, c_vp, c_i64, c_i64, c_int, c_vp, c_i64, c_i64, c_vp, c_i64]),
    'isdf_xc_fxc_apply': (c_int, [c_vp, c_int, c_vp, c_i64, c_i64, c_i64, c_vp, c_i64, c_i64, c_int, c_vp, c_i64, c_i64, c_int]),
    'isdf_dot': (c_int, [c_vp, c_vp, c_vp, c_i64, c_vp]),
    'isdf_gemm_nt': (c_int, [c_vp, c_int, c_int, c_i64, c_dbl, c_vp, c_i64, c_vp, c_i64, c_vp, c_dbl, c_vp, c_i64]),
    'isdf_gemm_nt_had3': (c_int, [c_vp, c_int, c_int, c_i64, c_dbl, c_vp, c_i64, c_vp, c_i64, c_vp, c_i64, c_i64, c_dbl, c_vp, c_i64,
                                  c_i64]),
    'isdf_pack_table_pm': (c_int, [c_vp, c_vp, c_vp, c_vp, c_int, c_dbl, c_vp, c_vp, c_i64]),
    'isdf_herm_kscale_nt': (c_int, [c_vp, c_int, c_int, c_i64, c_dbl, c_vp, c_i64, c_vp, c_i64, c_vp, c_vp, c_dbl, c_vp, c_vp, c_i64]),
    'isdf_get_k_exact': (c_int, [c_vp, c_vp, c_int, c_i64, c_i64, c_vp, c_int, c_vp, c_vp, c_int, c_int, c_int, c_vp]),
    'isdf_get_k': (c_int, [c_vp, c_vp, c_int, c_int, c_vp, c_i64, c_int, c_int, c_vp, c_int, c_vp]),
}


def load():
    global _lib
    if _lib is not None:
        return _lib
    if not os.path.exists(LIB_PATH):
        raise RuntimeError(
            'libmi355_isdf.so not found at %s — build it with `python -c "import __graft_entry__ as g; '
            'g.build()"` or `make -C pyscf_isdf_amd/csrc`.  There is no CPU fallback.' % LIB_PATH)
    try:
        import torch
    except ImportError:
        pass
    lib = ctypes.CDLL(LIB_PATH, mode=ctypes.RTLD_GLOBAL)
    for name, (res, args) in SIGNATURES.items():
        fn = getattr(lib, name)
        fn.restype = res
        fn.argtypes = args
    v = lib.isdf_abi_version()
    if v != ABI_VERSION:
        raise RuntimeError('libmi355_isdf.so ABI version %d != binding version %d' % (v, ABI_VERSION))
    _lib = lib
    return lib


class IsdfError(RuntimeError):
    pass


class Handle:

    def __init__(self, device=0):
        self.lib = load()
        h = c_vp()
        rc = self.lib.isdf_create(int(device), ctypes.byref(h))
        if rc != 0 or not h.value:
            raise IsdfError('isdf_create(device=%d) failed with status %d (no MI355X visible?)' % (device, rc))
        self.h = h
        self.device = device

    def call(self, name, *args):
        rc = getattr(self.lib, name)(self.h, *args)
# ... 15 lines not shown
```

pyscf_isdf_amd/sharded.py:

```python
import time
import warnings
import numpy as np
import torch
from . import gto
from ._common import partition_grid_by_atom, _default_fft_batch


class ShardedMixin:
    def _bj_finish_sharded(self, Afac, Dblk, ip_off, W):
        be, comm = self.backend, self.comm
        P = W.shape[0]
        c0, c1 = comm.split_range(P)
        X = W[:, c0:c1].clone()
        W.zero_()
        if c1 > c0:
            be.factor_solve(Afac, X)
            W[:, c0:c1] = X
        comm.all_reduce_sum(W)
        if c1 > c0:
            X.copy_(W[c0:c1, :].T)
        W.zero_()
        if c1 > c0:
            be.factor_solve(Afac, X)
            be.block_solve(Dblk, ip_off, 0, 1, X)
            W[:, c0:c1] = X
        comm.all_reduce_sum(W)
        del X
        be.block_solve(Dblk, ip_off, 1, 0, W)
        be.symmetrize_mean(W)

    def _build_sharded(self):
        cell, be, comm = self.cell, self.backend, self.comm
        if self.select not in ('local', 'refined'):
            raise NotImplementedError("multi-GPU build needs select='local' or 'refined'")
        R, rk = comm.size, comm.rank
        self.timings = {}
        t0 = time.perf_counter()
        mesh = np.asarray(self.mesh, dtype=np.int32)
        G = int(np.prod(mesh))
        nao = cell.nao_nr()
        a = np.asarray(cell.lattice_vectors(), dtype=float)
        coords = self.grids.coords
        rcut = gto.estimate_rcut_per_shell(cell)
        Ls = gto.get_lattice_Ls(cell, rcut=rcut.max())
        ao_args = (np.asarray(cell._atm), np.asarray(cell._bas), np.asarray(cell._env), Ls, rcut)
        g0, g1 = comm.split_range(G)
        self._slice = (g0, g1)
        ng = g1 - g0
        t0 = self._tick('host_setup', t0)

        self.ao = self._buffer('ao', (nao, ng))
        be.eval_ao(*ao_args, be.to_device(np.ascontiguousarray(coords[g0:g1].T)), self.ao)
        t0 = self._tick('S1_eval_ao', t0)

        owner = be.partition_by_atom(coords, cell.atom_coords(), a)
        perm = np.argsort(owner, kind='stable').astype(np.int64)
        counts = np.bincount(owner, minlength=cell.natm)
        blk_off = np.append(0, np.cumsum(counts)).astype(np.int64)
        nip_final = np.minimum(self.nip_per_atom(), counts).astype(np.int32)
        nip = nip_final
        if self.select == 'refined':
            nip = np.minimum(np.ceil(self.nip_per_atom() * float(self.refine_over)).astype(np.int64), counts).astype(np.int32)
        mine = [b for b in range(cell.natm) if b % R == rk and nip[b] > 0]
        t0 = self._tick('host_partition', t0)
        my_ips = {}
        if mine:
            idx = np.concatenate([perm[blk_off[b]:blk_off[b + 1]] for b in mine])
            loc_off = np.append(0, np.cumsum([counts[b] for b in mine])).astype(np.int64)
            ao_sel = be.empty((nao, len(idx)))
            be.eval_ao(*ao_args, be.to_device(np.ascontiguousarray(coords[idx].T)), ao_sel)
            kmax = int(max(nip[b] for b in mine))
            L = be.empty((kmax, len(idx)))
            piv = be.empty((len(mine), kmax), dtype=torch.int64)
            rank = be.select_ip(ao_sel, loc_off, [nip[b] for b in mine], self.select_tol, self.tie_rtol, L, piv)
            piv_h = be.to_host(piv)
            for k, b in enumerate(mine):
                my_ips[b] = idx[loc_off[k] + piv_h[k, :rank[k]]]
            del ao_sel, L, piv
        all_ips = comm.all_gather_object(my_ips)
        merged = {}
        for d in all_ips:
            merged.update(d)
        self._tick('S2_select_candidates' if self.select == 'refined' else 'S2_select_ip', t0)
        Pmax = int(nip_final.sum())
        need = 8 * Pmax * ng + 4 * 8 * Pmax * Pmax
        have = be.free_bytes() + sum(int(b.numel()) * 8 for k, b in self._bufs.items() if k in ('theta', 'W', 'factor', 'Dblk', 'Dinv'))
        rows_do_not_fit = comm.agree_max(1.0 if need > have else 0.0) > 0.0
        spectral_may = self.w_spectral and not self._want_theta and self.c_isdf <= self.w_spectral_max_c and self.fit_route != 'cholesky'
# ... 240 lines not shown
                    out = exchange_and_convolve(t, t % nslot)
                    staged[t] = (out, be.record_event())
            if t >= 1:
                out, ev = staged.pop(t - 1)
                be.wait_event(ev)
                products(*out)
                consumed[t - 1] = be.record_event()
        del staged, consumed, pieces, full, recvV
        comm.all_reduce_sum(W)
        be.symmetrize_upper(W)
        if st['kind'] == 'blockjacobi':
            self._bj_finish_sharded(st['Afac'], st['Dblk'], st['ip_off'], W)
        elif st['kind'] == 'cholesky':
            be.W_from_factor(st['chol'], 0, W)

    def _finish_W_sharded_spectral(self, W, plan, probe=None):
        cell, be, comm = self.cell, self.backend, self.comm
        st = self._fit_state
        ip_off = np.asarray(st['ip_off'], dtype=np.int64)
        P = int(ip_off[-1])
        ng = self.ao.shape[1]
        R, rk = comm.size, comm.rank
        mesh = np.asarray(self.mesh, dtype=np.int32)
        G = int(np.prod(mesh))
        ldx = int(plan['ldx'])
        self.w_spectral_fraction = plan['fraction']
        self._last_spectral_ldx = ldx
        self._last_fft_batch = int(self.fft_batch or 512)
        slices = [comm.split_range(G, r) for r in range(R)]
        ks = [tuple(16 * x for x in comm.split_range(ldx // 16, r)) for r in range(R)]
        kw = ks[rk][1] - ks[rk][0]
        nbat = int(self.fft_batch or 512)
        big = int(np.diff(ip_off).max())
        nblk = len(ip_off) - 1
        cuts = [int(np.searchsorted(ip_off, P * r / R, side='left')) for r in range(R)] + [nblk]
        cuts = [min(max(c, 0), nblk) for c in cuts]
        plans = []
        for q in range(R):
            b0, b1 = cuts[q], max(cuts[q + 1], cuts[q])
            steps, i = [], b0
            while i < b1:
                j = i + 1
                while j < b1 and ip_off[j + 1] - ip_off[i] <= max(nbat, big):
                    j += 1
                steps.append((int(ip_off[i]), int(ip_off[j])))
                i = j
            plans.append(steps)
        nsteps = max(len(p) for p in plans)
        cap = max([hi - lo for p in plans for lo, hi in p] + [1])
        Xloc = be.empty((P, max(kw, 1)))
        rows_loc = be.empty((R * cap, ng))
        pieces = be.empty((cap * G,))
        full = be.empty((cap, G))
        Xb = be.empty((cap, ldx))
        recvX = be.empty((R * cap * max(kw, 1),))

        def views(flat, nrow_of, width_of):
            out, off = [], 0
            for q in range(R):
                n = nrow_of(q) * width_of(q)
                out.append(flat[off:off + n].view(nrow_of(q), width_of(q)))
                off += n
            return out
        first = True
        for t in range(nsteps):
            bat = [p[t] if t < len(p) else (0, 0) for p in plans]
            nrow = [hi - lo for lo, hi in bat]
            send = []
            for q, (lo, hi) in enumerate(bat):
                blockrows = rows_loc[q * cap:q * cap + (hi - lo)]
                if hi > lo:
                    self._bj_rows_range(lo, hi, blockrows)
                    if probe is not None:
                        be.rows_combine(probe[0][:, lo:hi], blockrows, probe[1], accumulate=not first)
                        first = False
                send.append(blockrows)
            mine = nrow[rk]
            recv = views(pieces, lambda q: mine, lambda q: slices[q][1] - slices[q][0])
            comm.all_to_all(recv, send)
            rows_full = full[:mine]
            for (s0, s1), piece in zip(slices, recv):
                rows_full[:, s0:s1] = piece
            if mine:
                be.spectral_rows(rows_full, mesh, plan['idx'], plan['scale'], Xb[:mine], batch=mine)
            got = views(recvX, lambda q: nrow[q], lambda q: kw)
            comm.all_to_all(got, [Xb[:mine, k0:k1].contiguous() for k0, k1 in ks])
            for q in range(R):
                if nrow[q]:
                    Xloc[bat[q][0]:bat[q][1]] = got[q]
        del pieces, full, Xb, recvX, rows_loc
        W.zero_()
        if kw > 0:
            for b0 in range(0, P, 512):
                b1 = min(P, b0 + 512)
                be.gemm_nt(Xloc[b0:b1], Xloc[b0:], W[b0:b1, b0:], alpha=1.0)
        del Xloc
        comm.all_reduce_sum(W)
        be.symmetrize_upper(W)
        self._bj_finish_sharded(st['Afac'], st['Dblk'], st['ip_off'], W)

    def _keep_V_for_robust_k_sharded(self, t0):
        if not self.robust_k:
            return
        cell, be, comm = self.cell, self.backend, self.comm
        theta = self._fit_state['theta']
        P, ng = theta.shape
        R, rk = comm.size, comm.rank
        mesh = np.asarray(self.mesh, dtype=np.int32)
        G = int(np.prod(mesh))
        a = np.asarray(cell.lattice_vectors(), dtype=float)
        slices = [comm.split_range(G, r) for r in range(R)]
        rows = [comm.split_range(P, r) for r in range(R)]
        nb = self.fft_batch or _default_fft_batch(G, max(1, P // R))
        nsteps = max(-(-(hi - lo) // nb) for lo, hi in rows)
        for t in range(nsteps):
            bat = [(min(lo + t * nb, hi), min(lo + (t + 1) * nb, hi)) for lo, hi in rows]
            nrow = [hi - lo for lo, hi in bat]
            send = [theta[lo:hi] for lo, hi in bat]
            recv = [be.empty((nrow[rk], s1 - s0)) for s0, s1 in slices]
            comm.all_to_all(recv, send)
            full = be.empty((nrow[rk], G))
            for (s0, s1), piece in zip(slices, recv):
                full[:, s0:s1] = piece
            del recv
            if nrow[rk]:
                be.coulomb_rows(full, mesh, a, max(1, nrow[rk]))
            send = [full[:, s0:s1].contiguous() for s0, s1 in slices]
            recv = [be.empty((nrow[q], ng)) for q in range(R)]
            comm.all_to_all(recv, send)
            del full, send
            for q in range(R):
                if nrow[q]:
                    theta[bat[q][0]:bat[q][1]] = recv[q]
            del recv
        self._V = theta
        self._fit_state = None
        self._tick('S5_conv_for_robust_k', t0)

    def _get_jk_sharded(self, d_dm, out_shape, with_j, with_k, exxdiv=None):
        cell, be, comm = self.cell, self.backend, self.comm
        nao = cell.nao_nr()
        nset = d_dm.shape[0]
        mesh = np.asarray(self.mesh, dtype=np.int32)
        G = int(np.prod(mesh))
        a = np.asarray(cell.lattice_vectors(), dtype=float)
        g0, g1 = self._slice
        vj = vk = None
        t0 = time.perf_counter()
        if with_j:
            rho = be.zeros((nset, G))
            rho_loc = be.empty((nset, g1 - g0))
            be.rho(self.ao, g1 - g0, d_dm, rho_loc)
            rho[:, g0:g1] = rho_loc
            comm.all_reduce_sum(rho)
            be.coulomb_potential(rho, mesh, a)
            d_vj = be.empty((nset, nao, nao))
            be.vj_from_vR(self.ao, g1 - g0, rho[:, g0:g1].contiguous(), d_vj)
            comm.all_reduce_sum(d_vj)
            t0 = self._tick('S6_get_j', t0)
            vj = be.to_host(d_vj).reshape(out_shape)
        if with_k:
            P = self.W.shape[0]
            r0, r1 = comm.split_range(P)
            d_vk = be.empty((nset, nao, nao))
            be.get_k(self.aoP, self.W, r0, r1 - r0, d_dm, d_vk)
            comm.all_reduce_sum(d_vk)
            if self.robust_k:
# ... 7 lines not shown
```

Before: 16.94.

## Prune spectral FFT lines via mask, fuse probe into frontier rows, own block invert

Builds a bitmask of the spectral points that are actually kept, so the last strided FFT pass skips tiles and stores that no packed point needs. Adds a fused frontier path that accumulates the probe combine while applying the block inverse, instead of running a separate rows_combine pass. Replaces the block inversion with an identity fill plus a custom block forward-solve kernel. These cut FFT work and memory traffic, but add a mask-building kernel, atomics and extra code paths whose correctness depends on the mask layout.

```diff
diff --git a/include/mi355_isdf.h b/include/mi355_isdf.h
--- a/include/mi355_isdf.h
+++ b/include/mi355_isdf.h
@@ -128,6 +128,10 @@
 int isdf_pair_rows_frontier(isdf_handle h, const double* d_aoP, int nnew, int nao, const double* d_ao, int64_t ng,
                             int64_t ld, int squared, const double* d_Dinv, int64_t ldd, int nblk, const int32_t* blk_off,
                             double* d_B, int64_t ldb, int have);
+int isdf_pair_rows_frontier_probe(isdf_handle h, const double* d_aoP, int nnew, int nao, const double* d_ao, int64_t ng,
+                                  int64_t ld, int squared, const double* d_Dinv, int64_t ldd, int nblk, const int32_t* blk_off,
+                                  double* d_B, int64_t ldb, int have, const double* d_E, int n, int64_t ldE, double* d_F,
+                                  int64_t ldf, int accumulate);
 
 int isdf_gram_prod(isdf_handle h, const double* d_aoP, int P, int nao, const double* d_psiP, int nocc, double* d_A);
 int isdf_pair_prod_rows(isdf_handle h, const double* d_aoP, int P, int nao, const double* d_psiP, int nocc,
@@ -164,6 +168,9 @@
 int isdf_spectral_supported(isdf_handle h, const int32_t mesh[3], int batch, int* ok);
 int isdf_spectral_rows(isdf_handle h, const double* d_in, int nrows, int64_t ld, const int32_t mesh[3], const int32_t* d_idx,
                        const double* d_scale, int npts, int batch, double* d_out, int64_t ldx);
+int isdf_spectral_mask(isdf_handle h, const int32_t* d_idx, int npts, const int32_t mesh[3], int32_t* d_mask);
+int isdf_spectral_rows_masked(isdf_handle h, const double* d_in, int nrows, int64_t ld, const int32_t mesh[3], const int32_t* d_idx,
+                              const double* d_scale, int npts, int batch, double* d_out, int64_t ldx, const int32_t* d_mask);
 int isdf_coulomb_rows(isdf_handle h, const double* d_in, int nrows, int64_t ld,
                       const int32_t mesh[3], const double a[9], int batch, double* d_out, int64_t ldo);
 int isdf_symmetrize_upper(isdf_handle h, double* d_W, int P, int64_t ldw);
diff --git a/pyscf_isdf_amd/backend.py b/pyscf_isdf_amd/backend.py
--- a/pyscf_isdf_amd/backend.py
+++ b/pyscf_isdf_amd/backend.py
@@ -323,15 +323,24 @@
         return bool(sq.value)
 
     def pair_rows_frontier(self, aoP_new, ao, ng, squared, Dinv, blk_off, B, have):
+        self.handle.call('isdf_pair_rows_frontier', *self._frontier_args(aoP_new, ao, ng, squared, Dinv, blk_off, B, have))
+
+    def pair_rows_frontier_probe(self, aoP_new, ao, ng, squared, Dinv, blk_off, B, have, E, F, accumulate=False):
+        blk_off = np.ascontiguousarray(blk_off, dtype=np.int32)
+        assert E.stride(1) == 1 and F.stride(1) == 1 and E.shape[0] == F.shape[0] and E.shape[1] == blk_off[-1] and F.shape[1] >= ng
+        self.handle.call('isdf_pair_rows_frontier_probe', *self._frontier_args(aoP_new, ao, ng, squared, Dinv, blk_off, B, have),
+                         self._p(E), E.shape[0], E.stride(0), self._p(F), F.stride(0), int(bool(accumulate)))
+
+    def _frontier_args(self, aoP_new, ao, ng, squared, Dinv, blk_off, B, have):
         self._stream()
         blk_off = np.ascontiguousarray(blk_off, dtype=np.int32)
         nnew = aoP_new.shape[0]
         assert aoP_new.stride(1) == 1 and aoP_new.stride(0) == aoP_new.shape[1] and B.stride(1) == 1
         assert have + nnew <= B.shape[0] and blk_off[0] == 0 and blk_off[-1] <= have + nnew and B.shape[1] >= ng
         assert len(blk_off) == 1 or (Dinv.shape[0] >= blk_off[-1] and Dinv.shape[1] >= blk_off[-1])
-        self.handle.call('isdf_pair_rows_frontier', self._p(aoP_new) if nnew else None, nnew, aoP_new.shape[1], self._p(ao), int(ng),
-                         ao.stride(0), int(bool(squared)), self._p(Dinv) if len(blk_off) > 1 else None, Dinv.stride(0) if len(blk_off) > 1 else 0,
-                         len(blk_off) - 1, _np_ptr(blk_off), self._p(B), B.stride(0), int(have))
+        return (self._p(aoP_new) if nnew else None, nnew, aoP_new.shape[1], self._p(ao), int(ng),
+                ao.stride(0), int(bool(squared)), self._p(Dinv) if len(blk_off) > 1 else None, Dinv.stride(0) if len(blk_off) > 1 else 0,
+                len(blk_off) - 1, _np_ptr(blk_off), self._p(B), B.stride(0), int(have))
 
     def shift_diag(self, A, shift_rel):
         self._stream()
@@ -415,12 +424,30 @@
         self.handle.call('isdf_coulG_half', _np_ptr(mesh), _np_ptr(a), self._p(out))
         return self.to_host(out).reshape(int(mesh[0]), int(mesh[1]), int(mesh[2]) // 2 + 1)
 
-    def spectral_rows(self, rows, mesh, idx, scale, out, batch=512):
+    def spectral_rows(self, rows, mesh, idx, scale, out, batch=512, mask=None):
         self._stream()
         mesh = np.ascontiguousarray(mesh, dtype=np.int32)
         assert rows.is_contiguous() and out.stride(1) == 1 and idx.dtype == torch.int32 and out.stride(0) % 2 == 0
+        if mask is not None:
+            assert mask.dtype == torch.int32 and mask.is_contiguous() and mask.numel() == self.spectral_mask_words(mesh)
+            self.handle.call('isdf_spectral_rows_masked', self._p(rows), rows.shape[0], rows.stride(0), _np_ptr(mesh), self._p(idx),
+                             self._p(scale), int(idx.numel()), int(batch), self._p(out), out.stride(0), self._p(mask))
+            return
         self.handle.call('isdf_spectral_rows', self._p(rows), rows.shape[0], rows.stride(0), _np_ptr(mesh), self._p(idx),
                          self._p(scale), int(idx.numel()), int(batch), self._p(out), out.stride(0))
+
+    @staticmethod
+    def spectral_mask_words(mesh):
+        n0, n1, n2 = (int(x) for x in mesh)
+        return -(-(n1 * (n2 // 2 + 1)) // 16) * (-(-n0 // 32))
+
+    def spectral_mask(self, idx, mesh):
+        self._stream()
+        mesh = np.ascontiguousarray(mesh, dtype=np.int32)
+        assert idx.dtype == torch.int32 and idx.is_contiguous()
+        mask = torch.empty(self.spectral_mask_words(mesh), dtype=torch.int32, device=idx.device)
+        self.handle.call('isdf_spectral_mask', self._p(idx), int(idx.numel()), _np_ptr(mesh), self._p(mask))
+        return mask
 
     def symmetrize_upper(self, W):
         self._stream()
diff --git a/pyscf_isdf_amd/csrc/common.h b/pyscf_isdf_amd/csrc/common.h
--- a/pyscf_isdf_amd/csrc/common.h
+++ b/pyscf_isdf_amd/csrc/common.h
@@ -56,6 +56,9 @@
   int gram_compact_permille = 875;
   int block_apply_waves = 16;
   int block_apply_reg = 1;
+  int block_invert_own = 1;
+  int spectral_prune = 1;
+  int rows_probe_fused = 1;
   double coul_omega = 0.0;
   double coul_rc = 0.0;
   int coul_sphere = 0;
@@ -70,7 +73,9 @@
 bool conv_rows_q_own_supported(isdf_handle h, const int32_t mesh[3], int nb);
 bool spectral_rows_own_supported(isdf_handle h, const int32_t mesh[3], int nb);
 int spectral_rows_own(isdf_handle h, const double* d_in, int nb, const int32_t mesh[3], const int32_t* d_idx, const double* d_scale,
-                      int npts, double* d_out, int64_t ldx, HIP_vector_type<double, 2u>* zbuf);
+                      int npts, double* d_out, int64_t ldx, HIP_vector_type<double, 2u>* zbuf, const uint32_t* d_mask = nullptr);
+int64_t spectral_mask_words(const int32_t mesh[3]);
+int spectral_mask_own(isdf_handle h, const int32_t* d_idx, int npts, const int32_t mesh[3], uint32_t* d_mask);
 int conv_rows_q_own(isdf_handle h, const double* d_in, double* d_re, double* d_im, int nb, const int32_t mesh[3], const double* tab,
                     double2* zhalf, double2* zfull);
 int conv_rows_own(isdf_handle h, const double* d_in, double* d_out, int nb, const int32_t mesh[3], const double* cg,
@@ -134,8 +139,18 @@
 int trsm_lower_right(isdf_handle h, bool trans, int m, int64_t n, const double* L, int64_t ldl, double* X, int64_t ldx);
 int block_forward_solve(isdf_handle h, const double* D, int64_t ldd, int nblk, const int32_t* blk_off_host, double* X,
                         int64_t ldx, int64_t n);
+struct RowsProbe {
+  const double* E;
+  int n;
+  int64_t ldE;
+  double* F;
+  int64_t ldf;
+  int accumulate;
+};
 int block_apply_inverse(isdf_handle h, const double* Dinv, int64_t ldd, int nblk, const int32_t* blk_off_host, double* X,
-                        int64_t ldx, int64_t n, bool square_input = false);
+                        int64_t ldx, int64_t n, bool square_input = false, const RowsProbe* probe = nullptr);
+int block_forward_solve_own(isdf_handle h, const double* D, int64_t ldd, int nblk, const int32_t* blk_off_host, double* X,
+                            int64_t ldx);
 int transpose_rm(isdf_handle h, const double* src, int64_t lds, int64_t rows, int64_t cols, double* dst, int64_t ldd);
 int tri_left(isdf_handle h, bool trans, int m, int64_t n, const double* L, int64_t ldl, double* X, int64_t ldx);
 int tri_right(isdf_handle h, bool trans, int m, int64_t n, const double* L, int64_t ldl, double* X, int64_t ldx);
diff --git a/pyscf_isdf_amd/csrc/coulomb.hip b/pyscf_isdf_amd/csrc/coulomb.hip
--- a/pyscf_isdf_amd/csrc/coulomb.hip
+++ b/pyscf_isdf_amd/csrc/coulomb.hip
@@ -356,9 +356,8 @@
   return ISDF_OK;
 }
 
-extern "C" int isdf_spectral_rows(isdf_handle h, const double* d_in, int nrows, int64_t ld, const int32_t mesh[3],
-                                  const int32_t* d_idx, const double* d_scale, int npts, int batch, double* d_out, int64_t ldx) {
-  if (!h) return ISDF_ERR_ARG;
+static int spectral_rows(isdf_handle h, const double* d_in, int nrows, int64_t ld, const int32_t mesh[3], const int32_t* d_idx,
+                         const double* d_scale, int npts, int batch, double* d_out, int64_t ldx, const uint32_t* d_mask) {
   ARG_CHECK(h, d_in && d_out && mesh && d_idx && d_scale && nrows >= 0 && batch > 0 && npts > 0);
   const int64_t G = (int64_t)mesh[0] * mesh[1] * mesh[2];
   const int64_t gc = (int64_t)mesh[0] * mesh[1] * (mesh[2] / 2 + 1);
@@ -371,8 +370,29 @@
   if (!Z) return ISDF_ERR_HIP;
   for (int r = 0; r < nrows; r += batch) {
     const int nb = std::min(batch, nrows - r);
-    int rc = spectral_rows_own(h, d_in + (int64_t)r * ld, nb, mesh, d_idx, d_scale, npts, d_out + (int64_t)r * ldx, ldx, Z);
+    int rc = spectral_rows_own(h, d_in + (int64_t)r * ld, nb, mesh, d_idx, d_scale, npts, d_out + (int64_t)r * ldx, ldx, Z, d_mask);
     if (rc) return rc;
   }
   return ISDF_OK;
 }
+
+extern "C" int isdf_spectral_rows(isdf_handle h, const double* d_in, int nrows, int64_t ld, const int32_t mesh[3],
+                                  const int32_t* d_idx, const double* d_scale, int npts, int batch, double* d_out, int64_t ldx) {
+  if (!h) return ISDF_ERR_ARG;
+  return spectral_rows(h, d_in, nrows, ld, mesh, d_idx, d_scale, npts, batch, d_out, ldx, nullptr);
+}
+
+extern "C" int isdf_spectral_rows_masked(isdf_handle h, const double* d_in, int nrows, int64_t ld, const int32_t mesh[3],
+                                         const int32_t* d_idx, const double* d_scale, int npts, int batch, double* d_out,
+                                         int64_t ldx, const int32_t* d_mask) {
+  if (!h) return ISDF_ERR_ARG;
+  ARG_CHECK(h, d_mask);
+  return spectral_rows(h, d_in, nrows, ld, mesh, d_idx, d_scale, npts, batch, d_out, ldx, (const uint32_t*)d_mask);
+}
+
+extern "C" int isdf_spectral_mask(isdf_handle h, const int32_t* d_idx, int npts, const int32_t mesh[3], int32_t* d_mask) {
+  if (!h) return ISDF_ERR_ARG;
+  ARG_CHECK(h, d_idx && d_mask && mesh && npts > 0 && mesh[0] > 0 && mesh[1] > 0 && mesh[2] > 0);
+  ARG_CHECK(h, (int64_t)mesh[0] * mesh[1] * (mesh[2] / 2 + 1) < 2147483647LL);
+  return spectral_mask_own(h, d_idx, npts, mesh, (uint32_t*)d_mask);
+}
diff --git a/pyscf_isdf_amd/csrc/fft_conv.hip b/pyscf_isdf_amd/csrc/fft_conv.hip
--- a/pyscf_isdf_amd/csrc/fft_conv.hip
+++ b/pyscf_isdf_amd/csrc/fft_conv.hip
@@ -494,11 +494,19 @@
   }
 }
 
-template <int MODE, int ZCT>
+template <int MODE, int ZCT, bool MASKED = false>
 __global__ __launch_bounds__(TPB) void strided_fft_fast_kernel(double2* __restrict__ data, int64_t os, int64_t es, int Mtot,
-                                                               Axis ax, int ntile, const double* __restrict__ table) {
+                                                               Axis ax, int ntile, const double* __restrict__ table,
+                                                               const uint32_t* __restrict__ mask = nullptr, int nw = 0) {
   extern __shared__ double2 lds[];
   const int n = ax.n;
+  const uint32_t* mw = nullptr;
+  if (MASKED) {
+    mw = mask + (int64_t)(((int)(blockIdx.x % ntile) * ZCT) >> 4) * nw;
+    uint32_t any = 0;
+    for (int w = 0; w < nw; ++w) any |= mw[w];
+    if (any == 0) return;
+  }
   double2* x = lds;
   double2* tw = lds + n * ZCT;
   for (int k = threadIdx.x; k < n; k += TPB) tw[k] = ax.tw[k];
@@ -534,8 +542,17 @@
   }
   for (int c = threadIdx.x; c < n * ZCT; c += TPB) {
     const int e = c / ZCT, m = c & (ZCT - 1);
+    if (MASKED && !((mw[e >> 5] >> (e & 31)) & 1u)) continue;
     if (m < M) base[(int64_t)e * es + m] = x[c];
   }
+}
+
+__global__ void spectral_mask_kernel(const int32_t* __restrict__ idx, int npts, int n, int es, int nw, uint32_t* __restrict__ mask) {
+  const int i = blockIdx.x * blockDim.x + threadIdx.x;
+  if (i >= npts) return;
+  const int p = idx[i], e = p / es, m = p - e * es;
+  if (p < 0 || e >= n) return;
+  atomicOr(&mask[(int64_t)(m >> 4) * nw + (e >> 5)], 1u << (e & 31));
 }
 
 constexpr int TPBP = 1024;
@@ -983,10 +1000,19 @@
 
 template <int MODE>
 void launch_strided(isdf_handle h, bool fast, int L, double2* data, int64_t nouter, int64_t os, int64_t es, int Mtot, const Axis& ax,
-                    const double* table) {
+                    const double* table, const uint32_t* mask = nullptr) {
   const int nt = (int)cdiv(Mtot, L);
   const dim3 grid((unsigned)(nouter * nt));
   const size_t n = ax.n;
+  if constexpr (MODE == 0) {
+    if (fast && mask) {
+      with_lines(L, [&](auto z) {
+        strided_fft_fast_kernel<0, decltype(z)::value, true><<<grid, dim3(TPB), sizeof(double2) * (n * L + n), h->stream>>>(
+            data, os, es, Mtot, ax, nt, table, mask, (int)cdiv(ax.n, 32));
+      });
+      return;
+    }
+  }
   if (fast)
     with_lines(L, [&](auto z) {
       strided_fft_fast_kernel<MODE, decltype(z)::value><<<grid, dim3(TPB), sizeof(double2) * (n * L + n), h->stream>>>(
@@ -1137,7 +1163,7 @@
 }
 
 int spectral_rows_own(isdf_handle h, const double* d_in, int nb, const int32_t mesh[3], const int32_t* d_idx,
-                      const double* d_scale, int npts, double* d_out, int64_t ldx, double2* zbuf) {
+                      const double* d_scale, int npts, double* d_out, int64_t ldx, double2* zbuf, const uint32_t* d_mask) {
   const int n0 = mesh[0], n1 = mesh[1], n2 = mesh[2], n2h = n2 / 2 + 1;
   Axis ax[3];
   if (int rc = make_axes(h, mesh, ax, "spectral_rows_own")) return rc;
@@ -1147,10 +1173,22 @@
   ARG_CHECK(h, geo.bytes && FX >= 1 && (int64_t)nb * n0 < 2147483647LL && nb <= 65535 && (ldx & 1) == 0 && ldx >= 2 * (int64_t)npts);
   ProfScope ps(h, "spectral_rows_own[byte]", (8.0 * (double)n0 * n1 * n2 + 8.0 * (double)ldx) * nb, 3);
   if (int rc = launch_plane_fwd(h, d_in, zbuf, ax, geo, (int)((int64_t)nb * n0), PIPE_ANY)) return rc;
-  launch_strided<0>(h, true, FX, zbuf, nb, gc, (int64_t)n1 * n2h, n1 * n2h, ax[0], nullptr);
+  launch_strided<0>(h, true, FX, zbuf, nb, gc, (int64_t)n1 * n2h, n1 * n2h, ax[0], nullptr, h->spectral_prune ? d_mask : nullptr);
   const int64_t ldx2 = ldx / 2;
   spectral_pack_kernel<<<dim3((unsigned)cdiv(ldx2, 256), (unsigned)nb), dim3(256), 0, h->stream>>>(zbuf, gc, d_idx, d_scale, npts,
                                                                                                   (double2*)d_out, ldx2);
+  KERNEL_CHECK(h);
+  return ISDF_OK;
+}
+
+int64_t spectral_mask_words(const int32_t mesh[3]) {
+  return cdiv((int64_t)mesh[1] * (mesh[2] / 2 + 1), 16) * cdiv(mesh[0], 32);
+}
+
+int spectral_mask_own(isdf_handle h, const int32_t* d_idx, int npts, const int32_t mesh[3], uint32_t* d_mask) {
+  const int es = mesh[1] * (mesh[2] / 2 + 1);
+  HIP_TRY(h, hipMemsetAsync(d_mask, 0, sizeof(uint32_t) * (size_t)spectral_mask_words(mesh), h->stream));
+  spectral_mask_kernel<<<dim3((unsigned)cdiv(npts, 256)), dim3(256), 0, h->stream>>>(d_idx, npts, mesh[0], es, (int)cdiv(mesh[0], 32), d_mask);
   KERNEL_CHECK(h);
   return ISDF_OK;
 }
diff --git a/pyscf_isdf_amd/csrc/fit.hip b/pyscf_isdf_amd/csrc/fit.hip
--- a/pyscf_isdf_amd/csrc/fit.hip
+++ b/pyscf_isdf_amd/csrc/fit.hip
@@ -390,11 +390,21 @@
   if (i < (int64_t)P * P) E[i] = (i / P == i % P) ? 1.0 : 0.0;
   (void)blk_of_row;
 }
+__global__ void unit_diag_kernel(double* __restrict__ E, int P) {
+  const int i = blockIdx.x * blockDim.x + threadIdx.x;
+  if (i < P) E[(int64_t)i * P + i] = 1.0;
+}
 }
 
 extern "C" int isdf_block_invert(isdf_handle h, const double* d_D, int P, int nblk, const int32_t* blk_off, double* d_Dinv) {
   if (!h) return ISDF_ERR_ARG;
   ARG_CHECK(h, d_D && d_Dinv && blk_off && P > 0 && nblk > 0 && blk_off[0] == 0 && blk_off[nblk] <= P);
+  if (h->block_invert_own) {
+    HIP_TRY(h, hipMemsetAsync(d_Dinv, 0, sizeof(double) * (size_t)P * P, h->stream));
+    hipLaunchKernelGGL(unit_diag_kernel, dim3((unsigned)cdiv(P, 256)), dim3(256), 0, h->stream, d_Dinv, P);
+    KERNEL_CHECK(h);
+    return block_forward_solve_own(h, d_D, P, nblk, blk_off, d_Dinv, P);
+  }
   hipLaunchKernelGGL(block_identity_kernel, dim3((unsigned)cdiv((int64_t)P * P, 256)), dim3(256), 0, h->stream, d_Dinv, P,
                      (const int32_t*)nullptr);
   KERNEL_CHECK(h);
@@ -428,9 +438,9 @@
   return ISDF_OK;
 }
 
-extern "C" int isdf_pair_rows_frontier(isdf_handle h, const double* d_aoP, int nnew, int nao, const double* d_ao, int64_t ng,
-                                       int64_t ld, int squared, const double* d_Dinv, int64_t ldd, int nblk,
-                                       const int32_t* blk_off, double* d_B, int64_t ldb, int have) {
+static int pair_rows_frontier(isdf_handle h, const double* d_aoP, int nnew, int nao, const double* d_ao, int64_t ng, int64_t ld,
+                              int squared, const double* d_Dinv, int64_t ldd, int nblk, const int32_t* blk_off, double* d_B,
+                              int64_t ldb, int have, const RowsProbe* probe) {
   if (!h) return ISDF_ERR_ARG;
   ARG_CHECK(h, d_ao && d_B && nnew >= 0 && nnew <= 65535 && have >= 0 && nblk >= 0 && nao > 0 && ng > 0 && ld >= ng && ldb >= ng);
   ARG_CHECK(h, (nnew == 0 || d_aoP) && (nblk == 0 || (d_Dinv && blk_off && blk_off[0] == 0 && blk_off[nblk] <= have + nnew)));
@@ -441,7 +451,23 @@
     if (rc) return rc;
   }
   if (nblk == 0) return ISDF_OK;
-  return block_apply_inverse(h, d_Dinv, ldd, nblk, blk_off, d_B, ldb, ng, !squared);
+  return block_apply_inverse(h, d_Dinv, ldd, nblk, blk_off, d_B, ldb, ng, !squared, probe);
+}
+
+extern "C" int isdf_pair_rows_frontier(isdf_handle h, const double* d_aoP, int nnew, int nao, const double* d_ao, int64_t ng,
+                                       int64_t ld, int squared, const double* d_Dinv, int64_t ldd, int nblk,
+                                       const int32_t* blk_off, double* d_B, int64_t ldb, int have) {
+  return pair_rows_frontier(h, d_aoP, nnew, nao, d_ao, ng, ld, squared, d_Dinv, ldd, nblk, blk_off, d_B, ldb, have, nullptr);
+}
+
+extern "C" int isdf_pair_rows_frontier_probe(isdf_handle h, const double* d_aoP, int nnew, int nao, const double* d_ao, int64_t ng,
+                                             int64_t ld, int squared, const double* d_Dinv, int64_t ldd, int nblk,
+                                             const int32_t* blk_off, double* d_B, int64_t ldb, int have, const double* d_E, int n,
+                                             int64_t ldE, double* d_F, int64_t ldf, int accumulate) {
+  if (!h) return ISDF_ERR_ARG;
+  ARG_CHECK(h, d_E && d_F && n > 0 && ldf >= ng && (nblk == 0 || (blk_off && ldE >= blk_off[nblk])));
+  const RowsProbe probe{d_E, n, ldE, d_F, ldf, accumulate};
+  return pair_rows_frontier(h, d_aoP, nnew, nao, d_ao, ng, ld, squared, d_Dinv, ldd, nblk, blk_off, d_B, ldb, have, &probe);
 }
 
 extern "C" int isdf_shift_diag(isdf_handle h, double* d_A, int P, double shift_rel) {
diff --git a/pyscf_isdf_amd/csrc/handle.hip b/pyscf_isdf_amd/csrc/handle.hip
--- a/pyscf_isdf_amd/csrc/handle.hip
+++ b/pyscf_isdf_amd/csrc/handle.hip
@@ -112,6 +112,9 @@
   }
   if (std::string(key) == "block_apply_waves") { h->block_apply_waves = value < 1 ? 1 : value; return ISDF_OK; }
   if (std::string(key) == "block_apply_reg") { h->block_apply_reg = value ? 1 : 0; return ISDF_OK; }
+  if (std::string(key) == "spectral_prune") { h->spectral_prune = value ? 1 : 0; return ISDF_OK; }
+  if (std::string(key) == "rows_probe_fused") { h->rows_probe_fused = value ? 1 : 0; return ISDF_OK; }
+  if (std::string(key) == "block_invert_own") { h->block_invert_own = value ? 1 : 0; return ISDF_OK; }
   return isdf_fail(h, ISDF_ERR_ARG, "isdf_set_option: unknown key '%s'", key);
 }
 
diff --git a/pyscf_isdf_amd/csrc/trsm.hip b/pyscf_isdf_amd/csrc/trsm.hip
--- a/pyscf_isdf_amd/csrc/trsm.hip
+++ b/pyscf_isdf_amd/csrc/trsm.hip
@@ -56,14 +56,15 @@
   }
 }
 
+template <bool OWN>
 __global__ __launch_bounds__(256) void block_forward_kernel(const double* __restrict__ D, int64_t ldd,
                                                             const int32_t* __restrict__ blk_off,
                                                             double* __restrict__ X, int64_t ldx, int64_t n) {
   const int b = blockIdx.y;
   const int off = blk_off[b], m = blk_off[b + 1] - off;
   if (m <= 0) return;
-  const int64_t c = (int64_t)blockIdx.x * 256 + threadIdx.x;
-  if (c >= n) return;
+  const int64_t c = (int64_t)blockIdx.x * 256 + threadIdx.x + (OWN ? off : 0);
+  if (c >= (OWN ? (int64_t)off + m : n)) return;
   const double* Db = D + (int64_t)off * ldd + off;
   double* Xb = X + (int64_t)off * ldx + c;
   const int nsub = (m + 63) >> 6;
@@ -171,10 +172,18 @@
   }
 }
 
-template <int NT, int NCT, bool SQ>
+struct ProbeArgs {
+  const double* E;
+  int64_t ldE;
+  double* part;
+  int64_t ldp;
+  int np;
+};
+template <int NT, int NCT, bool SQ, bool PROBE>
 __global__ __launch_bounds__(64 * ((NT + 1) / 2)) __attribute__((amdgpu_waves_per_eu(1, 2))) void block_apply_reg_kernel(const double* __restrict__ Dinv, int64_t ldd,
                                                                             const int32_t* __restrict__ blk_off,
-                                                                            double* __restrict__ X, int64_t ldx, int64_t n) {
+                                                                            double* __restrict__ X, int64_t ldx, int64_t n,
+                                                                            ProbeArgs pr) {
   constexpr int TN = 16 * NCT;
   constexpr int LDB = TN + 2;
   constexpr int NPAIR = (NT + 1) / 2;
@@ -202,6 +211,25 @@
 #pragma unroll
     for (int j = 0; j < 8; ++j) a[8 * c + j] = (live && k0 + j < m) ? pa[j] : 0.0;
   }
+  constexpr bool E_LDS = PROBE && NT == 12;
+  double* const sP = sB + MP * LDB;
+  double* const sE = sP + NPAIR * 8 * TN;
+  double ea[4] = {0.0, 0.0, 0.0, 0.0}, eb[4] = {0.0, 0.0, 0.0, 0.0};
+  if (PROBE) {
+#pragma unroll
+    for (int r = 0; r < 4; ++r) {
+      const int rowA = tA * 16 + fk + 4 * r, rowB = tB * 16 + fk + 4 * r;
+      if (fr < pr.np && rowA < m) ea[r] = pr.E[(int64_t)fr * pr.ldE + off + rowA];
+      if (nchB > 0 && fr < pr.np && rowB < m) eb[r] = pr.E[(int64_t)fr * pr.ldE + off + rowB];
+    }
+    if (E_LDS) {
+#pragma unroll
+      for (int r = 0; r < 4; ++r) {
+        sE[(pair * 8 + r) * 64 + lane] = ea[r];
+        sE[(pair * 8 + 4 + r) * 64 + lane] = eb[r];
+      }
+    }
+  }
   const int64_t ntile = (n + TN - 1) / TN;
   double pre[NPRE];
   const int r0 = threadIdx.x / TN, cc = threadIdx.x % TN;
@@ -260,31 +288,71 @@
           }
         }
       }
+      if (PROBE) {
+        d4v accF = (d4v){0.0, 0.0, 0.0, 0.0};
+#pragma unroll
+        for (int r = 0; r < 4; ++r)
+          accF = __builtin_amdgcn_mfma_f64_16x16x4f64(E_LDS ? sE[(pair * 8 + r) * 64 + lane] : ea[r], accA[r], accF, 0, 0, 0);
+        if (nchB > 0) {
+#pragma unroll
+          for (int r = 0; r < 4; ++r)
+            accF = __builtin_amdgcn_mfma_f64_16x16x4f64(E_LDS ? sE[(pair * 8 + 4 + r) * 64 + lane] : eb[r], accB[r], accF, 0, 0, 0);
+        }
+        sP[(pair * 8 + fk) * TN + 16 * ct + fr] = accF[0];
+        sP[(pair * 8 + fk + 4) * TN + 16 * ct + fr] = accF[1];
+      }
     }
     __syncthreads();
-  }
+    if (PROBE) {
+      for (int idx = threadIdx.x; idx < pr.np * TN; idx += NTHREADS) {
+        const int j = idx / TN, c = idx - j * TN;
+        if (c0 + c < n) {
+          double s_ = sP[j * TN + c];
+#pragma unroll
+          for (int w = 1; w < NPAIR; ++w) s_ += sP[(w * 8 + j) * TN + c];
+          pr.part[((int64_t)b * pr.np + j) * pr.ldp + c0 + c] = s_;
+        }
+      }
+    }
+  }
+}
+
+__global__ __launch_bounds__(256) void rows_probe_sum_kernel(const double* __restrict__ part, int64_t ldp, int nblk,
+                                                             const int32_t* __restrict__ blk_off, int np, int64_t n,
+                                                             double* __restrict__ F, int64_t ldf, int accumulate) {
+  const int64_t g = (int64_t)blockIdx.x * 256 + threadIdx.x;
+  const int j = blockIdx.y;
+  if (g >= n) return;
+  double s_ = 0.0;
+  for (int b = 0; b < nblk; ++b)
+    if (blk_off[b + 1] > blk_off[b]) s_ += part[((int64_t)b * np + j) * ldp + g];
+  F[(int64_t)j * ldf + g] = accumulate ? F[(int64_t)j * ldf + g] + s_ : s_;
 }
 
 template <int NT, int NCT>
 static int block_apply_reg_launch(isdf_handle h, const double* Dinv, int64_t ldd, int nblk, const int32_t* d_off, double* X,
-                                  int64_t ldx, int64_t n, bool sq) {
+                                  int64_t ldx, int64_t n, bool sq, const ProbeArgs* pr) {
   constexpr int TN = 16 * NCT;
   constexpr int NTHREADS = 64 * ((NT + 1) / 2);
   static_assert(NTHREADS % TN == 0 && (16 * NT * TN) % NTHREADS == 0, "tile elements must divide evenly over the threads");
-  const size_t lds = (size_t)16 * NT * (TN + 2) * sizeof(double);
+  const size_t lds = ((size_t)16 * NT * (TN + 2) + (pr ? (size_t)((NT + 1) / 2) * 8 * (TN + (NT == 12 ? 64 : 0)) : 0)) * sizeof(double);
   const int64_t ntile = (n + TN - 1) / TN;
   const unsigned gx = (unsigned)std::max<int64_t>(1, std::min<int64_t>(ntile, ((int64_t)h->num_cu * h->block_apply_waves + nblk - 1) / nblk));
-  if (sq) {
-    if (lds > 64 * 1024)
-      HIP_TRY(h, hipFuncSetAttribute((const void*)&block_apply_reg_kernel<NT, NCT, true>, hipFuncAttributeMaxDynamicSharedMemorySize, 160 * 1024));
-    hipLaunchKernelGGL(HIP_KERNEL_NAME(block_apply_reg_kernel<NT, NCT, true>), dim3(gx, (unsigned)nblk), dim3(NTHREADS), lds, h->stream,
-                       Dinv, ldd, d_off, X, ldx, n);
+#define ISDF_BA_REG(SQ_, PROBE_)                                                                                             \
+  do {                                                                                                                       \
+    if (lds > 64 * 1024)                                                                                                     \
+      HIP_TRY(h, hipFuncSetAttribute((const void*)&block_apply_reg_kernel<NT, NCT, SQ_, PROBE_>,                             \
+                                     hipFuncAttributeMaxDynamicSharedMemorySize, 160 * 1024));                               \
+    hipLaunchKernelGGL(HIP_KERNEL_NAME(block_apply_reg_kernel<NT, NCT, SQ_, PROBE_>), dim3(gx, (unsigned)nblk), dim3(NTHREADS), \
+                       lds, h->stream, Dinv, ldd, d_off, X, ldx, n, pa);                                                     \
+  } while (0)
+  const ProbeArgs pa = pr ? *pr : ProbeArgs{nullptr, 0, nullptr, 0, 0};
+  if (pr) {
+    if (sq) ISDF_BA_REG(true, true); else ISDF_BA_REG(false, true);
   } else {
-    if (lds > 64 * 1024)
-      HIP_TRY(h, hipFuncSetAttribute((const void*)&block_apply_reg_kernel<NT, NCT, false>, hipFuncAttributeMaxDynamicSharedMemorySize, 160 * 1024));
-    hipLaunchKernelGGL(HIP_KERNEL_NAME(block_apply_reg_kernel<NT, NCT, false>), dim3(gx, (unsigned)nblk), dim3(NTHREADS), lds, h->stream,
-                       Dinv, ldd, d_off, X, ldx, n);
-  }
+    if (sq) ISDF_BA_REG(true, false); else ISDF_BA_REG(false, false);
+  }
+#undef ISDF_BA_REG
   KERNEL_CHECK(h);
   return ISDF_OK;
 }
@@ -295,8 +363,10 @@
 }
 
 int block_apply_inverse(isdf_handle h, const double* Dinv, int64_t ldd, int nblk, const int32_t* blk_off_host, double* X,
-                        int64_t ldx, int64_t n, bool square_input) {
+                        int64_t ldx, int64_t n, bool square_input, const RowsProbe* probe) {
   ARG_CHECK(h, Dinv && X && blk_off_host && nblk > 0 && n > 0 && nblk <= 65535);
+  const int rows = blk_off_host[nblk] - blk_off_host[0];
+  ARG_CHECK(h, !probe || (probe->E && probe->F && probe->n > 0 && blk_off_host[0] == 0 && probe->ldE >= rows && probe->ldf >= n));
   int mmax = 0;
   for (int b = 0; b < nblk; ++b) mmax = std::max(mmax, blk_off_host[b + 1] - blk_off_host[b]);
   const int mpad = (mmax + 31) & ~31;
@@ -316,16 +386,39 @@
     ARG_CHECK(h, (size_t)mpad * (16 + 2) * sizeof(double) <= 160 * 1024);
     tn = 16; label = "block_apply_mfma_kernel<16>[byte]";
   }
+  const bool fuse = probe && h->rows_probe_fused && reg && probe->n <= 8 && 2 * (int64_t)nblk * probe->n <= rows;
+  if (probe && !fuse) {
+    const int rc = block_apply_inverse(h, Dinv, ldd, nblk, blk_off_host, X, ldx, n, square_input, nullptr);
+    if (rc) return rc;
+    return isdf_rows_combine(h, probe->E, probe->n, probe->ldE, rows, X, n, ldx, probe->F, probe->ldf, probe->accumulate);
+  }
   int32_t* d_off = (int32_t*)isdf_ws(h, "trsm_blk_off", sizeof(int32_t) * (size_t)(nblk + 1));
   if (!d_off) return ISDF_ERR_HIP;
   HIP_TRY(h, hipMemcpyAsync(d_off, blk_off_host, sizeof(int32_t) * (size_t)(nblk + 1), hipMemcpyHostToDevice, h->stream));
+  ProbeArgs pa{nullptr, 0, nullptr, 0, 0};
+  if (fuse) {
+    pa.E = probe->E; pa.ldE = probe->ldE; pa.np = probe->n; pa.ldp = n;
+    pa.part = (double*)isdf_ws(h, "rows_probe_part", sizeof(double) * (size_t)nblk * (size_t)probe->n * (size_t)n);
+    if (!pa.part) return ISDF_ERR_HIP;
+  }
+  if (reg) {
+    const ProbeArgs* pp = fuse ? &pa : nullptr;
+    int rc;
+    {
+      ProfScope ps(h, label, 16.0 * (double)blk_off_host[nblk] * (double)n);
+      rc = nt <= 8 ? block_apply_reg_launch<8, 2>(h, Dinv, ldd, nblk, d_off, X, ldx, n, square_input, pp)
+         : nt <= 10 ? block_apply_reg_launch<10, 2>(h, Dinv, ldd, nblk, d_off, X, ldx, n, square_input, pp)
+         : nt <= 12 ? block_apply_reg_launch<12, 2>(h, Dinv, ldd, nblk, d_off, X, ldx, n, square_input, pp)
+                    : block_apply_reg_launch<16, 1>(h, Dinv, ldd, nblk, d_off, X, ldx, n, square_input, pp);
+    }
+    if (rc || !fuse) return rc;
+    ProfScope ps(h, "rows_probe_sum_kernel[byte]", 8.0 * ((double)nblk + 1.0) * probe->n * (double)n);
+    hipLaunchKernelGGL(rows_probe_sum_kernel, dim3((unsigned)cdiv(n, 256), (unsigned)probe->n), dim3(256), 0, h->stream, pa.part,
+                       pa.ldp, nblk, d_off, probe->n, n, probe->F, probe->ldf, probe->accumulate ? 1 : 0);
+    KERNEL_CHECK(h);
+    return ISDF_OK;
+  }
   ProfScope ps(h, label, 16.0 * (double)blk_off_host[nblk] * (double)n);
-  if (reg) {
-    if (nt <= 8) return block_apply_reg_launch<8, 2>(h, Dinv, ldd, nblk, d_off, X, ldx, n, square_input);
-    if (nt <= 10) return block_apply_reg_launch<10, 2>(h, Dinv, ldd, nblk, d_off, X, ldx, n, square_input);
-    if (nt <= 12) return block_apply_reg_launch<12, 2>(h, Dinv, ldd, nblk, d_off, X, ldx, n, square_input);
-    return block_apply_reg_launch<16, 1>(h, Dinv, ldd, nblk, d_off, X, ldx, n, square_input);
-  }
 #define ISDF_BA_LAUNCH(TN_, SQ_)                                                                                       \
   do {                                                                                                                 \
     if ((size_t)mpad * (TN_ + 2) * sizeof(double) > 64 * 1024) {                                                       \
@@ -356,8 +449,29 @@
   for (int b = 0; b < nblk; ++b) rows2 += (double)(blk_off_host[b + 1] - blk_off_host[b]) * (blk_off_host[b + 1] - blk_off_host[b]);
   ProfScope ps(h, "block_forward_kernel[byte]", 16.0 * (double)blk_off_host[nblk] * (double)n);
   (void)rows2;
-  hipLaunchKernelGGL(block_forward_kernel, dim3((unsigned)cdiv(n, 256), (unsigned)nblk), dim3(256), 0, h->stream, D, ldd, d_off,
+  hipLaunchKernelGGL(block_forward_kernel<false>, dim3((unsigned)cdiv(n, 256), (unsigned)nblk), dim3(256), 0, h->stream, D, ldd, d_off,
                      X, ldx, n);
+  KERNEL_CHECK(h);
+  return ISDF_OK;
+}
+
+int block_forward_solve_own(isdf_handle h, const double* D, int64_t ldd, int nblk, const int32_t* blk_off_host, double* X,
+                            int64_t ldx) {
+  ARG_CHECK(h, D && X && blk_off_host && nblk > 0 && nblk <= 65535);
+  int32_t* d_off = (int32_t*)isdf_ws(h, "trsm_blk_off", sizeof(int32_t) * (size_t)(nblk + 1));
+  if (!d_off) return ISDF_ERR_HIP;
+  HIP_TRY(h, hipMemcpyAsync(d_off, blk_off_host, sizeof(int32_t) * (size_t)(nblk + 1), hipMemcpyHostToDevice, h->stream));
+  int mmax = 0;
+  double rows2 = 0.0;
+  for (int b = 0; b < nblk; ++b) {
+    const int m = blk_off_host[b + 1] - blk_off_host[b];
+    mmax = std::max(mmax, m);
+    if (m > 0) rows2 += (double)m * m;
+  }
+  if (mmax <= 0) return ISDF_OK;
+  ProfScope ps(h, "block_forward_kernel[byte]", 16.0 * rows2);
+  hipLaunchKernelGGL(block_forward_kernel<true>, dim3((unsigned)cdiv(mmax, 256), (unsigned)nblk), dim3(256), 0, h->stream, D, ldd,
+                     d_off, X, ldx, (int64_t)0);
   KERNEL_CHECK(h);
   return ISDF_OK;
 }
diff --git a/pyscf_isdf_amd/fit_route.py b/pyscf_isdf_amd/fit_route.py
--- a/pyscf_isdf_amd/fit_route.py
+++ b/pyscf_isdf_amd/fit_route.py
@@ -1,4 +1,9 @@
 import numpy as np
+
+
+def _mask_kw(plan):
+    mask = plan.get('mask')
+    return {} if mask is None else {'mask': mask}
 
 
 class FitRouteMixin:
@@ -192,7 +197,9 @@
         scale = np.sqrt(mult.ravel()[idx] * w * cg.ravel()[idx])
         npts = len(idx)
         ldx = -(-2 * npts // 128) * 128
-        return dict(idx=be.to_device(idx), scale=be.to_device(scale), npts=npts, ldx=ldx, fraction=2.0 * npts / G)
+        d_idx = be.to_device(idx)
+        mask = be.spectral_mask(d_idx, mesh) if hasattr(be, 'spectral_mask') else None
+        return dict(idx=d_idx, scale=be.to_device(scale), npts=npts, ldx=ldx, fraction=2.0 * npts / G, mask=mask)
 
     def _spectral_point_set(self, mesh, box, share):
         a = np.asarray(self.cell.lattice_vectors(), dtype=float)
@@ -303,7 +310,7 @@
             rows = scratch[:take]
             if probe is not None:
                 be.rows_combine(probe[0][:, g0:g0 + take], rows, probe[1], accumulate=g0 > 0)
-            be.spectral_rows(rows, mesh, plan['idx'], plan['scale'], X[g0:g0 + take], batch=take)
+            be.spectral_rows(rows, mesh, plan['idx'], plan['scale'], X[g0:g0 + take], batch=take, **_mask_kw(plan))
             if fill > take:
                 scratch[:fill - take].copy_(scratch[take:fill].clone() if fill - take > take else scratch[take:fill])
             g0 += take
@@ -335,20 +342,25 @@
         Dinv = self._block_inverse(st['Dblk'], ip_off)
         nbat = int(self.fft_batch or 512)
         squared = be.pair_rows_squared(self.aoP, min(piece, P), self.ao, G)
+        with_probe = probe is not None and hasattr(be, 'pair_rows_frontier_probe')
         app, prod = 0, 0
         while app < P:
             new = min(piece, P - prod)
             j = int(np.searchsorted(ip_off, prod + new, side='right')) - 1
             i = int(np.searchsorted(ip_off, app))
             end = int(ip_off[j])
-            be.pair_rows_frontier(self.aoP[prod:prod + new], self.ao, G, squared, Dinv[app:, app:],
-                                  (ip_off[i:j + 1] - app).astype(np.int32), scratch, prod - app)
+            blocks = (ip_off[i:j + 1] - app).astype(np.int32)
+            if with_probe and end > app:
+                be.pair_rows_frontier_probe(self.aoP[prod:prod + new], self.ao, G, squared, Dinv[app:, app:], blocks, scratch,
+                                            prod - app, probe[0][:, app:end], probe[1], accumulate=app > 0)
+            else:
+                be.pair_rows_frontier(self.aoP[prod:prod + new], self.ao, G, squared, Dinv[app:, app:], blocks, scratch, prod - app)
             prod += new
             if end > app:
                 rows = scratch[:end - app]
-                if probe is not None:
+                if probe is not None and not with_probe:
                     be.rows_combine(probe[0][:, app:end], rows, probe[1], accumulate=app > 0)
-                be.spectral_rows(rows, mesh, plan['idx'], plan['scale'], X[app:end], batch=min(nbat, end - app))
+                be.spectral_rows(rows, mesh, plan['idx'], plan['scale'], X[app:end], batch=min(nbat, end - app), **_mask_kw(plan))
                 tail = prod - end
                 if tail > 0:
                     src = scratch[end - app:prod - app]
diff --git a/pyscf_isdf_amd/lib.py b/pyscf_isdf_amd/lib.py
--- a/pyscf_isdf_amd/lib.py
+++ b/pyscf_isdf_amd/lib.py
@@ -54,6 +54,8 @@
     'isdf_pair_rows_squared': (c_int, [c_vp, c_vp, c_int, c_int, c_vp, c_i64, c_i64, ctypes.POINTER(c_int)]),
     'isdf_pair_rows_frontier': (c_int, [c_vp, c_vp, c_int, c_int, c_vp, c_i64, c_i64, c_int, c_vp, c_i64, c_int, c_vp, c_vp, c_i64,
                                         c_int]),
+    'isdf_pair_rows_frontier_probe': (c_int, [c_vp, c_vp, c_int, c_int, c_vp, c_i64, c_i64, c_int, c_vp, c_i64, c_int, c_vp, c_vp,
+                                              c_i64, c_int, c_vp, c_int, c_i64, c_vp, c_i64, c_int]),
     'isdf_shift_diag': (c_int, [c_vp, c_vp, c_int, c_dbl]),
     'isdf_chol_inplace': (c_int, [c_vp, c_vp, c_int, c_dbl, c_vp, ctypes.POINTER(c_dbl)]),
     'isdf_factor_solve': (c_int, [c_vp, c_vp, c_int, c_vp, c_i64, c_i64]),
@@ -84,6 +86,8 @@
     'isdf_coulG_half': (c_int, [c_vp, c_vp, c_vp, c_vp]),
     'isdf_spectral_supported': (c_int, [c_vp, c_vp, c_int, ctypes.POINTER(c_int)]),
     'isdf_spectral_rows': (c_int, [c_vp, c_vp, c_int, c_i64, c_vp, c_vp, c_vp, c_int, c_int, c_vp, c_i64]),
+    'isdf_spectral_mask': (c_int, [c_vp, c_vp, c_int, c_vp, c_vp]),
+    'isdf_spectral_rows_masked': (c_int, [c_vp, c_vp, c_int, c_i64, c_vp, c_vp, c_vp, c_int, c_int, c_vp, c_i64, c_vp]),
     'isdf_coulomb_rows_q': (c_int, [c_vp, c_vp, c_int, c_i64, c_vp, c_vp, c_vp, c_vp]),
     'isdf_nyquist_spectra': (c_int, [c_vp, c_vp, c_int, c_i64, c_vp, c_int, c_vp, c_vp]),
     'isdf_zhadamard_planes': (c_int, [c_vp, c_vp, c_vp, c_i64, c_vp, c_vp, c_i64, c_int, c_i64]),
diff --git a/pyscf_isdf_amd/sharded.py b/pyscf_isdf_amd/sharded.py
--- a/pyscf_isdf_amd/sharded.py
+++ b/pyscf_isdf_amd/sharded.py
@@ -4,6 +4,7 @@
 import torch
 from . import gto
 from ._common import partition_grid_by_atom, _default_fft_batch
+from .fit_route import _mask_kw
 
 
 class ShardedMixin:
@@ -410,7 +411,7 @@
             for (s0, s1), piece in zip(slices, recv):
                 rows_full[:, s0:s1] = piece
             if mine:
-                be.spectral_rows(rows_full, mesh, plan['idx'], plan['scale'], Xb[:mine], batch=mine)
+                be.spectral_rows(rows_full, mesh, plan['idx'], plan['scale'], Xb[:mine], batch=mine, **_mask_kw(plan))
             got = views(recvX, lambda q: nrow[q], lambda q: kw)
             comm.all_to_all(got, [Xb[:mine, k0:k1].contiguous() for k0, k1 in ks])
             for q in range(R):
```

After: 16.86 (median of 6 runs). No clear change (-0.5%).
